# ACMEAtronOmatic/DSen2

Measured on AMD Instinct MI355X. Metric: 32x32x6 patches/sec (DSen2_20, d=6, batch 512), higher is better.
Workload: dtype f32; 1 GPU; DSen2_20 d=6 F=128 fp32, 512 synthetic 32x32 patches (4+6 bands) per GPU per step, he_uniform random-init weights; batch_per_gpu=512, parallelism=patch-sharded dp1, backend=rccl, output_gather=False

## Files before the change

dsen2_amd/DSen2Net.py:

```python
import ctypes
import sys
import threading

import numpy as np
import torch

from . import _lib, weights as _weights

RES_SCALE = 0.1
PRECISIONS = {'fp32': 0, 'bf16': 1, 'bf16x3': 2}


def _ptr(t):
    return ctypes.c_void_p(t.data_ptr()) if t is not None else ctypes.c_void_p(0)


def _stream_ptr(device):
    return ctypes.c_void_p(torch.cuda.current_stream(device).cuda_stream)


def ensemble_mask(ensemble):
    if ensemble is None or ensemble is False:
        return 0
    if ensemble is True:
        return 255
    mask = 0
    for op in ensemble:
        if int(op) != op or not 0 <= int(op) <= 7:
            raise ValueError('an ensemble member must be an op 0..7, got %r' % (op,))
        mask |= 1 << int(op)
    if mask == 0:
        raise ValueError('an ensemble needs at least one member')
    return mask


def dihedral(x, op=None, ops=None, inverse=False, out=None):
    if not torch.cuda.is_available():
        raise RuntimeError('dsen2_amd needs a ROCm GPU (gfx950); there is no CPU fallback')
    if (op is None) == (ops is None):
        raise ValueError('give either op (one for the tensor) or ops (one per sample)')
    if x.dim() != 4 or x.dtype != torch.float32 or not x.is_contiguous() or not x.is_cuda:
        raise ValueError('x must be a contiguous float32 CUDA tensor [n, c, h, w], got %r %s %s' % (tuple(x.shape), x.dtype, x.device))
    n, c, h, w = x.shape
    ops_dev = None
    if ops is not None:
        if h != w:
            raise ValueError('per-sample ops need square images (an odd rotation swaps H and W), got %dx%d' % (h, w))
        if isinstance(ops, torch.Tensor):
            ops_dev = ops
        else:
            host = np.ascontiguousarray(ops, dtype=np.int32)
            if host.size and (host.min() < 0 or host.max() > 7):
                raise ValueError('ops must be 0..7, got %r' % (host.tolist(),))
            ops_dev = torch.from_numpy(host).to(x.device)
        if tuple(ops_dev.shape) != (n,) or ops_dev.dtype != torch.int32 or not ops_dev.is_contiguous() or ops_dev.device != x.device:
            raise ValueError('ops must hold one int32 per sample (%d) on %s' % (n, x.device))
        op = 0
    elif int(op) != op or not 0 <= int(op) <= 7:
        raise ValueError('op must be 0..7, got %r' % (op,))
    shape = (n, c, w, h) if int(op) & 1 else (n, c, h, w)
    if out is None:
        out = torch.empty(shape, dtype=torch.float32, device=x.device)
    elif tuple(out.shape) != shape or out.dtype != torch.float32 or not out.is_contiguous() or out.device != x.device:
        raise ValueError('out must be a contiguous float32 %s tensor of shape %r, got %r %s' % (x.device, shape, tuple(out.shape), out.dtype))
    with torch.cuda.device(x.device):
        _lib.call('dsen2_dihedral_nchw', _ptr(x), _ptr(out), n, c, h, w, int(op), _ptr(ops_dev), int(bool(inverse)),
                  _stream_ptr(x.device))
    return out


class S2Model(object):

    def __init__(self, input_shape, num_layers, feature_size, device=None, precision='fp32'):
        if len(input_shape) not in (2, 3):
            raise ValueError('input_shape must describe 2 or 3 inputs, got %r' % (input_shape,))
        if not torch.cuda.is_available():
            raise RuntimeError('dsen2_amd needs a ROCm GPU (gfx950); there is no CPU fallback')
        self.device = torch.device('cuda', torch.cuda.current_device()) if device is None else torch.device(device)
        self.bands = tuple(int(s[0]) for s in input_shape)
        self.num_layers = int(num_layers)
        self.feature_size = int(feature_size)
        self.cin = sum(self.bands)
        self.cout = self.bands[-1]
        self._handle = ctypes.c_void_p(0)
        c60 = self.bands[2] if len(self.bands) == 3 else 0
        with torch.cuda.device(self.device):
            if precision not in PRECISIONS:
                raise ValueError("precision must be one of %s" % ', '.join(repr(k) for k in PRECISIONS))
            self.precision = precision
            _lib.call('dsen2_model_create', ctypes.byref(self._handle), self.bands[0], self.bands[1], c60,
                      self.num_layers, self.feature_size, PRECISIONS[precision])
        self._workspaces = {}
        self._ws_lock = threading.Lock()
        self.max_workspace_bytes = 6 << 30
        self.optimizer = None
        self._train = None
        self._error_work = None

    def count_params(self):
        return int(_lib.load().dsen2_model_num_params(self._handle))

    def set_weights_flat(self, flat):
        flat = np.ascontiguousarray(flat, np.float32).ravel()
        with torch.cuda.device(self.device):
            _lib.call('dsen2_model_load_weights', self._handle,
                      flat.ctypes.data_as(_lib.c_float_p), flat.size)
            if self._train is not None:
                self._train['flat'].copy_(torch.from_numpy(flat))

    def load_weights(self, path):
        self.set_weights_flat(_weights.load_flat(path, self.cin, self.cout, self.num_layers, self.feature_size))

    def workspace_bytes(self, n, h, w, ensemble=False):
        out = ctypes.c_size_t(0)
        mask = ensemble_mask(ensemble)
        if mask:
            _lib.call('dsen2_model_ensemble_workspace_bytes', self._handle, n, h, w, mask, ctypes.byref(out))
        else:
            _lib.call('dsen2_model_workspace_bytes', self._handle, n, h, w, ctypes.byref(out))
        return out.value

    def _get_workspace(self, nbytes):
        key = torch.cuda.current_stream(self.device).cuda_stream
        with self._ws_lock:
            ws = self._workspaces.get(key)
            if ws is None or ws.numel() < nbytes:
                self._workspaces.pop(key, None)
                ws = None
                ws = torch.empty(nbytes, dtype=torch.uint8, device=self.device)
                self._workspaces[key] = ws
            return ws

    def release_workspaces(self):
        with self._ws_lock:
            self._workspaces.clear()

    def forward_device(self, xs, out=None):
        if len(xs) != len(self.bands):
            raise ValueError('expected %d inputs, got %d' % (len(self.bands), len(xs)))
        n, _, h, w = xs[0].shape
        for x, c in zip(xs, self.bands):
            if tuple(x.shape) != (n, c, h, w) or x.dtype != torch.float32 or not x.is_contiguous() or \
                    x.device != self.device:
                raise ValueError('input must be a contiguous float32 %s tensor of shape %r, got %r %s %s'
                                 % (self.device, (n, c, h, w), tuple(x.shape), x.dtype, x.device))
        out = self._check_out(out, n, h, w)
        if n == 0:
            return out
        ws = self._get_workspace(self.workspace_bytes(n, h, w))
        with torch.cuda.device(self.device):
            _lib.call('dsen2_model_forward', self._handle, _ptr(xs[0]), _ptr(xs[1]),
                      _ptr(xs[2]) if len(xs) == 3 else ctypes.c_void_p(0), _ptr(out), n, h, w,
                      _ptr(ws), ws.numel(), _stream_ptr(self.device))
        return out

    def forward_device_ensemble(self, xs, out=None, ops=range(8)):
        ops = list(range(8)) if ops is True else list(ops)
        mask = ensemble_mask(ops)
        if len(xs) != len(self.bands):
            raise ValueError('expected %d inputs, got %d' % (len(self.bands), len(xs)))
        n, _, h, w = xs[0].shape
        for x, c in zip(xs, self.bands):
            if tuple(x.shape) != (n, c, h, w) or x.dtype != torch.float32 or not x.is_contiguous() or \
                    x.device != self.device:
                raise ValueError('input must be a contiguous float32 %s tensor of shape %r, got %r %s %s'
                                 % (self.device, (n, c, h, w), tuple(x.shape), x.dtype, x.device))
        out = self._check_out(out, n, h, w)
        if n == 0:
            return out
        ws = self._get_workspace(self.workspace_bytes(n, h, w, ensemble=ops))
        with torch.cuda.device(self.device):
            _lib.call('dsen2_model_forward_ensemble', self._handle, _ptr(xs[0]), _ptr(xs[1]),
                      _ptr(xs[2]) if len(xs) == 3 else ctypes.c_void_p(0), _ptr(out), n, h, w, mask,
                      _ptr(ws), ws.numel(), _stream_ptr(self.device))
        return out

    def _check_out(self, out, n, h, w):
        if out is None:
            return torch.empty((n, self.cout, h, w), dtype=torch.float32, device=self.device)
        if tuple(out.shape) != (n, self.cout, h, w) or out.dtype != torch.float32 or not out.is_contiguous() or \
                out.device != self.device:
            raise ValueError('out must be a contiguous float32 %s tensor of shape %r, got %r %s %s (contiguous: %s)'
                             % (self.device, (n, self.cout, h, w), tuple(out.shape), out.dtype, out.device,
                                out.is_contiguous()))
        return out

    def time_body_in_forward(self, xs, out=None, iters=10):
        n, _, h, w = xs[0].shape
        out = self._check_out(out, n, h, w)
        ws = self._get_workspace(self.workspace_bytes(n, h, w))
        ms = ctypes.c_float(0)
        with torch.cuda.device(self.device):
            _lib.call('dsen2_model_forward_timed', self._handle, _ptr(xs[0]), _ptr(xs[1]),
                      _ptr(xs[2]) if len(xs) == 3 else ctypes.c_void_p(0), _ptr(out), n, h, w,
                      _ptr(ws), ws.numel(), _stream_ptr(self.device), int(iters), ctypes.byref(ms))
        return ms.value

    def profile_forward(self, xs, out=None, iters=10, warm=3):
        n, _, h, w = xs[0].shape
        out = self._check_out(out, n, h, w)
        ws = self._get_workspace(self.workspace_bytes(n, h, w))
        ms = (ctypes.c_float * 5)()
        with torch.cuda.device(self.device):
            _lib.call('dsen2_model_forward_profile', self._handle, _ptr(xs[0]), _ptr(xs[1]),
                      _ptr(xs[2]) if len(xs) == 3 else ctypes.c_void_p(0), _ptr(out), n, h, w,
                      _ptr(ws), ws.numel(), _stream_ptr(self.device), int(warm), int(iters), ms)
        return dict(forward_ms=ms[0], first_ms=ms[1], body_ms=ms[2], out_ms=ms[3], wall_ms=ms[4])

    def body_launches(self, n, h, w):
        with torch.cuda.device(self.device):
            r = _lib.load().dsen2_model_body_launches(self._handle, int(n), int(h), int(w))
        if r < 0:
            raise _lib.DSen2Error(r, _lib.load().dsen2_last_error().decode())
        return r

    def batch_limit(self, h, w, ensemble=False):
        per = self.workspace_bytes(1, h, w, ensemble=ensemble)
        return max(1, int(self.max_workspace_bytes // per))

    def preferred_batch(self, h, w, ensemble=False):
        limit = self.batch_limit(h, w, ensemble=ensemble) if ensemble_mask(ensemble) else self.batch_limit(h, w)
        if self.precision == 'fp32' or self.num_layers <= 0:
            return limit
        turned = h != w and ensemble_mask(ensemble) & 0xAA
        cus = int(torch.cuda.get_device_properties(self.device).multi_processor_count)
        n = (limit // cus) * cus
        while n >= cus:
            if self.body_launches(n, h, w) == 1 and (not turned or self.body_launches(n, w, h) == 1):
                return n
            n -= cus
        return limit

    def predict(self, x, batch_size=None, verbose=0, ensemble=False):
        xs = [np.ascontiguousarray(a, dtype=np.float32) for a in x]
        if len(xs) != len(self.bands):
            raise ValueError('expected %d inputs, got %d' % (len(self.bands), len(xs)))
        n, _, h, w = xs[0].shape
        for a, c in zip(xs, self.bands):
            if a.shape != (n, c, h, w):
                raise ValueError('input of shape %r where %r is expected' % (a.shape, (n, c, h, w)))
        mask = ensemble_mask(ensemble if isinstance(ensemble, bool) or ensemble is None else list(ensemble))
        members = [op for op in range(8) if (mask >> op) & 1]
        if batch_size is not None:
            bs = int(batch_size)
        else:
            bs = self.preferred_batch(h, w, ensemble=members) if members else self.preferred_batch(h, w)
        out = np.empty((n, self.cout, h, w), np.float32)
        if n == 0:
            return self._progress_end(verbose, out)
        starts = list(range(0, n, bs))
        bs = min(bs, n)
        with torch.cuda.device(self.device):
            comp = torch.cuda.current_stream(self.device)
            h2d, d2h = torch.cuda.Stream(self.device), torch.cuda.Stream(self.device)
            slots = []
            for _ in range(min(2, len(starts))):
                slots.append(dict(
                    pin_in=[torch.empty((bs, c, h, w), dtype=torch.float32, pin_memory=True) for c in self.bands],
                    dev_in=[torch.empty((bs, c, h, w), dtype=torch.float32, device=self.device) for c in self.bands],
                    dev_out=torch.empty((bs, self.cout, h, w), dtype=torch.float32, device=self.device),
                    pin_out=torch.empty((bs, self.cout, h, w), dtype=torch.float32, pin_memory=True),
                    ev_in=torch.cuda.Event(), ev_comp=torch.cuda.Event(), ev_out=torch.cuda.Event(), span=None))

            def collect(slot):
                if slot['span'] is not None:
                    slot['ev_out'].synchronize()
                    j0, j1 = slot['span']
                    out[j0:j1] = slot['pin_out'][:j1 - j0].numpy()
                    slot['span'] = None
                    self._progress(verbose, j1, n)

            for i, i0 in enumerate(starts):
                i1 = min(n, i0 + bs)
                m = i1 - i0
                slot = slots[i % len(slots)]
                collect(slot)
                for k, a in enumerate(xs):
                    slot['pin_in'][k][:m].numpy()[...] = a[i0:i1]
                with torch.cuda.stream(h2d):
                    for k in range(len(xs)):
                        slot['dev_in'][k][:m].copy_(slot['pin_in'][k][:m], non_blocking=True)
                    slot['ev_in'].record(h2d)
                comp.wait_event(slot['ev_in'])
                if members:
                    self.forward_device_ensemble([t[:m] for t in slot['dev_in']], out=slot['dev_out'][:m], ops=members)
                else:
                    self.forward_device([t[:m] for t in slot['dev_in']], out=slot['dev_out'][:m])
                slot['ev_comp'].record(comp)
                with torch.cuda.stream(d2h):
                    d2h.wait_event(slot['ev_comp'])
                    slot['pin_out'][:m].copy_(slot['dev_out'][:m], non_blocking=True)
                    slot['ev_out'].record(d2h)
                slot['span'] = (i0, i1)
            last = len(starts) - 1
            if len(slots) > 1:
                collect(slots[(last - 1) % 2])
            collect(slots[last % len(slots)])
        return self._progress_end(verbose, out)

    @staticmethod
    def _progress(verbose, done, total):
        if verbose:
            sys.stdout.write('\r%d/%d' % (done, total))
            sys.stdout.flush()

    @staticmethod
    def _progress_end(verbose, out):
        if verbose:
            sys.stdout.write('\n')
        return out

    def time_body_conv(self, layer, x_in, aux, out, iters=10):
        n, h, w, _ = x_in.shape
        ms = ctypes.c_float(0)
        with torch.cuda.device(self.device):
            _lib.call('dsen2_model_time_body_conv', self._handle, layer, _ptr(x_in), _ptr(aux), _ptr(out), n, h, w,
                      iters, _stream_ptr(self.device), ctypes.byref(ms))
        return ms.value

    TRAINABLE = ('fp32', 'bf16x3')
    MIXED_PRECISIONS = {None: 0, 'bf16': 1}

    def compile(self, optimizer='nadam', loss='mean_absolute_error', metrics=None, mixed_precision=None, *, loss_param=None,
                mask_nodata=False, ssim_weight=0.0, ssim_win=11, ssim_sigma=1.5, ssim_data_range=5.0):
        from . import training, losses
        if self.precision not in self.TRAINABLE:
            raise ValueError('training needs an fp32 or a bf16x3 model (this one is %r)' % self.precision)
        if mixed_precision not in self.MIXED_PRECISIONS:
            raise ValueError("mixed_precision must be None or 'bf16', got %r" % (mixed_precision,))
        if mixed_precision is not None and self.precision != 'fp32':
            raise ValueError('mixed_precision=%r is an option of an fp32 model (this one is %r)' % (mixed_precision, self.precision))
        setting = losses.parse_ssim(losses.parse(loss, loss_param, mask_nodata), ssim_weight, ssim_win, ssim_sigma, ssim_data_range)
        if isinstance(optimizer, str):
            if optimizer.lower() != 'nadam':
                raise ValueError("optimizer must be 'nadam' or a dsen2_amd.training.Nadam, got %r" % optimizer)
            optimizer = training.Nadam()
        if not isinstance(optimizer, training.Nadam):
            raise ValueError('optimizer must be a dsen2_amd.training.Nadam')
        if self.precision == 'fp32':
            with torch.cuda.device(self.device):
                _lib.call('dsen2_model_set_train_precision', self._handle, self.MIXED_PRECISIONS[mixed_precision])
        with torch.cuda.device(self.device):
            _lib.call('dsen2_model_set_loss', self._handle, setting[0], setting[1], setting[2])
            ssim = losses.ssim_part(setting) or (0.0, 11, 1.5, 5.0)
            window, c1, c2 = losses.ssim_constants(ssim)
            _lib.call('dsen2_model_set_loss_ssim', self._handle, ssim[0], (ctypes.c_double * window.size)(*window.tolist()),
                      int(window.size), c1, c2)
        self.loss_setting = setting
        self.mixed_precision = mixed_precision
        self.optimizer = optimizer
        self.optimizer.reset()
        self._train = None
        self.stop_training = False

    def _train_state(self):
        if getattr(self, 'optimizer', None) is None:
            raise RuntimeError('compile() the model before training it')
        if self._train is None:
            count = self.count_params()
            kw = dict(dtype=torch.float32, device=self.device)
            flat = torch.empty(count, **kw)
            with torch.cuda.device(self.device):
                _lib.call('dsen2_model_get_weights', self._handle, _ptr(flat), _stream_ptr(self.device))
            self._train = dict(flat=flat, grad=torch.empty(count, **kw), m=torch.zeros(count, **kw),
                               v=torch.zeros(count, **kw), loss2=torch.empty(2, **kw), ws=None)
        return self._train

    def train_workspace_bytes(self, n, h, w):
        out = ctypes.c_size_t(0)
        _lib.call('dsen2_model_train_workspace_bytes', self._handle, n, h, w, ctypes.byref(out))
        return out.value

    def gradients_device(self, xs, y, grad, loss2, out=None, workspace=None):
        if self.precision not in self.TRAINABLE:
            raise ValueError('training needs an fp32 or a bf16x3 model (this one is %r)' % self.precision)
        n, _, h, w = xs[0].shape
        for x, c in zip(xs, self.bands):
            if tuple(x.shape) != (n, c, h, w) or x.dtype != torch.float32 or not x.is_contiguous() or x.device != self.device:
                raise ValueError('input must be a contiguous float32 %s tensor of shape %r' % (self.device, (n, c, h, w)))
        if len(xs) != len(self.bands):
            raise ValueError('expected %d inputs, got %d' % (len(self.bands), len(xs)))
        if tuple(y.shape) != (n, self.cout, h, w) or y.dtype != torch.float32 or not y.is_contiguous() or y.device != self.device:
            raise ValueError('target must be a contiguous float32 %s tensor of shape %r, got %r'
                             % (self.device, (n, self.cout, h, w), tuple(y.shape)))
        if grad.numel() != self.count_params() or not grad.is_contiguous() or loss2.numel() < 2:
            raise ValueError('grad must hold num_params floats, loss2 two')
        if out is not None:
            out = self._check_out(out, n, h, w)
        if workspace is None:
            need = self.train_workspace_bytes(n, h, w)
            st = self._train if self._train is not None else {}
            if st.get('ws') is None or st['ws'].numel() < need:
                st['ws'] = None
                st['ws'] = torch.empty(need, dtype=torch.uint8, device=self.device)
            workspace = st['ws']
        with torch.cuda.device(self.device):
            _lib.call('dsen2_model_gradients', self._handle, _ptr(xs[0]), _ptr(xs[1]),
                      _ptr(xs[2]) if len(xs) == 3 else ctypes.c_void_p(0), _ptr(y), _ptr(out), _ptr(grad), _ptr(loss2),
                      n, h, w, _ptr(workspace), workspace.numel(), _stream_ptr(self.device))
        return out

    def set_weights_device(self, flat):
        if flat.numel() != self.count_params() or flat.dtype != torch.float32 or not flat.is_contiguous() or \
                flat.device != self.device:
            raise ValueError('flat must be a contiguous float32 %s tensor of %d values' % (self.device, self.count_params()))
        with torch.cuda.device(self.device):
            _lib.call('dsen2_model_set_weights_device', self._handle, _ptr(flat), _stream_ptr(self.device))
            if self._train is not None and flat.data_ptr() != self._train['flat'].data_ptr():
                self._train['flat'].copy_(flat)

    def nadam_update(self, grad):
        st = self._train_state()
        s = self.optimizer.next_step()
        with torch.cuda.device(self.device):
            _lib.call('dsen2_nadam_step', _ptr(st['flat']), _ptr(grad), _ptr(st['m']), _ptr(st['v']), st['flat'].numel(),
                      s['lr'], s['b1'], s['b2'], s['eps'], s['mc_t'], s['mc_t1'], s['ms_new'], s['ms_next'], s['b2_pow_t'],
                      _stream_ptr(self.device))
        self.set_weights_device(st['flat'])

    def _to_device(self, arrays, shapes):
        out = []
        for a, shp in zip(arrays, shapes):
            a = np.ascontiguousarray(a, dtype=np.float32)
            if a.shape != shp:
                raise ValueError('array of shape %r where %r is expected' % (a.shape, shp))
            out.append(torch.from_numpy(a).to(self.device))
        return out

    def _shard_rows(self, k):
        st = self._train_state()
        count = st['flat'].numel()
        rows = st.get('rows')
        if rows is None or rows.shape[0] != k:
            stride = -(-(count + 2) // 4) * 4
            rows = st['rows'] = torch.empty((k, stride), dtype=torch.float32, device=self.device)
        return rows

    def nadam_update_shards(self, buf, counts, g_mean=None):
        st = self._train_state()
        count = st['flat'].numel()
        counts = [int(c) for c in counts]
        if buf.dim() != 2 or buf.shape[0] != len(counts) or buf.shape[1] < count or buf.dtype != torch.float32 or \
                buf.device != self.device or buf.stride(1) != 1 or (len(counts) > 1 and buf.stride(0) < count):
            raise ValueError('buf must hold %d float32 %s rows of at least %d values, got %r strides %r'
                             % (len(counts), self.device, count, tuple(buf.shape), buf.stride()))
        if g_mean is not None and (g_mean.numel() != count or g_mean.dtype != torch.float32 or not g_mean.is_contiguous() or
                                   g_mean.device != self.device):
            raise ValueError('g_mean must be a contiguous float32 %s tensor of %d values' % (self.device, count))
        before = (self.optimizer.iterations, self.optimizer.m_schedule)
        s = self.optimizer.next_step()
        try:
            with torch.cuda.device(self.device):
                _lib.call('dsen2_nadam_step_shards', _ptr(st['flat']), _ptr(buf), max(buf.stride(0), count), len(counts),
                          (ctypes.c_int * len(counts))(*counts), _ptr(g_mean), _ptr(st['m']), _ptr(st['v']), count,
                          s['lr'], s['b1'], s['b2'], s['eps'], s['mc_t'], s['mc_t1'], s['ms_new'], s['ms_next'], s['b2_pow_t'],
                          _stream_ptr(self.device))
        except Exception:
            self.optimizer.iterations, self.optimizer.m_schedule = before
            raise
        self.set_weights_device(st['flat'])

    @staticmethod
    def weighted_loss(loss2, counts):
        total = float(sum(counts))
        acc = [0.0, 0.0]
        for l2, c in zip(loss2, counts):
            if c > 0:
                acc[0] += float(c) * float(l2[0])
                acc[1] += float(c) * float(l2[1])
        return [acc[0] / total, acc[1] / total]

    @staticmethod
    def _check_augment_ops(augment_ops, n, h, w):
        if augment_ops is None:
            return None
        ops = np.ascontiguousarray(augment_ops, dtype=np.int32)
        if ops.shape != (n,) or (n and (ops.min() < 0 or ops.max() > 7)):
            raise ValueError('augment_ops must hold one op 0..7 for each of the %d samples, got %r' % (n, np.asarray(augment_ops).tolist()))
        if h != w:
            raise ValueError('augmentation turns every sample by its own op: it needs square patches, got %dx%d' % (h, w))
        return ops

    def _augment_device(self, tensors, ops):
        if ops is None:
            return tensors
        ops_dev = torch.from_numpy(ops).to(self.device)
        return [dihedral(t, ops=ops_dev) for t in tensors]

    def _step_on_shards(self, fetch, counts, mine=None, augment_ops=None):
        from . import dist
        count = self._train_state()['flat'].numel()
        rows = self._shard_rows(len(counts) if mine is None else 1)
        first = 0
        for r, n in enumerate(counts):
            if n > 0 and mine in (None, r):
                x, y = fetch(first, n)
                _, _, h, w = np.shape(x[0])
                if isinstance(y, torch.Tensor):
                    xs, yd = list(x), y
                else:
                    xs = self._to_device(x, [(n, c, h, w) for c in self.bands])
                    yd = self._to_device([y], [(n, self.cout, h, w)])[0]
                if augment_ops is not None:
                    *xs, yd = self._augment_device(xs + [yd], self._check_augment_ops(augment_ops[first:first + n], n, h, w))
                row = rows[r if mine is None else 0]
                self.gradients_device(xs, yd, row[:count], row[count:count + 2])
            first += n
        if mine is not None:
            rows = dist.all_gather_rows(rows[0])
        self.nadam_update_shards(rows, counts)
        return self.weighted_loss(rows[:, count:count + 2].cpu().numpy().astype(np.float64), counts)

    def _shard_counts(self, n, shards):
        from . import dist
        if isinstance(shards, (int, np.integer)):
            if shards < 1:
                raise ValueError('shards must be at least 1, got %d' % shards)
            return [dist.shard_range(n, r, int(shards))[1] for r in range(int(shards))]
        counts = [int(c) for c in shards]
        if not counts or min(counts) < 0 or sum(counts) != n:
            raise ValueError('the shard counts %r must be non-negative and add up to the batch of %d' % (counts, n))
        return counts

    def train_on_batch(self, x, y, shards=None, augment_ops=None):
        st = self._train_state()
        if len(x) != len(self.bands):
            raise ValueError('expected %d inputs, got %d' % (len(self.bands), len(x)))
        n, _, h, w = np.shape(x[0])
        ops = self._check_augment_ops(augment_ops, n, h, w)
        if shards is not None:
            counts = self._shard_counts(n, shards)
            x = [np.ascontiguousarray(a, dtype=np.float32) for a in x]
            y = np.ascontiguousarray(y, dtype=np.float32)
            if y.shape != (n, self.cout, h, w) or any(a.shape != (n, c, h, w) for a, c in zip(x, self.bands)):
                raise ValueError('inputs %r and target %r do not describe one batch' % ([a.shape for a in x], y.shape))
            return self._step_on_shards(lambda first, m: ([a[first:first + m] for a in x], y[first:first + m]), counts,
                                        augment_ops=ops)
        xs = self._to_device(x, [(n, c, h, w) for c in self.bands])
        yd = self._to_device([y], [(n, self.cout, h, w)])[0]
        *xs, yd = self._augment_device(xs + [yd], ops)
        self.gradients_device(xs, yd, st['grad'], st['loss2'])
        self.nadam_update(st['grad'])
        loss = st['loss2'].cpu().numpy().astype(np.float64)
        return [float(loss[0]), float(loss[1])]

    def train_on_device_batch(self, xs, y, loss_out=None):
        st = self._train_state()
        loss2 = st['loss2'] if loss_out is None else loss_out
        if loss2.dtype != torch.float32 or loss2.numel() != 2 or not loss2.is_contiguous() or loss2.device != self.device:
            raise ValueError('loss_out must be a contiguous float32 %s tensor of two values' % (self.device,))
        self.gradients_device(list(xs), y, st['grad'], loss2)
        self.nadam_update(st['grad'])
        return loss2

    def evaluate(self, x, y, batch_size=None, verbose=0):
        y = np.asarray(y, dtype=np.float32)
        pred = self.predict(x, batch_size=batch_size, verbose=verbose)
        if pred.shape != y.shape:
            raise ValueError('target of shape %r where %r is expected' % (y.shape, pred.shape))
        from . import losses
        return losses.host_loss(pred, y, self._loss_setting())

    def _loss_setting(self):
        from . import losses
        return getattr(self, 'loss_setting', losses.DEFAULT)

    def _means_of_triples(self, triples, mine):
        if mine is not None:
            from . import dist
            triples = dist.all_gather_rows(torch.from_numpy(triples[mine]).to(self.device)).cpu().numpy()
        sa = sq = cnt = 0.0
        for t in triples:
            sa, sq, cnt = sa + t[0], sq + t[1], cnt + t[2]
        return [float(sa / cnt), float(sq / cnt)]

    def _evaluate_shards(self, x, y, batch_size, world, mine=None):
        from . import dist, losses
        y = np.asarray(y, dtype=np.float32)
        n = y.shape[0]
        triples = np.zeros((world, 3), np.float64)
        for r in range(world):
            if mine in (None, r):
                first, cnt = dist.shard_range(n, r, world)
                pred = self.predict([a[first:first + cnt] for a in x], batch_size=batch_size)
                triples[r] = losses.host_sums(pred, y[first:first + cnt], self._loss_setting())
        return self._means_of_triples(triples, mine)

    def _data_parallel_plan(self, data_parallel, emulate_world):
        if not data_parallel and emulate_world is None:
            return None
        from . import dist
        rank, world = dist.rank_world()
        if emulate_world is not None:
            if not data_parallel or world > 1 or int(emulate_world) < 1:
                raise ValueError('emulate_world restates a data-parallel run in ONE process: it needs data_parallel=True, a world '
                                 'of at least 1 and no process group of more than one rank')
            return (int(emulate_world), None) if int(emulate_world) > 1 else None
        return (world, rank) if data_parallel and world > 1 else None

    def _data_parallel_start(self, seed):
        from . import dist
        rank, _ = dist.rank_world()
        payload = None
        if rank == 0:
            if seed is None:
                seed = int(np.random.SeedSequence().generate_state(1, np.uint64)[0] >> np.uint64(1))
            payload = np.concatenate([self.get_weights_flat(), np.array([seed], np.uint64).view(np.float32)])
        payload = dist.broadcast_weights(payload, self.count_params() + 2, device=self.device)
        self.set_weights_flat(payload[:-2])
        return int(payload[-2:].view(np.uint64)[0])

    def _sums_device(self, pred, target, out, setting=None):
        for t in (pred, target):
            if t.dtype != torch.float32 or not t.is_contiguous() or t.device != self.device or tuple(t.shape) != tuple(pred.shape) \
                    or (setting is not None and t.dim() != 4):
                raise ValueError('pred and target must be contiguous float32 %s %stensors of one shape'
                                 % (self.device, 'NCHW ' if setting is not None else ''))
        if out.dtype != torch.float64 or out.numel() != 2 or not out.is_contiguous() or out.device != self.device:
            raise ValueError('out must be a contiguous float64 %s tensor of two values' % (self.device,))
        need = ctypes.c_size_t(0)
        _lib.call('dsen2_abs_sq_error_sums_workspace_bytes' if setting is None else 'dsen2_loss_sums_workspace_bytes', ctypes.byref(need))
        size = need.value + (0 if setting is None else 24)
        work = self._error_work
        if work is None or work.numel() < size:
            work = self._error_work = torch.empty(size, dtype=torch.uint8, device=self.device)
        with torch.cuda.device(self.device):
            if setting is None:
                _lib.call('dsen2_abs_sq_error_sums', _ptr(pred), _ptr(target), pred.numel(), _ptr(work), work.numel(), _ptr(out),
                          _stream_ptr(self.device))
                return out
            out3 = work[need.value:need.value + 24].view(torch.float64)
            n, c, h, w = pred.shape
            kind, param, mask = setting
            _lib.call('dsen2_loss_sums', _ptr(pred), _ptr(target), n, c, h * w, kind, param, mask, _ptr(work), need.value, _ptr(out3),
                      _stream_ptr(self.device))
        out.copy_(out3[:2])
        return out

    def abs_sq_error_sums_device(self, pred, target, out):
        return self._sums_device(pred, target, out)

    def loss_sums_device(self, pred, target, out):
        from . import losses
        setting = self._loss_setting()
        kind, param, mask = losses.pointwise(setting)
        self._sums_device(pred, target, out, None if (kind, mask) == (0, 0) else (kind, param, mask))
        if losses.ssim_part(setting):
            s3 = self._ssim_sums_device(pred, target, setting)
            out[0:1].add_(s3[0:1] * losses.ssim_fold(setting, tuple(pred.shape)))
        return out

    def _ssim_sums_device(self, pred, target, setting):
        from . import losses
        window, c1, c2 = losses.ssim_constants(losses.ssim_part(setting))
        need = ctypes.c_size_t(0)
        _lib.call('dsen2_ssim_loss_sums_workspace_bytes', ctypes.byref(need))
        work = getattr(self, '_ssim_work', None)
        if work is None or work.numel() < need.value + 24 or work.device != self.device:
            work = self._ssim_work = torch.empty(need.value + 24, dtype=torch.uint8, device=self.device)
        out3 = work[need.value:need.value + 24].view(torch.float64)
        n, c, h, w = pred.shape
        with torch.cuda.device(self.device):
            _lib.call('dsen2_ssim_loss_sums', _ptr(pred), _ptr(target), n, c, h, w, (ctypes.c_double * window.size)(*window.tolist()),
                      int(window.size), c1, c2, setting[2], _ptr(work), need.value, _ptr(out3), _stream_ptr(self.device))
        return out3

    def _validation_rows(self, corpus, table, rows):
        from . import training
        chunk = self._validation_chunk(corpus)
        for j, i0 in enumerate(range(0, table.shape[0], chunk)):
            xs, y = corpus.batch(table[i0:i0 + chunk], divisor=training.SCALE)
            self.loss_sums_device(self.forward_device(xs), y, rows[j])

    def _validation_chunk(self, corpus):
        return max(1, int(self.preferred_batch(corpus.patch, corpus.patch)))

    @staticmethod
    def _check_validation_crops(corpus, validation_crops):
        table = corpus.check_table(validation_crops)
        if table.shape[0] == 0:
            raise ValueError('validation_crops holds no sample')
        if (table[:, 3] != 0).any():
            raise ValueError('validation is never augmented: every row of validation_crops must have op 0 (corpus.validation_table '
                             'draws such rows), got ops %r' % (sorted(set(table[:, 3].tolist())),))
        return table

    def _validate_crops(self, corpus, table, plan):
        from . import dist
        world, mine = plan
        elements = self.cout * corpus.patch * corpus.patch
        chunk = self._validation_chunk(corpus)
        triples = np.zeros((world, 3), np.float64)
        for r in range(world):
            if mine in (None, r):
                first, cnt = dist.shard_range(table.shape[0], r, world)
                if cnt > 0:
                    rows = torch.empty((-(-cnt // chunk), 2), dtype=torch.float64, device=self.device)
                    self._validation_rows(corpus, table[first:first + cnt], rows)
                    sa = sq = 0.0
                    for row in rows.cpu().numpy():
                        sa, sq = sa + row[0], sq + row[1]
                    triples[r] = (sa, sq, float(cnt * elements))
        return self._means_of_triples(triples, mine)

    def _end_epoch(self, epoch, epochs, sums, count, validation_data, batch_size, plan, callbacks, history, verbose, val=None):
        logs = {'loss': sums[0] / count, 'mean_squared_error': sums[1] / count}
        if val is not None:
            logs['val_loss'], logs['val_mean_squared_error'] = val
        elif validation_data is not None:
            if plan is None:
                vl = self.evaluate(validation_data[0], validation_data[1], batch_size=batch_size)
            else:
                vl = self._evaluate_shards(validation_data[0], validation_data[1], batch_size, plan[0], plan[1])
            logs['val_loss'], logs['val_mean_squared_error'] = vl
        logs['lr'] = self.optimizer.lr
        if verbose:
            sys.stdout.write('\rEpoch %d/%d ' % (epoch + 1, epochs) +
                             ' '.join('%s %.4e' % kv for kv in logs.items()) + '\n')
        for cb in callbacks:
            cb.on_epoch_end(epoch, logs)
        history.append(epoch, logs)
        if plan is not None and plan[1] is not None:
            from . import dist
            dist.assert_replicas_identical(self._train['flat'])

    def fit(self, x=None, y=None, batch_size=32, epochs=1, verbose=1, callbacks=None, validation_data=None, shuffle=True,
            initial_epoch=0, seed=None, data_parallel=False, emulate_world=None, augment=False):
        from . import training
        if getattr(y, 'class_masked', False) or (validation_data is not None and getattr(validation_data[1], 'class_masked', False)):
            training.check_masked_target(self._loss_setting(), True, 'fit')
        plan = self._data_parallel_plan(data_parallel, emulate_world)
        x = [np.ascontiguousarray(a, dtype=np.float32) for a in x]
        y = np.ascontiguousarray(y, dtype=np.float32)
        count = y.shape[0]
        if any(a.shape[0] != count for a in x):
            raise ValueError('inputs and target hold different numbers of samples')
        self._train_state()
        callbacks = list(callbacks or [])
        history = training.History()
        for cb in callbacks:
            cb.set_model(self)
            cb.on_train_begin()
        if plan is not None:
            seed = self._data_parallel_start(seed)
        rng = np.random.default_rng(seed)
        aug = training.AugmentOps(seed) if augment else None
        self.stop_training = False
        for epoch in range(initial_epoch, epochs):
            order = rng.permutation(count) if shuffle else np.arange(count)
            sums = np.zeros(2)
            for i0 in range(0, count, batch_size):
                idx = order[i0:i0 + batch_size]
                ops = aug.draw(len(idx)) if aug is not None else None
                if plan is None:
                    r = self.train_on_batch([a[idx] for a in x], y[idx], augment_ops=ops)
                else:
                    r = self._step_on_shards(lambda first, m: ([a[idx[first:first + m]] for a in x], y[idx[first:first + m]]),
                                             self._shard_counts(len(idx), plan[0]), plan[1], augment_ops=ops)
                sums += np.asarray(r) * len(idx)
                if verbose:
                    sys.stdout.write('\rEpoch %d/%d %d/%d loss %.4e' % (epoch + 1, epochs, min(i0 + batch_size, count), count,
                                                                     sums[0] / min(i0 + batch_size, count)))
                    sys.stdout.flush()
            self._end_epoch(epoch, epochs, sums, count, validation_data, batch_size, plan, callbacks, history, verbose)
            if self.stop_training:
                break
        return history

    def fit_corpus(self, corpus, batch_size, steps_per_epoch, epochs=1, validation_data=None, seed=None, augment=False,
                   callbacks=None, initial_epoch=0, verbose=1, shards=None, data_parallel=False, emulate_world=None,
                   validation_crops=None, masks=None):
        from . import training
        from .corpus import CorpusSampler
        if getattr(corpus, 'class_masked', False):
            training.check_masked_target(self._loss_setting(), True, 'fit_corpus')
        plan = self._data_parallel_plan(data_parallel, emulate_world)
        if plan is not None and shards is not None:
            raise ValueError('shards is the one-process cut of a batch: it cannot be combined with data_parallel')
        batch_size, steps = int(batch_size), int(steps_per_epoch)
        if batch_size < 1 or steps < 1:
            raise ValueError('batch_size and steps_per_epoch must be at least 1, got %d and %d' % (batch_size, steps))
        if corpus.device != self.device or tuple(c for c in self.bands) != tuple(s[1] for s in corpus.output_shapes(1)[0]) or \
                self.cout != corpus.cout:
            raise ValueError('the corpus (%s, run_60=%r) does not feed this model (%s, bands %r)'
                             % (corpus.device, corpus.run_60, self.device, tuple(self.bands)))
        if validation_crops is not None and validation_data is not None:
            raise ValueError('validation_data (host arrays) and validation_crops (a sample table, validated on the device) exclude '
                             'each other')
        val_table = None if validation_crops is None else self._check_validation_crops(corpus, validation_crops)
        self._train_state()
        callbacks = list(callbacks or [])
        history = training.History()
        for cb in callbacks:
            cb.set_model(self)
            cb.on_train_begin()
        if plan is not None:
            seed = self._data_parallel_start(seed)
        sampler = CorpusSampler(corpus, seed, augment, masks=masks)
        sharded = plan is not None or shards is not None
        chunks = 0
        if val_table is not None and plan is None:
            chunks = -(-val_table.shape[0] // self._validation_chunk(corpus))
            val_elements = float(val_table.shape[0] * self.cout * corpus.patch * corpus.patch)
        report = torch.empty((0 if sharded else steps) * 8 + chunks * 16, dtype=torch.uint8, device=self.device)
        if chunks:
            val_rows = report[report.numel() - chunks * 16:].view(torch.float64).view(chunks, 2)
        if not sharded:
            losses = report[:steps * 8].view(torch.float32).view(steps, 2)
            tables = torch.empty((steps, batch_size, 4), dtype=torch.int32).pin_memory()
            tables_dev = torch.empty((steps, batch_size, 4), dtype=torch.int32, device=self.device)
        count = steps * batch_size
        self.stop_training = False
        for epoch in range(initial_epoch, epochs):
            sums = np.zeros(2)
            for i in range(steps):
                table = sampler.draw(batch_size)
                if not sharded:
                    tables[i].numpy()[...] = table
                    tables_dev[i].copy_(tables[i], non_blocking=True)
                    xs, y = corpus.batch(table, table_dev=tables_dev[i])
                    self.train_on_device_batch(xs, y, loss_out=losses[i])
                else:
                    counts = self._shard_counts(batch_size, shards if plan is None else plan[0])
                    r = self._step_on_shards(lambda first, m: corpus.batch(table[first:first + m]), counts,
                                             None if plan is None else plan[1])
                    sums += np.asarray(r) * batch_size
                if verbose:
                    sys.stdout.write('\rEpoch %d/%d %d/%d' % (epoch + 1, epochs, (i + 1) * batch_size, count))
                    sys.stdout.flush()
            val = None
            if chunks:
                self._validation_rows(corpus, val_table, val_rows)
            if not sharded or chunks:
                host = report.cpu().numpy()
                if not sharded:
                    for r in host[:steps * 8].view(np.float32).reshape(steps, 2).astype(np.float64):
                        sums += r * batch_size
                if chunks:
                    sa = sq = 0.0
                    for row in host[host.size - chunks * 16:].view(np.float64).reshape(chunks, 2):
                        sa, sq = sa + row[0], sq + row[1]
                    val = [float(sa / val_elements), float(sq / val_elements)]
            elif val_table is not None:
                val = self._validate_crops(corpus, val_table, plan)
            self._end_epoch(epoch, epochs, sums, count, validation_data, batch_size, plan, callbacks, history, verbose, val=val)
            if self.stop_training:
                break
        return history

    def get_weights_flat(self):
        if self._train is not None:
            flat = self._train['flat']
        else:
            flat = torch.empty(self.count_params(), dtype=torch.float32, device=self.device)
            with torch.cuda.device(self.device):
                _lib.call('dsen2_model_get_weights', self._handle, _ptr(flat), _stream_ptr(self.device))
        return flat.cpu().numpy()

    def save_weights(self, path):
        np.save(path, self.get_weights_flat())

    def __del__(self):
        try:
            if self._handle:
                _lib.load().dsen2_model_destroy(self._handle)
                self._handle = ctypes.c_void_p(0)
        except Exception:
            pass


def s2model(input_shape, num_layers=32, feature_size=256, device=None, precision='fp32'):
    return S2Model(input_shape, num_layers, feature_size, device=device, precision=precision)


def to_blocked(x_nhwc):
    n, h, w, c = x_nhwc.shape
    return x_nhwc.reshape(n, h, w, c // 8, 8).permute(0, 3, 1, 2, 4).contiguous()


def from_blocked(x_blk):
    n, b, h, w, e = x_blk.shape
    return x_blk.permute(0, 2, 3, 1, 4).reshape(n, h, w, b * e).contiguous()


def split_f32(x):
    x = x.contiguous()
    n, h, w, c = x.shape
    hi = torch.empty((n, c // 8, h, w, 8), dtype=torch.int16, device=x.device)
    lo = torch.empty_like(hi)
    with torch.cuda.device(x.device):
        _lib.call('dsen2_split_f32', _ptr(x), _ptr(hi), _ptr(lo), n, h, w, c, _stream_ptr(x.device))
    return hi, lo


def join_f32(hi, lo):
    n, b, h, w, e = hi.shape
    out = torch.empty((n, h, w, b * e), dtype=torch.float32, device=hi.device)
    with torch.cuda.device(hi.device):
        _lib.call('dsen2_join_f32', _ptr(hi), _ptr(lo), _ptr(out), n, h, w, b * e, _stream_ptr(hi.device))
    return out


def split3_f32(x):
    x = x.contiguous()
    n, h, w, c = x.shape
    hx = torch.empty((n, 2, c // 8, h, w, 8), dtype=torch.int16, device=x.device)
    lo = torch.empty((n, c // 8, h, w, 8), dtype=torch.int16, device=x.device)
    with torch.cuda.device(x.device):
        _lib.call('dsen2_split3_f32', _ptr(x), _ptr(hx), _ptr(lo), n, h, w, c, _stream_ptr(x.device))
    return hx, lo


def join3_f32(hx, lo):
    n, _, b, h, w, e = hx.shape
    out = torch.empty((n, h, w, b * e), dtype=torch.float32, device=hx.device)
    with torch.cuda.device(hx.device):
        _lib.call('dsen2_join3_f32', _ptr(hx), _ptr(lo), _ptr(out), n, h, w, b * e, _stream_ptr(hx.device))
    return out


def conv3x3_wgrad_bf16x3(a_planes, g_planes, scale=1.0):
    n, _, b, h, w, e = a_planes.shape
    feat = b * e
    if tuple(g_planes.shape) != tuple(a_planes.shape) or not a_planes.is_contiguous() or not g_planes.is_contiguous():
        raise ValueError('a_planes and g_planes must be contiguous tensors of the same shape')
    dw = torch.empty((3, 3, feat, feat), dtype=torch.float32, device=a_planes.device)
    db = torch.empty(feat, dtype=torch.float32, device=a_planes.device)
    with torch.cuda.device(a_planes.device):
        _lib.call('dsen2_conv3x3_wgrad_bf16x3', _ptr(a_planes), _ptr(g_planes), _ptr(dw), _ptr(db), n, h, w, feat, float(scale),
                  _stream_ptr(a_planes.device))
    return dw, db


def bf16_plane_f32(x):
    return split_f32(x)[0]


def conv3x3_wgrad_bf16(a_plane, g_plane, scale=1.0):
    n, b, h, w, e = a_plane.shape
    feat = b * e
    if tuple(g_plane.shape) != tuple(a_plane.shape) or not a_plane.is_contiguous() or not g_plane.is_contiguous() or \
            a_plane.element_size() != 2 or g_plane.element_size() != 2:
        raise ValueError('a_plane and g_plane must be contiguous 16-bit tensors of the same shape')
    dw = torch.empty((3, 3, feat, feat), dtype=torch.float32, device=a_plane.device)
    db = torch.empty(feat, dtype=torch.float32, device=a_plane.device)
    with torch.cuda.device(a_plane.device):
        _lib.call('dsen2_conv3x3_wgrad_bf16', _ptr(a_plane), _ptr(g_plane), _ptr(dw), _ptr(db), n, h, w, feat, float(scale),
                  _stream_ptr(a_plane.device))
    return dw, db


WGRAD_KINDS = {'fp32': 0, 'bf16x3': 1, 'bf16': 2}


def conv3x3_wgrad_geometry(kind, n, h, w, ca, cg=None):
    cg = ca if cg is None else cg
    tiles, splits, floats = ctypes.c_longlong(0), ctypes.c_int(0), ctypes.c_size_t(0)
    _lib.call('dsen2_conv3x3_wgrad_geometry', WGRAD_KINDS[kind], n, h, w, ca, cg, ctypes.byref(tiles), ctypes.byref(splits),
              ctypes.byref(floats))
    return tiles.value, splits.value, floats.value


def conv3x3_first_planes(xs, kernel_hwio, bias, precision):
    kernel_hwio = np.ascontiguousarray(kernel_hwio, np.float32)
    bias = np.ascontiguousarray(bias, np.float32)
    feat = kernel_hwio.shape[3]
    n, _, h, w = xs[0].shape
    dev = xs[0].device
    xs = [x.contiguous() for x in xs]
    if precision == 2:
        out = torch.empty((n, 2, feat // 8, h, w, 8), dtype=torch.int16, device=dev)
    else:
        out = torch.empty((n, feat // 8, h, w, 8), dtype=torch.int16, device=dev)
    out2 = torch.empty((n, feat // 8, h, w, 8), dtype=torch.int16, device=dev)
    with torch.cuda.device(dev):
        _lib.call('dsen2_conv3x3_first_planes', _ptr(xs[0]), _ptr(xs[1]), _ptr(xs[2]) if len(xs) == 3 else ctypes.c_void_p(0),
                  xs[0].shape[1], xs[1].shape[1], xs[2].shape[1] if len(xs) == 3 else 0,
                  kernel_hwio.ctypes.data_as(_lib.c_float_p), bias.ctypes.data_as(_lib.c_float_p), int(feat), int(precision),
                  _ptr(out), _ptr(out2), n, h, w, _stream_ptr(dev))
    return out, out2


def conv3x3_body_bf16x3(x_planes, kernel_hwio, bias, epilogue=0, res_hx=None, res_lo=None, res_scale=RES_SCALE):
    n, _, blocks, h, w, _ = x_planes.shape
    feat = blocks * 8
    kernel_hwio = np.ascontiguousarray(kernel_hwio, np.float32)
    bias = np.ascontiguousarray(bias, np.float32)
    out = None
    if epilogue == 0:
        out = torch.empty((n, 2, feat // 8, h, w, 8), dtype=torch.int16, device=x_planes.device)
    elif epilogue == 3:
        out = torch.empty((n, h, w, feat), dtype=torch.float32, device=x_planes.device)
    with torch.cuda.device(x_planes.device):
        _lib.call('dsen2_conv3x3_body_bf16x3', _ptr(x_planes.contiguous()), kernel_hwio.ctypes.data_as(_lib.c_float_p),
                  bias.ctypes.data_as(_lib.c_float_p), _ptr(res_hx), _ptr(res_lo), _ptr(out), n, h, w, feat, int(epilogue),
                  float(res_scale), _stream_ptr(x_planes.device))
    return (res_hx, res_lo) if epilogue == 1 else out


def conv3x3_body_bf16(x_bf16, kernel_hwio, bias, epilogue=0, res_hi=None, res_lo=None, res_scale=RES_SCALE):
    n, h, w, feat = x_bf16.shape
    kernel_hwio = np.ascontiguousarray(kernel_hwio, np.float32)
    bias = np.ascontiguousarray(bias, np.float32)
    xb = to_blocked(x_bf16)
    out = None
    if epilogue == 0:
        out = torch.empty((n, feat // 8, h, w, 8), dtype=torch.bfloat16, device=x_bf16.device)
    elif epilogue == 3:
        out = torch.empty((n, h, w, feat), dtype=torch.float32, device=x_bf16.device)
    with torch.cuda.device(x_bf16.device):
        _lib.call('dsen2_conv3x3_body_bf16', _ptr(xb), kernel_hwio.ctypes.data_as(_lib.c_float_p),
                  bias.ctypes.data_as(_lib.c_float_p), _ptr(res_hi), _ptr(res_lo), _ptr(out), n, h, w, feat, int(epilogue),
                  float(res_scale), _stream_ptr(x_bf16.device))
    if epilogue == 1:
        return res_hi, res_lo
    return from_blocked(out) if epilogue == 0 else out


def conv3x3_nhwc(x, kernel_hwio, bias, epilogue=0, aux=None, res_scale=RES_SCALE, ref=False):
    n, h, w, cin = x.shape
    kernel_hwio = np.ascontiguousarray(kernel_hwio, np.float32)
    bias = np.ascontiguousarray(bias, np.float32)
    cout = kernel_hwio.shape[3]
    if epilogue == 2:
        out = torch.empty((n, cout, h, w), dtype=torch.float32, device=x.device)
    else:
        out = torch.empty((n, h, w, cout), dtype=torch.float32, device=x.device)
    with torch.cuda.device(x.device):
        _lib.call('dsen2_conv3x3_nhwc_ref' if ref else 'dsen2_conv3x3_nhwc', _ptr(x), kernel_hwio.ctypes.data_as(_lib.c_float_p),
                  bias.ctypes.data_as(_lib.c_float_p), _ptr(aux), _ptr(out), n, h, w, cin, cout, int(epilogue),
                  float(res_scale), _stream_ptr(x.device))
    return out
```

dsen2_amd/_lib.py:

```python
import ctypes
import os
import sys

_HERE = os.path.dirname(os.path.abspath(__file__))
LIB_PATH = os.environ.get('DSEN2_HIP_LIB') or os.path.join(_HERE, 'libdsen2_hip.so')

OK = 0
ERR_INVALID, ERR_HIP, ERR_NO_WEIGHTS, ERR_WORKSPACE, ERR_NO_DEVICE, ERR_NOMEM, ERR_INTERNAL = -1, -2, -3, -4, -5, -6, -7
DTYPE_U16, DTYPE_F32 = 0, 1
DTYPE_F64 = 2
MASK_BLANK_MAP = 3

c_float_p = ctypes.POINTER(ctypes.c_float)
c_int_p = ctypes.POINTER(ctypes.c_int)
c_void_p = ctypes.c_void_p
c_int = ctypes.c_int
c_size_t = ctypes.c_size_t
c_double = ctypes.c_double


class CorpusTile(ctypes.Structure):
    _fields_ = [('dev_lr10', c_void_p), ('dev_lr20', c_void_p), ('dev_lr60', c_void_p), ('dev_gt', c_void_p),
                ('grid_h', c_int), ('grid_w', c_int), ('gt_dtype', c_int)]


SIGNATURES = {
    'dsen2_version': (ctypes.c_char_p, []),
    'dsen2_last_error': (ctypes.c_char_p, []),
    'dsen2_device_count': (c_int, []),
    'dsen2_model_create': (c_int, [ctypes.POINTER(c_void_p), c_int, c_int, c_int, c_int, c_int, c_int]),
    'dsen2_model_destroy': (None, [c_void_p]),
    'dsen2_model_num_params': (c_size_t, [c_void_p]),
    'dsen2_model_load_weights': (c_int, [c_void_p, c_float_p, c_size_t]),
    'dsen2_model_workspace_bytes': (c_int, [c_void_p, c_int, c_int, c_int, ctypes.POINTER(c_size_t)]),
    'dsen2_model_forward': (c_int, [c_void_p, c_void_p, c_void_p, c_void_p, c_void_p, c_int, c_int, c_int,
                                    c_void_p, c_size_t, c_void_p]),
    'dsen2_model_body_launches': (c_int, [c_void_p, c_int, c_int, c_int]),
    'dsen2_dihedral_nchw': (c_int, [c_void_p, c_void_p, c_int, c_int, c_int, c_int, c_int, c_void_p, c_int, c_void_p]),
    'dsen2_dihedral_accumulate': (c_int, [c_void_p, c_void_p, c_int, c_int, c_int, c_int, c_int, c_int, c_void_p]),
    'dsen2_model_ensemble_workspace_bytes': (c_int, [c_void_p, c_int, c_int, c_int, c_int, ctypes.POINTER(c_size_t)]),
    'dsen2_model_forward_ensemble': (c_int, [c_void_p, c_void_p, c_void_p, c_void_p, c_void_p, c_int, c_int, c_int, c_int,
                                             c_void_p, c_size_t, c_void_p]),
    'dsen2_model_forward_timed': (c_int, [c_void_p, c_void_p, c_void_p, c_void_p, c_void_p, c_int, c_int, c_int,
                                          c_void_p, c_size_t, c_void_p, c_int, c_float_p]),
    'dsen2_model_forward_profile': (c_int, [c_void_p, c_void_p, c_void_p, c_void_p, c_void_p, c_int, c_int, c_int,
                                            c_void_p, c_size_t, c_void_p, c_int, c_int, c_float_p]),
    'dsen2_conv3x3_nhwc': (c_int, [c_void_p, c_float_p, c_float_p, c_void_p, c_void_p, c_int, c_int, c_int, c_int,
                                   c_int, c_int, ctypes.c_float, c_void_p]),
    'dsen2_conv3x3_nhwc_ref': (c_int, [c_void_p, c_float_p, c_float_p, c_void_p, c_void_p, c_int, c_int, c_int, c_int,
                                       c_int, c_int, ctypes.c_float, c_void_p]),
    'dsen2_split_f32': (c_int, [c_void_p, c_void_p, c_void_p, c_int, c_int, c_int, c_int, c_void_p]),
    'dsen2_join_f32': (c_int, [c_void_p, c_void_p, c_void_p, c_int, c_int, c_int, c_int, c_void_p]),
    'dsen2_conv3x3_body_bf16': (c_int, [c_void_p, c_float_p, c_float_p, c_void_p, c_void_p, c_void_p, c_int, c_int, c_int,
                                        c_int, c_int, ctypes.c_float, c_void_p]),
    'dsen2_conv3x3_first_planes': (c_int, [c_void_p, c_void_p, c_void_p, c_int, c_int, c_int, c_float_p, c_float_p, c_int, c_int,
                                           c_void_p, c_void_p, c_int, c_int, c_int, c_void_p]),
    'dsen2_split3_f32': (c_int, [c_void_p, c_void_p, c_void_p, c_int, c_int, c_int, c_int, c_void_p]),
    'dsen2_conv3x3_body_bf16x3': (c_int, [c_void_p, c_float_p, c_float_p, c_void_p, c_void_p, c_void_p, c_int, c_int, c_int,
                                          c_int, c_int, ctypes.c_float, c_void_p]),
    'dsen2_model_time_body_conv': (c_int, [c_void_p, c_int, c_void_p, c_void_p, c_void_p, c_int, c_int, c_int, c_int,
                                           c_void_p, c_float_p]),
    'dsen2_model_train_workspace_bytes': (c_int, [c_void_p, c_int, c_int, c_int, ctypes.POINTER(c_size_t)]),
    'dsen2_model_gradients': (c_int, [c_void_p, c_void_p, c_void_p, c_void_p, c_void_p, c_void_p, c_void_p, c_void_p, c_int,
                                      c_int, c_int, c_void_p, c_size_t, c_void_p]),
    'dsen2_model_set_train_precision': (c_int, [c_void_p, c_int]),
    'dsen2_model_get_weights': (c_int, [c_void_p, c_void_p, c_void_p]),
    'dsen2_model_set_weights_device': (c_int, [c_void_p, c_void_p, c_void_p]),
    'dsen2_nadam_step': (c_int, [c_void_p, c_void_p, c_void_p, c_void_p, c_size_t] + [ctypes.c_float] * 9 + [c_void_p]),
    'dsen2_nadam_step_shards': (c_int, [c_void_p, c_void_p, c_size_t, c_int, c_int_p, c_void_p, c_void_p, c_void_p, c_size_t] +
                                [ctypes.c_float] * 9 + [c_void_p]),
    'dsen2_conv3x3_wgrad': (c_int, [c_void_p, c_void_p, c_void_p, c_void_p, c_int, c_int, c_int, c_int, c_int, c_int, c_int,
                                    ctypes.c_float, c_void_p]),
    'dsen2_conv3x3_wgrad_bf16x3': (c_int, [c_void_p, c_void_p, c_void_p, c_void_p, c_int, c_int, c_int, c_int, ctypes.c_float,
                                           c_void_p]),
    'dsen2_conv3x3_wgrad_bf16': (c_int, [c_void_p, c_void_p, c_void_p, c_void_p, c_int, c_int, c_int, c_int, ctypes.c_float,
                                         c_void_p]),
    'dsen2_conv3x3_wgrad_geometry': (c_int, [c_int, c_int, c_int, c_int, c_int, c_int, ctypes.POINTER(ctypes.c_longlong), c_int_p,
                                             ctypes.POINTER(c_size_t)]),
    'dsen2_join3_f32': (c_int, [c_void_p, c_void_p, c_void_p, c_int, c_int, c_int, c_int, c_void_p]),
    'dsen2_upsample_mirror_bilinear': (c_int, [c_void_p, c_void_p, c_int, c_int, c_int, c_int, c_int, ctypes.c_float,
                                               c_void_p]),
    'dsen2_upsample_mirror_bilinear_ref': (c_int, [c_void_p, c_void_p, c_int, c_int, c_int, c_int, c_int, ctypes.c_float,
                                                   c_void_p]),
    'dsen2_tile_gather': (c_int, [c_void_p, c_int, c_int, c_int, c_int, c_void_p, c_int, c_int, ctypes.c_float,
                                  c_void_p, c_void_p]),
    'dsen2_recompose': (c_int, [c_void_p, c_int, c_int, c_int, c_int, c_void_p, c_int, c_int, ctypes.c_float,
                                c_void_p]),
    'dsen2_recompose_rows': (c_int, [c_void_p, c_int, c_int, c_int, c_int, c_void_p, c_int, c_int, ctypes.c_float,
                                     c_int, c_int, c_void_p]),
    'dsen2_tile_nodata_geometry': (c_int, [c_int, c_int, c_int, c_int, c_int_p, c_int_p, ctypes.POINTER(c_size_t)]),
    'dsen2_tile_nodata': (c_int, [c_void_p, c_int, c_int, c_int, c_int, c_int, c_void_p, c_void_p, c_void_p]),
    'dsen2_recompose_rows_nodata': (c_int, [c_void_p, c_int, c_int, c_int, c_int, c_void_p, c_void_p, c_void_p, c_int, c_int,
                                            ctypes.c_float, c_int, c_int, c_void_p]),
    'dsen2_recompose_rows_blend': (c_int, [c_void_p, c_int, c_int, c_int, c_int, c_int, c_void_p, c_void_p, c_void_p, c_int, c_int,
                                           ctypes.c_float, c_int, c_int, c_void_p]),
    'dsen2_corpus_create': (c_int, [c_void_p, c_int, c_int, ctypes.POINTER(c_void_p)]),
    'dsen2_corpus_destroy': (None, [c_void_p]),
    'dsen2_corpus_batch': (c_int, [c_void_p, c_void_p, c_void_p, c_int, ctypes.c_float, c_void_p, c_void_p, c_void_p, c_void_p,
                                   c_void_p]),
    'dsen2_corpus_origin_mask': (c_int, [c_void_p, c_int, c_int, c_int, c_int, c_int, c_int, c_void_p, c_void_p, c_int, c_int, c_void_p,
                                         c_void_p, c_void_p, c_void_p]),
    'dsen2_class_valid_bits': (c_int, [c_void_p, c_int, c_int, c_void_p, c_int, c_int, c_int, c_int, c_int, c_void_p, c_void_p, c_void_p]),
    'dsen2_tile_flags_from_bits': (c_int, [c_void_p, c_int, c_int, c_int, c_int, c_void_p, c_void_p]),
    'dsen2_raster_apply_valid': (c_int, [c_void_p, c_int, c_int, c_int, c_int, c_void_p, c_void_p]),
    'dsen2_cells_from_valid_bits': (c_int, [c_void_p, c_int, c_int, c_int, c_int, c_void_p, c_void_p]),
    'dsen2_abs_sq_error_sums_workspace_bytes': (c_int, [ctypes.POINTER(c_size_t)]),
    'dsen2_abs_sq_error_sums': (c_int, [c_void_p, c_void_p, ctypes.c_longlong, c_void_p, c_size_t, c_void_p, c_void_p]),
    'dsen2_model_set_loss': (c_int, [c_void_p, c_int, ctypes.c_float, c_int]),
    'dsen2_loss_grad': (c_int, [c_void_p, c_void_p, c_int, c_int, c_int, c_int, c_int, ctypes.c_float, c_int, c_void_p, c_void_p,
                                c_void_p]),
    'dsen2_loss_sums_workspace_bytes': (c_int, [ctypes.POINTER(c_size_t)]),
    'dsen2_loss_sums': (c_int, [c_void_p, c_void_p, c_int, c_int, ctypes.c_longlong, c_int, ctypes.c_float, c_int, c_void_p, c_size_t,
                                c_void_p, c_void_p]),
    'dsen2_model_set_loss_ssim': (c_int, [c_void_p, ctypes.c_float, ctypes.POINTER(c_double), c_int, c_double, c_double]),
    'dsen2_ssim_loss_grad': (c_int, [c_void_p, c_void_p, c_int, c_int, c_int, c_int, ctypes.c_float, ctypes.POINTER(c_double), c_int,
                                     c_double, c_double, c_int, c_void_p, c_void_p, c_void_p]),
    'dsen2_ssim_loss_sums_workspace_bytes': (c_int, [ctypes.POINTER(c_size_t)]),
    'dsen2_ssim_loss_sums': (c_int, [c_void_p, c_void_p, c_int, c_int, c_int, c_int, ctypes.POINTER(c_double), c_int, c_double, c_double,
                                     c_int, c_void_p, c_size_t, c_void_p, c_void_p]),
    'dsen2_down_pixel_aggr': (c_int, [c_void_p, c_int, c_int, c_int, c_int, c_int, ctypes.POINTER(ctypes.c_double), c_int,
                                      c_void_p, c_int, c_void_p]),
    'dsen2_imresize_axis': (c_int, [c_void_p, c_int, c_int, c_int, c_int, c_int, c_int, c_void_p, c_void_p, c_int, c_void_p, c_void_p]),
    'dsen2_band_errors_workspace_bytes': (c_int, [c_int, ctypes.POINTER(c_size_t)]),
    'dsen2_band_errors': (c_int, [c_void_p, c_int, c_void_p, c_int, c_int, c_int, c_int, c_void_p, c_size_t, c_void_p, c_void_p]),
    'dsen2_imresize_band_errors': (c_int, [c_void_p, c_int, c_int, c_int, c_int, c_int, c_int, c_void_p, c_void_p, c_int, c_void_p, c_int,
                                           c_void_p, c_size_t, c_void_p, c_void_p]),
    'dsen2_quality_workspace_bytes': (c_int, [c_int, ctypes.POINTER(c_size_t)]),
    'dsen2_uiq_map': (c_int, [c_void_p, c_int, c_void_p, c_int, c_int, c_int, c_int, c_int, c_void_p, c_void_p]),
    'dsen2_uiq_sums': (c_int, [c_void_p, c_int, c_void_p, c_int, c_int, c_int, c_int, c_int, c_void_p, c_size_t, c_void_p, c_void_p]),
    'dsen2_sam_sums': (c_int, [c_void_p, c_int, c_void_p, c_int, c_int, c_int, c_int, c_void_p, c_size_t, c_void_p, c_void_p]),
    'dsen2_imresize_uiq_sums': (c_int, [c_void_p, c_int, c_int, c_int, c_int, c_int, c_int, c_void_p, c_void_p, c_int, c_void_p, c_int,
                                        c_int, c_void_p, c_size_t, c_void_p, c_void_p]),
    'dsen2_imresize_sam_sums': (c_int, [c_void_p, c_int, c_int, c_int, c_int, c_int, c_int, c_void_p, c_void_p, c_int, c_void_p, c_int,
                                        c_void_p, c_size_t, c_void_p, c_void_p]),
    'dsen2_ssim_map': (c_int, [c_void_p, c_int, c_void_p, c_int, c_int, c_int, c_int, ctypes.POINTER(c_double), c_int, c_double, c_double,
                               c_void_p, c_void_p]),
    'dsen2_ssim_sums': (c_int, [c_void_p, c_int, c_void_p, c_int, c_int, c_int, c_int, ctypes.POINTER(c_double), c_int, c_double, c_double,
                                c_void_p, c_size_t, c_void_p, c_void_p]),
    'dsen2_imresize_ssim_sums': (c_int, [c_void_p, c_int, c_int, c_int, c_int, c_int, c_int, c_void_p, c_void_p, c_int, c_void_p, c_int,
                                         ctypes.POINTER(c_double), c_int, c_double, c_double, c_void_p, c_size_t, c_void_p, c_void_p]),
}

_lib = None


class DSen2Error(RuntimeError):
    def __init__(self, code, message):
        super().__init__('libdsen2_hip error %d: %s' % (code, message))
        self.code = code


def load():
    global _lib
    if _lib is None:
        import torch
        if not os.path.exists(LIB_PATH):
            raise ImportError('%s not found: build it with `python -m dsen2_amd.build` (hipcc, gfx950). '
                              'dsen2_amd has no CPU fallback.' % LIB_PATH)
        if os.environ.get('DSEN2_HIP_LIB'):
            sys.stderr.write('dsen2_amd: DSEN2_HIP_LIB overrides the product library: loading %s\n' % LIB_PATH)
        lib = ctypes.CDLL(LIB_PATH)
        for name, (restype, argtypes) in SIGNATURES.items():
            fn = getattr(lib, name)
            fn.restype = restype
            fn.argtypes = argtypes
        _lib = lib
        want = list(filter(None, os.environ.get('DSEN2_DIAG_SET', '').split(',')))
        if want and not hasattr(lib, 'dsen2_diag_set'):
            raise ImportError('DSEN2_DIAG_SET is set but %s is not a diagnostic build' % LIB_PATH)
        for kv in want:
            key, value = kv.split('=')
            diag_set(int(key), int(value))
    return _lib


def diag_set(key, value):
    lib = load()
    if not hasattr(lib, 'dsen2_diag_set'):
        raise DSen2Error(ERR_INVALID, '%s is not a diagnostic build (python -m dsen2_amd.build --diag)' % LIB_PATH)
    fn = lib.dsen2_diag_set
    fn.restype, fn.argtypes = c_int, [c_int, c_int]
    check(fn(int(key), int(value)))


def check(code):
    if code == ERR_NOMEM:
        raise MemoryError('libdsen2_hip: ' + load().dsen2_last_error().decode('utf-8', 'replace'))
    if code != OK:
        raise DSen2Error(code, load().dsen2_last_error().decode('utf-8', 'replace'))


def call(name, *args):
    check(getattr(load(), name)(*args))
```

dsen2_amd/asm_contract.py:

```python
import os
import re
import subprocess
import tempfile

HERE = os.path.dirname(os.path.abspath(__file__))
CSRC = os.path.join(HERE, 'csrc')
DMA_SOURCES = ['conv3x3_body32.hip', 'conv3x3_body16w.hip']


class AsmContractError(RuntimeError):
    pass


def _code_lines(text):
    return [ln.strip() for ln in text.splitlines() if ln.strip() and not ln.strip().startswith((';', '.', '//'))]


def _kernels(text):
    out, name, body = {}, None, []
    for ln in text.splitlines():
        m = re.match(r'^(_Z\w+):', ln)
        if m:
            name, body = m.group(1), []
            continue
        if name is not None:
            t = ln.strip()
            if t and not t.startswith((';', '.', '//')):
                body.append(t.split(';')[0].strip())
            if t.startswith('s_endpgm'):
                out[name] = body
                name = None
    return out


def normalised(body):
    return [re.sub(r'\.L\w+', 'L', re.sub(r'\s+', ' ', ln)) for ln in body]


def compile_isa(hipcc, flags, path, out, verbose=False):
    cmd = [hipcc] + [f for f in flags if f != '-fPIC'] + ['-S', '--cuda-device-only', path, '-o', out]
    if verbose:
        print(' '.join(cmd), flush=True)
    subprocess.check_call(cmd, stderr=subprocess.DEVNULL)
    with open(out) as f:
        return f.read()


def _needer(src):
    def need(cond, msg, ctx=()):
        if not cond:
            raise AsmContractError('%s: %s %s' % (src, msg, list(ctx)))
    return need


def check_listing(text, src):
    code = _code_lines(text)
    code = [ln.split(';')[0].strip() for ln in code]
    need = _needer(src)

    m0 = [i for i, ln in enumerate(code) if re.search(r'\bm0\b', ln)]
    need(m0, 'no M0 use found (the DMA statements are gone?)')
    dma = [i for i, ln in enumerate(code) if ln.startswith('buffer_load_dword') and ln.endswith('lds')]
    need(dma, 'no LDS-DMA instruction found')
    allowed = set()
    for i in dma:
        need(code[i - 1] == 's_nop 0' and re.match(r's_mov_b32 m0, (s\d+|vcc_lo|vcc_hi)$', code[i - 2]), 'DMA without its M0 write + wait state',
             code[i - 2:i + 1])
        allowed.update((i - 2,))
        for j in range(i - 3, max(i - 7, -1), -1):
            if re.match(r's_mov_b32 (s\d+|vcc_lo|vcc_hi), m0$', code[j]):
                allowed.add(j)
                break
        k = i + 1
        if re.match(r's_mov_b32 m0, (s\d+|vcc_lo|vcc_hi)$', code[k]):
            allowed.add(k)
    for i in m0:
        need(i in allowed, 'M0 touched outside a DMA statement', code[max(0, i - 2):i + 3])
    saves = sum(1 for ln in code if re.match(r's_mov_b32 (s\d+|vcc_lo|vcc_hi), m0$', ln))
    need(saves > 0, 'the DMA statements no longer save M0')
    STEP_MFMAS = 9 * 32
    need(not any(ln.startswith(('s_swappc', 's_call')) for ln in code), 'a DMA kernel calls a function (an epilogue was not inlined)')
    kernels = _kernels(text)
    need(kernels, 'no kernel found')
    n_dma_kernels = 0
    for name, body in kernels.items():
        if not any(ln.startswith('buffer_load_dword') and ln.endswith('lds') for ln in body):
            continue
        n_dma_kernels += 1
        chain = '_chain_kernel' in name
        if not chain:
            need(not any('scratch_' in ln for ln in body), 'kernel %s spills registers' % name)
        else:
            mf = [i for i, ln in enumerate(body) if ln.startswith('v_mfma')]
            need(mf and len(mf) % STEP_MFMAS == 0, 'chain kernel %s: %d MFMAs is not a whole number of item bodies' % (name, len(mf)))
            for g in range(0, len(mf), STEP_MFMAS):
                inner = body[mf[g]:mf[g + STEP_MFMAS - 1]]
                need(not any('scratch_' in ln for ln in inner), 'chain kernel %s spills inside an item body' % name)
            for i, ln in enumerate(body):
                if 'scratch_' not in ln:
                    continue
                nxt = None
                for ln2 in body[i + 1:]:
                    if ln2.startswith('v_mfma'):
                        break
                    mm = re.search(r'vmcnt\((\d+)\)', ln2) if ln2.startswith('s_waitcnt') else None
                    if mm:
                        nxt = int(mm.group(1))
                        break
                need(nxt == 0, 'chain kernel %s: scratch access outside a drained region (next vmcnt wait: %r)' % (name, nxt), [ln])
        back = [ln for ln in body[-40:] if ln.startswith('s_waitcnt') and 'vmcnt' in ln]
        need(back and back[-1].replace(' ', '') in ('s_waitcntvmcnt(0)', 's_waitcntvmcnt(0)lgkmcnt(0)'),
             'kernel %s does not drain its DMAs before s_endpgm' % name, back[-3:])
    need(n_dma_kernels > 0, 'no LDS-DMA kernel found')
    if src == 'conv3x3_body32.hip':
        ITEM_MFMAS = 2 * 9 * 64
        asym = {k: v for k, v in kernels.items() if re.search(r'conv3x3_body32_kernelILi\d+ELi\d+ELi\d+ELi\d+ELi\d+ELi[2-9]E', k)}
        need(asym, 'no DeferAsym instantiation of the fp32 body kernel found')
        for name, body in asym.items():
            mf = [i for i, ln in enumerate(body) if ln.startswith('v_mfma')]
            need(len(mf) == 2 * ITEM_MFMAS, 'kernel %s: %d MFMAs, expected two copies of the item loop' % (name, len(mf)))
            copies = [body[mf[0]:mf[ITEM_MFMAS - 1]], body[mf[ITEM_MFMAS]:mf[-1]]]
            n_dma = [sum(1 for ln in c if ln.startswith('buffer_load_dword') and ln.endswith('lds')) for c in copies]
            need(min(n_dma) == 0 and max(n_dma) > 0, 'kernel %s: DMAs in both copies of the item loop' % name, n_dma)
            quiet, loud = (copies[0], copies[1]) if n_dma[0] == 0 else (copies[1], copies[0])
            need(not any(re.search(r'\bm0\b', ln) for ln in quiet), 'kernel %s: M0 use in the compute-only copy' % name)
            run = None
            for ln in loud:
                if re.match(r's_mov_b32 (s\d+|vcc_lo|vcc_hi), m0$', ln):
                    need(run is None, 'kernel %s: M0 saved twice in one DMA statement' % name)
                    run = 0
                elif ln.startswith('buffer_load_dword') and ln.endswith('lds'):
                    need(run is not None, 'kernel %s: DMA outside a statement that saves M0' % name)
                    run += 1
                elif run and not re.match(r'(s_mov_b32 m0, |s_nop 0$)', ln):
                    need(run in (2, 4), 'kernel %s: a DMA statement of %d instructions' % (name, run))
                    run = None
    if src == 'conv3x3_body16w.hip':
        expect = {0: (0, 32), 1: (64, 64), 3: (64, 64)}
        expect3 = {0: (0, 64), 1: (64, 96), 3: (64, 64)}

        def count(pattern, want, msg, product=lambda m: True):
            found = []
            for name, body in kernels.items():
                m = re.search(pattern, name)
                if not m or not product(m):
                    continue
                found.append(body)
                loads = sum(1 for ln in body if ln.startswith('buffer_load_dwordx4') and not ln.endswith('lds'))
                stores = sum(1 for ln in body if ln.startswith('buffer_store_dwordx4'))
                need((loads, stores) == want(m), msg(m) % (loads, stores, want(m)))
            return found

        def total(e):
            return lambda m: (sum(v[0] for v in e.values()), sum(v[1] for v in e.values()))

        found = count(r'conv3x3_body16[wx]_kernelILi(\d+)ELi(\d+)ELi(\d+)ELi(\d+)E', lambda m: expect[int(m.group(3))],
                      lambda m: 'epilogue ' + m.group(3) + ' has %d loads / %d stores, the waits count %r', lambda m: int(m.group(4)) == 0)
        need(len(found) >= 6, 'expected the 6 product instantiations of the bf16 body kernel, found %d' % len(found))
        for body in found:
            other = [ln for ln in body if re.match(r'(buffer|global|flat)_(load|store|atomic)', ln)
                     and not ln.startswith(('buffer_load_dwordx4', 'buffer_store_dwordx4'))]
            need(len(other) <= 1, 'unexpected vector-memory instructions in the bf16 body kernel', other[:4])
        found3 = count(r'conv3x3_body16w_x3_kernelILi(\d+)ELi(\d+)ELi(\d+)E', lambda m: expect3[int(m.group(3))],
                       lambda m: 'bf16x3 epilogue ' + m.group(3) + ' has %d loads / %d stores, the waits count %r')
        need(len(found3) == 6, 'expected the 6 instantiations of the bf16x3 body kernel, found %d' % len(found3))
        chains = count(r'conv3x3_body16w_chain_kernelILi(\d+)ELi(\d+)ELi(\d+)E', total(expect),
                       lambda m: 'chain kernel has %d loads / %d stores in its epilogues, the waits count %r', lambda m: int(m.group(3)) == 0)
        need(len(chains) == 2, 'expected the 2 product instantiations of the chain kernel, found %d' % len(chains))
        chains3 = count(r'conv3x3_body16w_x3_chain_kernelILi(\d+)ELi(\d+)E', total(expect3),
                        lambda m: 'bf16x3 chain kernel has %d loads / %d stores in its epilogues, the waits count %r')
        need(len(chains3) == 2, 'expected the 2 instantiations of the bf16x3 chain kernel, found %d' % len(chains3))


def check_out_mfma_listing(text, src='conv3x3_out_mfma.hip'):
    need = _needer(src)
    kernels = {k: v for k, v in _kernels(text).items() if 'conv3x3_out_mfma_kernel' in k}
    need(len(kernels) == 4, 'expected 4 instantiations of the output kernel, found %d' % len(kernels))
    for name, body in kernels.items():
        need(not any('scratch_' in ln for ln in body), 'kernel %s spills registers' % name)
        need(not any(ln.startswith(('s_swappc', 's_call')) for ln in body), 'kernel %s calls a function' % name)
        mf = [i for i, ln in enumerate(body) if ln.startswith('v_mfma')]
        need(mf, 'kernel %s has no MFMA' % name)
        waits = [ln for ln in body[mf[0]:mf[-1]] if ln.startswith('s_waitcnt') and 'vmcnt' in ln]
        need(len(waits) >= 8, 'kernel %s: no operand waits between its MFMAs' % name)
        bad = [ln for ln in waits if int(re.search(r'vmcnt\((\d+)\)', ln).group(1)) < 8]
        need(not bad, 'kernel %s waits for the loads of the NEXT unit' % name, bad[:4])
    return True


def check_first16_listing(text, src='conv3x3_first16.hip'):
    need = _needer(src)
    kernels = {k: v for k, v in _kernels(text).items() if 'conv3x3_first16_kernel' in k}
    need(len(kernels) == 8, 'expected 8 instantiations of the kernel, found %d' % len(kernels))
    for name, body in kernels.items():
        need(not any('scratch_' in ln for ln in body), 'kernel %s spills registers' % name)
        need(not any(ln.startswith(('s_swappc', 's_call')) for ln in body), 'kernel %s calls a function' % name)
        stores = [ln for ln in body if ln.startswith('buffer_store_dwordx4')]
        need(stores, 'kernel %s has no 128-bit buffer store' % name)
        bad = [ln for ln in stores if not re.search(r'\], 0 offen', ln)]
        need(not bad, 'kernel %s: 128-bit buffer store with a register soffset (late data read, unpadded hazard)' % name, bad[:2])
        need(not any(ln.startswith('global_store') for ln in body), 'kernel %s stores outside its buffer descriptors' % name)
        mf = [i for i, ln in enumerate(body) if ln.startswith('v_mfma')]
        need(mf, 'kernel %s has no MFMA' % name)
        x3 = 'ELb1EEE' in name
        floor = 24 if x3 else 16
        loop = body[mf[0]:]
        scat = [i for i, ln in enumerate(loop) if ln.startswith('ds_write_b16')]
        need(scat, 'kernel %s: no halo scatter after the first MFMA' % name)
        waits = [ln for ln in loop[:scat[-1]] if ln.startswith('s_waitcnt') and 'vmcnt' in ln]
        low = [ln for ln in waits if int(re.search(r'vmcnt\((\d+)\)', ln).group(1)) < floor]
        need(not low, 'kernel %s: a wait inside the tile loop drains the deferred stores (divergent branch in the loop body?)' % name, low[:4])
    return True


TRAFFIC_KERNELS = {
    'dsen2_20_fp32': ('conv3x3_body32.hip', r'conv3x3_body32_kernelILi128ELi128ELi0ELi0ELi0ELi4ELb1E'),
    'vdsen2_20_bf16': ('conv3x3_body16w.hip', r'conv3x3_body16w_chain_kernelILi128ELi256ELi0E'),
    'dsen2_20_bf16x3': ('conv3x3_body16w.hip', r'conv3x3_body16w_x3_chain_kernelILi64ELi128E'),
    'vdsen2_20_fp32': ('conv3x3_body32.hip', r'conv3x3_body32_kernelILi256ELi256ELi0ELi0ELi0ELi4ELb1E'),
    'dsen2_20_bf16': ('conv3x3_body16w.hip', r'conv3x3_body16w_chain_kernelILi64ELi128ELi0E'),
    'vdsen2_20_bf16x3': ('conv3x3_body16w.hip', r'conv3x3_body16w_x3_chain_kernelILi128ELi256E'),
}
ISA_JSON = os.path.join(HERE, 'kernel_isa.json')


def isa_hashes(text):
    import hashlib
    out = {}
    for name, body in _kernels(text).items():
        out[name] = hashlib.sha256('\n'.join(normalised(body)).encode()).hexdigest()
    return out


def traffic_kernel_hashes(listings):
    out = {}
    for cfg, (src, pat) in TRAFFIC_KERNELS.items():
        hits = {k: v for k, v in isa_hashes(listings[src]).items() if re.search(pat, k)}
        if len(hits) != 1:
            raise AsmContractError('%s: expected one kernel matching %s, found %d' % (src, pat, len(hits)))
        (k, v), = hits.items()
        out[cfg] = {'kernel': k, 'isa_sha256': v}
    return out


def check_sources(hipcc, flags, verbose=False, isa_json=None):
    listings = {}
    with tempfile.TemporaryDirectory(prefix='dsen2_asm_') as tmp:
        for src in DMA_SOURCES + ['conv3x3_out_mfma.hip', 'conv3x3_first16.hip']:
            listings[src] = compile_isa(hipcc, flags, os.path.join(CSRC, src), os.path.join(tmp, src + '.s'), verbose)
            if src in DMA_SOURCES:
                check_listing(listings[src], src)
            elif src == 'conv3x3_first16.hip':
                check_first16_listing(listings[src], src)
            else:
                check_out_mfma_listing(listings[src], src)
    hashes = traffic_kernel_hashes(listings)
    if isa_json:
        import json
        with open(isa_json, 'w') as f:
            json.dump(hashes, f, indent=1, sort_keys=True)
            f.write('\n')
    return hashes
```

dsen2_amd/csrc/capi.hip:

```cpp

#include <chrono>
#include <cstdarg>
#include <cstdio>
#include <cstring>
#include <exception>
#include <new>
#include <vector>

#include "capi_internal.h"

using namespace dsen2;

namespace {

thread_local char g_err[512] = "";

#ifdef DSEN2_DIAG
Tuning g_diag_tuning;
unsigned long long* g_diag_stamps = nullptr;
#endif
Tuning default_tuning() {
#ifdef DSEN2_DIAG
  return g_diag_tuning;
#else
  return Tuning{};
#endif
}

constexpr int kWarmLaunches = 24;

}

namespace dsen2 {
int fail(int code, const char* fmt, ...) {
  va_list ap;
  va_start(ap, fmt);
  vsnprintf(g_err, sizeof(g_err), fmt, ap);
  va_end(ap);
  return code;
}
}

static bool may_chain(const dsen2_model* m) {
  return m->chain_stride != 0 && m->tune.chain && m->tune.grid_cap == 0 && (m->precision == 1 || m->tune.ablate == 0);
}

static int first_layer(const dsen2_model* m, const float* x10, const float* x20, const float* x60, int n, int h, int w,
                       const ForwardWs& B, bool x0_packed, hipStream_t stream) {
  const Layer& L = m->layers[0];
  const ConvPlan& pl = L.plan;
  const float* P = m->dev_params;
  const bool x3 = m->precision == 2 && m->num_layers > 0;
  ConvParams pf = make_params(B.x0, L.weights(P), L.bias(P), nullptr, B.a, n, h, w, 0, 0.f);
  if (pl.epilogue == kEpiReluSplit) {
    pf.out = reinterpret_cast<float*>(B.s0);
    pf.out2 = B.s1;
  }
  const FirstInputs fi{x60, m->c10, m->c20, m->c60};
  ConvParams pd = pf;
  pd.in = x10;
  pd.aux = x20;
  bool done = false;
  if (pl.first16_planes) {
    pd.wpk = L.first16(P);
    pd.out = reinterpret_cast<float*>(B.s0);
    pd.out2 = B.s1;
    HIP_TRY(try_launch(launch_conv3x3_first16(pd, fi, m->feat, x3, stream), &done));
  } else if (pl.first_direct) {
    HIP_TRY(try_launch(launch_conv3x3_first(pd, fi, m->feat, pl.epilogue, stream, m->tune.first_ablate), &done));
  }
  if (!done) {
    if (!x0_packed) HIP_TRY(launch_pack_inputs(x10, x20, x60, m->c10, m->c20, m->c60, B.x0, n, h, w, stream));
    HIP_TRY(launch(pl, pf, pl.epilogue, m->tune, stream));
    if (x3) HIP_TRY(launch_split3_f32(B.a, B.s0, B.s1, n, h, w, m->feat, stream));
  }
  return DSEN2_OK;
}

static size_t operand16_bytes(const dsen2_model* m, int n, int h, int w) {
  return (size_t)n * h * w * m->feat * (m->precision == 2 ? 4 : 2);
}

static int body16(const dsen2_model* m, void* s0, void* s1, void* t16, float* out_f32, int n, int h, int w, hipStream_t stream,
                  size_t keep_step = 0, void* xkeep = nullptr) {
  const float* P = m->dev_params;
  if (keep_step == 0 && may_chain(m)) {
    const Layer& L1 = m->layers[1];
    const bool x3 = L1.plan.kernel == ConvKernel::Body16x3;
    ConvParams pc = make_params(nullptr, L1.weights(P), L1.bias(P), nullptr, nullptr, n, h, w, 0, 0.1f);
#ifdef DSEN2_DIAG
    if (!x3) pc.diag = g_diag_stamps;
#endif
    ChainArgs ca;
    ca.hi = s0; ca.lo = s1; ca.t = t16; ca.out_f32 = out_f32;
    ca.layer_stride = (unsigned)m->chain_stride; ca.n_layers = 2 * m->num_layers; ca.patches_per_wg = 0; ca.seamless = 0;
    bool done = false;
    HIP_TRY(try_launch(launch_conv3x3_body16w_chain(pc, ca, m->feat, stream, m->tune.ablate, x3), &done));
    if (done) return DSEN2_OK;
  }
  for (int l = 1; l <= m->num_layers; ++l) {
    const Layer& LA = m->layers[2 * l - 1];
    const Layer& LB = m->layers[2 * l];
    float* const t = reinterpret_cast<float*>(t16) + (size_t)(l - 1) * keep_step;
    HIP_TRY(launch(LA.plan, make_params(reinterpret_cast<const float*>(s0), LA.weights(P), LA.bias(P), nullptr, t, n, h, w, 0, 0.f),
                   kEpiRelu, m->tune, stream));
    const bool last = l == m->num_layers;
    ConvParams pb = make_params(t, LB.weights(P), LB.bias(P),
                                reinterpret_cast<const float*>(s0), last ? out_f32 : reinterpret_cast<float*>(s0), n, h, w, 0, 0.1f);
    pb.out2 = s1;
    HIP_TRY(launch(LB.plan, pb, last ? kEpiResidualF32 : kEpiResidual, m->tune, stream));
    if (keep_step > 0 && !last)
      HIP_TRY(hipMemcpyAsync(reinterpret_cast<float*>(xkeep) + (size_t)l * keep_step, s0, operand16_bytes(m, n, h, w),
                             hipMemcpyDeviceToDevice, stream));
  }
  return DSEN2_OK;
}

namespace dsen2 {

ForwardWs forward_ws(const dsen2_model* m, int n, int h, int w, char* base) {
  const size_t pix = (size_t)n * h * w;
  const size_t full = align_up(pix * m->feat), half = align_up(pix * m->feat / 2);
  ForwardWs r;
  size_t off = 0;
  auto take = [&](size_t floats) -> float* {
    float* p = base ? reinterpret_cast<float*>(base) + off : nullptr;
    off += floats;
    return p;
  };
  r.x0 = take(align_up(pix * 16));
  r.a = take(full);
  if (m->precision == 0) {
    r.t = take(full);
  } else {
    const size_t operand = m->precision == 2 ? full : half;
    r.s0 = take(operand); r.s1 = take(half); r.t16 = take(operand);
  }
  r.bytes = off * sizeof(float);
  return r;
}

int forward_launches(const dsen2_model* m, const float* x10, const float* x20, const float* x60, float* out, int n, int h, int w,
                     const ForwardWs& B, size_t keep_step, bool x0_packed, hipStream_t stream, const hipEvent_t* ev) {
  const float* P = m->dev_params;
  const int d = m->num_layers;
  if (ev) HIP_TRY(hipEventRecord(ev[0], stream));
  if (int rc = first_layer(m, x10, x20, x60, n, h, w, B, x0_packed, stream)) return rc;
  if (ev) HIP_TRY(hipEventRecord(ev[1], stream));
  if (m->precision != 0 && d > 0) {
    if (keep_step > 0) {
      HIP_TRY((m->precision == 2 ? launch_join3_f32 : launch_join_f32)(B.s0, B.s1, B.x0f, n, h, w, m->feat, stream));
      HIP_TRY(hipMemcpyAsync(B.xkeep, B.s0, operand16_bytes(m, n, h, w), hipMemcpyDeviceToDevice, stream));
    }
    if (int rc = body16(m, B.s0, B.s1, B.t16, B.a, n, h, w, stream, keep_step, B.xkeep)) return rc;
  } else {
    for (int l = 1; l <= d; ++l) {
      const Layer& LA = m->layers[2 * l - 1];
      const Layer& LB = m->layers[2 * l];
      const float* x_in = B.a + (size_t)(l - 1) * keep_step;
      float* t = B.t + (size_t)(l - 1) * keep_step;
      HIP_TRY(launch(LA.plan, make_params(x_in, LA.weights(P), LA.bias(P), nullptr, t, n, h, w, 0, 0.f), LA.plan.epilogue, m->tune, stream));
      HIP_TRY(launch(LB.plan, make_params(t, LB.weights(P), LB.bias(P), x_in, B.a + (size_t)l * keep_step, n, h, w, 0, 0.1f),
                     LB.plan.epilogue, m->tune, stream));
    }
  }
  if (ev) HIP_TRY(hipEventRecord(ev[2], stream));
  {
    const Layer& L = m->layers.back();
    const float* skip = m->c60 > 0 ? x60 : x20;
    const float* x_d = B.a + (m->precision == 0 ? (size_t)d * keep_step : 0);
    ConvParams po = make_params(x_d, L.weights(P), L.bias(P), skip, out, n, h, w, m->cout, 0.f);
#ifdef DSEN2_DIAG
    po.diag = g_diag_stamps;
#endif
    HIP_TRY(launch(L.plan, po, L.plan.epilogue, m->tune, stream));
  }
  if (ev) HIP_TRY(hipEventRecord(ev[3], stream));
  return DSEN2_OK;
}

}

static int forward(dsen2_model* m, const float* x10, const float* x20, const float* x60, float* out, int n, int h, int w,
                   void* workspace, size_t workspace_bytes, void* stream, const hipEvent_t* ev) {
  if (!m || !x10 || !x20 || !out || !workspace) return fail(DSEN2_ERR_INVALID, "NULL argument");
  if ((m->c60 > 0) != (x60 != nullptr)) return fail(DSEN2_ERR_INVALID, "x60 must be given iff the model has a 60 m input");
  if (!m->loaded) return fail(DSEN2_ERR_NO_WEIGHTS, "dsen2_model_load_weights has not been called");
  if (int rc = check_shape(m, n, h, w)) return rc;
  if (int rc = check_device(m)) return rc;
  const ForwardWs B = forward_ws(m, n, h, w, reinterpret_cast<char*>(workspace));
  if (workspace_bytes < B.bytes) return fail(DSEN2_ERR_WORKSPACE, "workspace %zu < %zu bytes", workspace_bytes, B.bytes);
  return forward_launches(m, x10, x20, x60, out, n, h, w, B, 0, false, (hipStream_t)stream, ev);
}

static int forward_profile(dsen2_model* m, const float* x10, const float* x20, const float* x60, float* out, int n, int h, int w,
                           void* workspace, size_t workspace_bytes, void* stream, int warm, int iters, float* ms) {
  if (iters <= 0 || iters > 4096 || warm < 0 || warm > 4096 || !ms) return fail(DSEN2_ERR_INVALID, "bad warm / iters / NULL result");
  if (!m) return fail(DSEN2_ERR_INVALID, "NULL model");
  Events evs;
  if (int rc = evs.create(4 * (size_t)iters)) return rc;
  for (int i = 0; i < warm; ++i) {
    int rc = forward(m, x10, x20, x60, out, n, h, w, workspace, workspace_bytes, stream, nullptr);
    if (rc != DSEN2_OK) return rc;
  }
  const auto t0 = std::chrono::steady_clock::now();
  for (int i = 0; i < iters; ++i) {
    int rc = forward(m, x10, x20, x60, out, n, h, w, workspace, workspace_bytes, stream, &evs.ev[4 * (size_t)i]);
    if (rc != DSEN2_OK) {
      (void)hipStreamSynchronize((hipStream_t)stream);
      return rc;
    }
  }
  HIP_TRY(hipEventSynchronize(evs.ev.back()));
  const auto t1 = std::chrono::steady_clock::now();
  double sum[4] = {0.0, 0.0, 0.0, 0.0};
  for (int i = 0; i < iters; ++i) {
    const hipEvent_t* e = &evs.ev[4 * (size_t)i];
    float v = 0.f;
    HIP_TRY(hipEventElapsedTime(&v, e[0], e[3])); sum[0] += v;
    HIP_TRY(hipEventElapsedTime(&v, e[0], e[1])); sum[1] += v;
    HIP_TRY(hipEventElapsedTime(&v, e[1], e[2])); sum[2] += v;
    HIP_TRY(hipEventElapsedTime(&v, e[2], e[3])); sum[3] += v;
  }
  for (int k = 0; k < 4; ++k) ms[k] = (float)(sum[k] / iters);
  double wall = std::chrono::duration<double, std::milli>(t1 - t0).count();
  if (warm > 0) {
    float span = 0.f;
    HIP_TRY(hipEventElapsedTime(&span, evs.ev.front(), evs.ev.back()));
    wall = span;
  }
  ms[4] = (float)(wall / iters);
  return DSEN2_OK;
}

static int conv3x3_nhwc(const float* dev_in, const float* host_kernel, const float* host_bias, const float* dev_aux, float* dev_out,
                        int n, int h, int w, int cin, int cout, int epilogue, float res_scale, void* stream_, const Tuning& tune) {
  if (!dev_in || !host_kernel || !host_bias || !dev_out) return fail(DSEN2_ERR_INVALID, "NULL argument");
  if (epilogue != kEpiRelu && epilogue != kEpiResidual && epilogue != kEpiSkipNCHW) return fail(DSEN2_ERR_INVALID, "epilogue %d", epilogue);
  if (epilogue != kEpiRelu && !dev_aux) return fail(DSEN2_ERR_INVALID, "epilogue %d needs dev_aux", epilogue);
  if (int rc = check_shape(nullptr, n, h, w)) return rc;
  const ConvRole role = epilogue == kEpiSkipNCHW ? ConvRole::Output
                        : cin <= 16 ? (epilogue == kEpiRelu ? ConvRole::First : ConvRole::DgradOutput)
                        : epilogue == kEpiRelu ? ConvRole::BodyA : ConvRole::BodyB;
  ConvPlan pl;
  if (!plan_conv(role, cin, cout, 0, tune, nullptr, &pl) || pl.cin_pad != cin)
    return fail(DSEN2_ERR_INVALID, "unsupported conv %d->%d epilogue %d", cin, cout, epilogue);
  hipStream_t stream = (hipStream_t)stream_;
  std::vector<float> staged(pl.floats);
  pack(pl, host_kernel, host_bias, staged.data());
  return launch_once_with_temp("conv3x3", staged.data(), staged.size() * sizeof(float), stream, [&](char* dev) {
    const float* wpk = reinterpret_cast<const float*>(dev);
    return launch(pl, make_params(dev_in, wpk, wpk + pl.bias_off, dev_aux, dev_out, n, h, w, cout, res_scale), epilogue, tune, stream);
  });
}

static int conv3x3_body16(int precision, const void* dev_in, const float* host_kernel, const float* host_bias, void* s0, void* s1,
                          void* dev_out, int n, int h, int w, int feat, int epilogue, float res_scale, void* stream_) {
  const bool x3 = precision == 2;
  if (!dev_in || !host_kernel || !host_bias) return fail(DSEN2_ERR_INVALID, "NULL argument");
  if (feat != 128 && feat != 256) return fail(DSEN2_ERR_INVALID, "feat %d unsupported", feat);
  if (epilogue != kEpiRelu && epilogue != kEpiResidual && epilogue != kEpiResidualF32) return fail(DSEN2_ERR_INVALID, "epilogue %d", epilogue);
  if (epilogue != kEpiRelu && (!s0 || !s1))
    return fail(DSEN2_ERR_INVALID, x3 ? "residual epilogue needs the stream's tensors" : "residual epilogue needs the hi and lo planes");
  if (epilogue != kEpiResidual && !dev_out) return fail(DSEN2_ERR_INVALID, "dev_out is NULL");
  if (int rc = check_shape(nullptr, n, h, w)) return rc;
  hipStream_t stream = (hipStream_t)stream_;
  const Tuning tune = default_tuning();
  ConvPlan pl;
  if (!plan_conv(epilogue == kEpiRelu ? ConvRole::BodyA : ConvRole::BodyB, feat, feat, precision, tune, nullptr, &pl))
    return fail(DSEN2_ERR_INVALID, "feat %d unsupported", feat);
  std::vector<float> staged(pl.floats);
  pack(pl, host_kernel, host_bias, staged.data());
  return launch_once_with_temp(x3 ? "bf16x3 conv" : "bf16 conv", staged.data(), staged.size() * sizeof(float), stream, [&](char* dev) {
    const float* wpk = reinterpret_cast<const float*>(dev);
    ConvParams p = make_params(reinterpret_cast<const float*>(dev_in), wpk, wpk + pl.bias_off, reinterpret_cast<const float*>(s0),
                               reinterpret_cast<float*>(epilogue == kEpiResidual ? s0 : dev_out), n, h, w, 0, res_scale);
    p.out2 = s1;
    return launch(pl, p, epilogue, tune, stream);
  });
}

static int check_split_args(const void* a, const void* b, const void* c_, int n, int h, int w, int c) {
  if (!a || !b || !c_ || n < 0 || h <= 0 || w <= 0 || c <= 0 || c % 8 != 0 || c > 512)
    return fail(DSEN2_ERR_INVALID, "bad argument (c must be a multiple of 8, at most 512)");
  return DSEN2_OK;
}

static int upsample(const float* dev_in, float* dev_out, int planes, int h, int w, int oh, int ow, float post_divisor, void* stream,
                    bool general) {
  if (!dev_in || !dev_out || planes < 0 || h <= 0 || w <= 0 || oh <= 0 || ow <= 0 || post_divisor == 0.f)
    return fail(DSEN2_ERR_INVALID, "bad argument");
  if ((size_t)h * w >= ((size_t)1 << 31) || (size_t)oh * ow >= ((size_t)1 << 31))
    return fail(DSEN2_ERR_INVALID, "plane too large");
  if (planes == 0) return DSEN2_OK;
  HIP_TRY(launch_upsample(dev_in, dev_out, planes, h, w, oh, ow, post_divisor, (hipStream_t)stream, general));
  return DSEN2_OK;
}

static int recompose_rows(const float* dev_patches, int count, int C, int P, int border, float* dev_img, int H, int W, float scale,
                          int row0, int row1, void* stream) {
  if (!dev_patches || !dev_img || count <= 0 || C <= 0 || P <= 0 || border < 0 || H <= 0 || W <= 0)
    return fail(DSEN2_ERR_INVALID, "bad argument");
  hipError_t e = launch_recompose(dev_patches, count, C, P, border, dev_img, H, W, scale, row0, row1, (hipStream_t)stream);
  if (e == hipErrorInvalidValue)
    return fail(DSEN2_ERR_INVALID, "recompose geometry: count=%d P=%d border=%d H=%d W=%d rows [%d, %d)", count, P, border, H, W, row0, row1);
  if (e != hipSuccess) return fail(DSEN2_ERR_HIP, "recompose launch: %s", hipGetErrorString(e));
  return DSEN2_OK;
}

static bool overlaps(const void* a, size_t a_bytes, const void* b, size_t b_bytes) {
  const uintptr_t x = reinterpret_cast<uintptr_t>(a), y = reinterpret_cast<uintptr_t>(b);
  return x < y + b_bytes && y < x + a_bytes;
}

static int check_dihedral_args(const void* in, const void* out, int n, int c, int h, int w, int op, size_t* elems) {
  if (!in || !out) return fail(DSEN2_ERR_INVALID, "NULL argument");
  if (n < 0 || c <= 0 || h <= 0 || w <= 0) return fail(DSEN2_ERR_INVALID, "bad shape n=%d c=%d h=%d w=%d", n, c, h, w);
  if (op < 0 || op > 7) return fail(DSEN2_ERR_INVALID, "op %d outside 0..7", op);
  *elems = (size_t)n * c * h * w;
  if (*elems >= ((size_t)1 << 31)) return fail(DSEN2_ERR_INVALID, "tensor of %zu elements (2^31 or more)", *elems);
  if (*elems > 0 && overlaps(in, *elems * sizeof(float), out, *elems * sizeof(float))) return fail(DSEN2_ERR_INVALID, "the output aliases the input");
  return DSEN2_OK;
}

namespace {
struct EnsembleWs {
  char* fwd = nullptr;
  size_t fwd_bytes = 0;
  float *x10 = nullptr, *x20 = nullptr, *x60 = nullptr, *y = nullptr;
  size_t bytes = 0;
};
}

static EnsembleWs ensemble_ws(const dsen2_model* m, int n, int h, int w, int mask, char* base) {
  const size_t pix = (size_t)n * h * w;
  EnsembleWs r;
  r.fwd = base;
  r.fwd_bytes = forward_ws(m, n, h, w, nullptr).bytes;
  size_t off = r.fwd_bytes / sizeof(float);
  auto take = [&](size_t floats) -> float* {
    float* p = base ? reinterpret_cast<float*>(base) + off : nullptr;
    off += align_up(floats);
    return p;
  };
  if (mask & ~1) {
    r.x10 = take(pix * m->c10);
    r.x20 = take(pix * m->c20);
    if (m->c60 > 0) r.x60 = take(pix * m->c60);
    r.y = take(pix * m->cout);
  }
  r.bytes = off * sizeof(float);
  return r;
}

static int check_ensemble_shape(const dsen2_model* m, int n, int h, int w, int mask) {
  if (mask <= 0 || mask > 255) return fail(DSEN2_ERR_INVALID, "ensemble mask %d outside 1..255", mask);
  if (int rc = check_shape(m, n, h, w)) return rc;
  if (int rc = check_shape(m, n, w, h)) return rc;
  int cmax = m->cout;
  for (int c : {m->c10, m->c20, m->c60}) cmax = c > cmax ? c : cmax;
  if ((size_t)n * h * w * cmax >= ((size_t)1 << 31))
    return fail(DSEN2_ERR_INVALID, "batch of %d images of %dx%d: a tensor of 2^31 elements or more", n, h, w);
  return DSEN2_OK;
}

static int forward_ensemble(dsen2_model* m, const float* x10, const float* x20, const float* x60, float* out, int n, int h, int w,
                            int mask, void* workspace, size_t workspace_bytes, void* stream_) {
  if (!m || !x10 || !x20 || !out || !workspace) return fail(DSEN2_ERR_INVALID, "NULL argument");
  if ((m->c60 > 0) != (x60 != nullptr)) return fail(DSEN2_ERR_INVALID, "x60 must be given iff the model has a 60 m input");
  if (mask <= 0 || mask > 255) return fail(DSEN2_ERR_INVALID, "ensemble mask %d outside 1..255", mask);
  if (n == 0) return DSEN2_OK;
  if (!m->loaded) return fail(DSEN2_ERR_NO_WEIGHTS, "dsen2_model_load_weights has not been called");
  if (int rc = check_ensemble_shape(m, n, h, w, mask)) return rc;
  if (int rc = check_device(m)) return rc;
  const size_t pix = (size_t)n * h * w;
  const float* const ins[3] = {x10, x20, x60};
  const int cs[3] = {m->c10, m->c20, m->c60};
  for (int k = 0; k < 3; ++k)
    if (ins[k] && overlaps(ins[k], pix * cs[k] * sizeof(float), out, pix * m->cout * sizeof(float)))
      return fail(DSEN2_ERR_INVALID, "the output aliases an input");
  const EnsembleWs E = ensemble_ws(m, n, h, w, mask, reinterpret_cast<char*>(workspace));
  if (workspace_bytes < E.bytes) return fail(DSEN2_ERR_WORKSPACE, "workspace %zu < %zu bytes", workspace_bytes, E.bytes);
  hipStream_t stream = (hipStream_t)stream_;
  int count = 0;
  for (int op = 0; op < 8; ++op) count += (mask >> op) & 1;
  int done = 0;
  for (int op = 0; op < 8; ++op) {
    if (!((mask >> op) & 1)) continue;
    const bool first = done == 0, last = done + 1 == count;
    if (op == 0) {
      const ForwardWs B = forward_ws(m, n, h, w, E.fwd);
      if (int rc = forward_launches(m, x10, x20, x60, out, n, h, w, B, 0, false, stream, nullptr)) return rc;
    } else {
      const bool tr = op & 1;
      const int th = tr ? w : h, tw = tr ? h : w;
      float* const turned[3] = {E.x10, E.x20, E.x60};
      for (int k = 0; k < 3; ++k)
        if (ins[k]) HIP_TRY(launch_dihedral(ins[k], turned[k], n, cs[k], h, w, op, nullptr, false, stream));
      const ForwardWs B = forward_ws(m, n, th, tw, E.fwd);
      if (int rc = forward_launches(m, E.x10, E.x20, E.x60, E.y, n, th, tw, B, 0, false, stream, nullptr)) return rc;
      if (first) HIP_TRY(launch_dihedral(E.y, out, n, m->cout, th, tw, op, nullptr, true, stream));
      else HIP_TRY(launch_dihedral_accumulate(E.y, out, n, m->cout, h, w, op, last ? count : 0, stream));
    }
    ++done;
  }
  return DSEN2_OK;
}

extern "C" {

const char* dsen2_version(void) {
#ifdef DSEN2_DIAG
  return "dsen2_hip 0.3-diag (gfx950; fp32 MFMA 32x32x2 / bf16 MFMA 16x16x32 / bf16x3; DIAGNOSTIC build)";
#else
  return "dsen2_hip 0.3 (gfx950; fp32 MFMA 32x32x2 / bf16 MFMA 16x16x32 / bf16x3)";
#endif
}
const char* dsen2_last_error(void) { return g_err; }

#ifdef DSEN2_DIAG
int dsen2_diag_set(int key, int value) {
  Tuning& t = g_diag_tuning;
  switch (key) {
    case 0:
      if (value != 0 && (value < 11 || value > 19)) return fail(DSEN2_ERR_INVALID, "body variant %d unknown", value);
      t.first = value == 0 ? FirstKernel::Tile16 : FirstKernel::Direct;
      t.body = value == 0 ? BodyKernel::Tile : BodyKernel::Body32;
      t.body32 = value == 0 ? Body32Form::DeferAsym : static_cast<Body32Form>(value - 11);
      return DSEN2_OK;
    case 2:
      if (value != 0 && value != 2 && value != 3) return fail(DSEN2_ERR_INVALID, "output variant %d unknown", value);
      t.out = value == 2 ? OutKernel::MfmaThenValu : value == 3 ? OutKernel::Valu : OutKernel::Tile;
      return DSEN2_OK;
    case 1: t.ablate = value; return DSEN2_OK;
    case 3: t.grid_cap = value; return DSEN2_OK;
    case 4: t.chain = value; return DSEN2_OK;
    case 5: t.first_ablate = value; return DSEN2_OK;
    case 6: t.out_ablate = value; return DSEN2_OK;
  }
  return fail(DSEN2_ERR_INVALID, "unknown diagnostic key %d", key);
}
int dsen2_diag_set_stamps(void* dev_buffer) {
  g_diag_stamps = reinterpret_cast<unsigned long long*>(dev_buffer);
  return DSEN2_OK;
}
#endif

int dsen2_device_count(void) {
  int n = 0;
  hipError_t e = hipGetDeviceCount(&n);
  if (e != hipSuccess) {
    (void)hipGetLastError();
    return fail(DSEN2_ERR_NO_DEVICE, "hipGetDeviceCount: %s", hipGetErrorString(e));
  }
  int good = 0;
  for (int i = 0; i < n; ++i) {
    hipDeviceProp_t prop;
    if (hipGetDeviceProperties(&prop, i) == hipSuccess && strncmp(prop.gcnArchName, "gfx950", 6) == 0) ++good;
  }
  return good;
}

int dsen2_model_create(dsen2_model** out, int c10, int c20, int c60, int num_layers, int feature_size, int precision) {
  return guarded([&]() -> int {
    if (!out) return fail(DSEN2_ERR_INVALID, "out is NULL");
    *out = nullptr;
    if (c10 <= 0 || c20 <= 0 || c60 < 0 || num_layers < 0) return fail(DSEN2_ERR_INVALID, "bad channel/layer counts");
    if (feature_size != 128 && feature_size != 256)
      return fail(DSEN2_ERR_INVALID, "feature_size %d unsupported (128 or 256)", feature_size);
    if (precision < 0 || precision > 2)
      return fail(DSEN2_ERR_INVALID, "precision %d unknown (0 = fp32, 1 = bf16 operands, 2 = bf16x3)", precision);
    const int cin = c10 + c20 + c60;
    const int cout = c60 > 0 ? c60 : c20;
    if (cin > 16) return fail(DSEN2_ERR_INVALID, "%d input channels > 16", cin);
    dsen2_model* m = new (std::nothrow) dsen2_model();
    if (!m) return fail(DSEN2_ERR_INVALID, "out of host memory");
    m->c10 = c10; m->c20 = c20; m->c60 = c60; m->cin = cin; m->cout = cout;
    m->num_layers = num_layers; m->feat = feature_size; m->precision = precision;
    m->dev_params = nullptr; m->loaded = false; m->train = nullptr;
    m->tune = default_tuning();
    if (hipGetDevice(&m->device) != hipSuccess) {
      delete m;
      return fail(DSEN2_ERR_NO_DEVICE, "no HIP device");
    }
    if (!plan_network(c10, c20, c60, num_layers, feature_size, precision, m->tune, m)) {
      delete m;
      return fail(DSEN2_ERR_INVALID, "no kernel for a layer of this network");
    }
    *out = m;
    return DSEN2_OK;
  });
}

void dsen2_model_destroy(dsen2_model* m) {
  if (!m) return;
  train_state_destroy(m->train);
  if (m->dev_params) (void)hipFree(m->dev_params);
  delete m;
}

size_t dsen2_model_num_params(const dsen2_model* m) { return m ? m->n_params : 0; }

int dsen2_model_load_weights(dsen2_model* m, const float* host_flat, size_t count) {
  return guarded([&]() -> int {
    if (!m || !host_flat) return fail(DSEN2_ERR_INVALID, "NULL argument");
    if (count != m->n_params)
      return fail(DSEN2_ERR_INVALID, "expected %zu parameters, got %zu", m->n_params, count);
    if (int rc = check_device(m)) return rc;
    std::vector<float> staged(m->dev_param_floats);
    for (const Layer& L : m->layers) {
      const float* k = host_flat + L.flat_off;
      pack(L.plan, k, k + (size_t)9 * L.plan.cin * L.plan.cout, staged.data() + L.off);
    }
    if (!m->dev_params) HIP_TRY(hipMalloc((void**)&m->dev_params, m->dev_param_floats * sizeof(float)));
    HIP_TRY(hipMemcpy(m->dev_params, staged.data(), m->dev_param_floats * sizeof(float), hipMemcpyHostToDevice));
    m->loaded = true;
    if (m->train_planes() == 2) m->host_flat.assign(host_flat, host_flat + count);
    if (m->train) return train_state_after_load(m);
    return DSEN2_OK;
  });
}

int dsen2_model_workspace_bytes(const dsen2_model* m, int n, int h, int w, size_t* bytes) {
  if (!m || !bytes || n <= 0 || h <= 0 || w <= 0) return fail(DSEN2_ERR_INVALID, "bad argument");
  *bytes = forward_ws(m, n, h, w, nullptr).bytes;
  return DSEN2_OK;
}

int dsen2_model_forward(dsen2_model* m, const float* x10, const float* x20, const float* x60, float* out, int n, int h, int w,
                        void* workspace, size_t workspace_bytes, void* stream) {
  return guarded([&] { return forward(m, x10, x20, x60, out, n, h, w, workspace, workspace_bytes, stream, nullptr); });
}

int dsen2_model_body_launches(const dsen2_model* m, int n, int h, int w) {
  return guarded([&]() -> int {
    if (!m) return fail(DSEN2_ERR_INVALID, "NULL model");
    if (int rc = check_shape(m, n, h, w)) return rc;
    if (int rc = check_device(m)) return rc;
    int dev = 0, cus = 0;
    if (hipGetDevice(&dev) != hipSuccess || hipDeviceGetAttribute(&cus, hipDeviceAttributeMultiprocessorCount, dev) != hipSuccess)
      return fail(DSEN2_ERR_NO_DEVICE, "no HIP device");
    return may_chain(m) && body16w_chain_patches_per_wg(n, h, w, m->feat, cus) > 0 ? 1 : 2 * m->num_layers;
  });
}

int dsen2_model_forward_timed(dsen2_model* m, const float* x10, const float* x20, const float* x60, float* out, int n, int h, int w,
                              void* workspace, size_t workspace_bytes, void* stream, int iters, float* body_ms_per_launch) {
  return guarded([&]() -> int {
    if (!body_ms_per_launch) return fail(DSEN2_ERR_INVALID, "NULL result");
    if (!m || m->num_layers <= 0) return fail(DSEN2_ERR_INVALID, "model has no residual blocks");
    float ms[5];
    int rc = forward_profile(m, x10, x20, x60, out, n, h, w, workspace, workspace_bytes, stream, 0, iters, ms);
    if (rc == DSEN2_OK) *body_ms_per_launch = ms[2] / (2.0f * m->num_layers);
    return rc;
  });
}

int dsen2_model_forward_profile(dsen2_model* m, const float* x10, const float* x20, const float* x60, float* out, int n, int h,
                                int w, void* workspace, size_t workspace_bytes, void* stream, int warm, int iters, float* ms5) {
  return guarded([&] { return forward_profile(m, x10, x20, x60, out, n, h, w, workspace, workspace_bytes, stream, warm, iters, ms5); });
}

int dsen2_conv3x3_nhwc(const float* dev_in, const float* host_kernel, const float* host_bias, const float* dev_aux, float* dev_out,
                       int n, int h, int w, int cin, int cout, int epilogue, float res_scale, void* stream) {
  return guarded([&] {
    return conv3x3_nhwc(dev_in, host_kernel, host_bias, dev_aux, dev_out, n, h, w, cin, cout, epilogue, res_scale, stream, default_tuning());
  });
}

int dsen2_conv3x3_nhwc_ref(const float* dev_in, const float* host_kernel, const float* host_bias, const float* dev_aux,
                           float* dev_out, int n, int h, int w, int cin, int cout, int epilogue, float res_scale, void* stream) {
  return guarded([&] {
    return conv3x3_nhwc(dev_in, host_kernel, host_bias, dev_aux, dev_out, n, h, w, cin, cout, epilogue, res_scale, stream,
                        Tuning::reference());
  });
}

int dsen2_split_f32(const float* dev_in, void* dev_hi, void* dev_lo, int n, int h, int w, int c, void* stream) {
  return guarded([&]() -> int {
    if (int rc = check_split_args(dev_in, dev_hi, dev_lo, n, h, w, c)) return rc;
    if (n == 0) return DSEN2_OK;
    HIP_TRY(launch_split_f32(dev_in, dev_hi, dev_lo, n, h, w, c, (hipStream_t)stream));
    return DSEN2_OK;
  });
}

int dsen2_join_f32(const void* dev_hi, const void* dev_lo, float* dev_out, int n, int h, int w, int c, void* stream) {
  return guarded([&]() -> int {
    if (int rc = check_split_args(dev_hi, dev_lo, dev_out, n, h, w, c)) return rc;
    if (n == 0) return DSEN2_OK;
    HIP_TRY(launch_join_f32(dev_hi, dev_lo, dev_out, n, h, w, c, (hipStream_t)stream));
    return DSEN2_OK;
  });
}

int dsen2_split3_f32(const float* dev_in, void* dev_hx, void* dev_lo, int n, int h, int w, int c, void* stream) {
  return guarded([&]() -> int {
    if (int rc = check_split_args(dev_in, dev_hx, dev_lo, n, h, w, c)) return rc;
    if (n == 0) return DSEN2_OK;
    HIP_TRY(launch_split3_f32(dev_in, dev_hx, dev_lo, n, h, w, c, (hipStream_t)stream));
    return DSEN2_OK;
  });
}

int dsen2_join3_f32(const void* dev_hx, const void* dev_lo16, float* dev_out, int n, int h, int w, int c, void* stream) {
  return guarded([&]() -> int {
    if (int rc = check_split_args(dev_hx, dev_lo16, dev_out, n, h, w, c)) return rc;
    if (n == 0) return DSEN2_OK;
    HIP_TRY(launch_join3_f32(dev_hx, dev_lo16, dev_out, n, h, w, c, (hipStream_t)stream));
    return DSEN2_OK;
  });
}

int dsen2_conv3x3_body_bf16(const void* dev_in_bf16, const float* host_kernel, const float* host_bias, void* dev_res_hi,
                            void* dev_res_lo, void* dev_out, int n, int h, int w, int feat, int epilogue, float res_scale,
                            void* stream) {
  return guarded([&] {
    return conv3x3_body16(1, dev_in_bf16, host_kernel, host_bias, dev_res_hi, dev_res_lo, dev_out, n, h, w, feat, epilogue, res_scale, stream);
  });
}

int dsen2_conv3x3_body_bf16x3(const void* dev_in_planes, const float* host_kernel, const float* host_bias, void* dev_res_hx,
                              void* dev_res_lo, void* dev_out, int n, int h, int w, int feat, int epilogue, float res_scale,
                              void* stream) {
  return guarded([&] {
    return conv3x3_body16(2, dev_in_planes, host_kernel, host_bias, dev_res_hx, dev_res_lo, dev_out, n, h, w, feat, epilogue, res_scale, stream);
  });
}

int dsen2_conv3x3_first_planes(const float* dev_x10, const float* dev_x20, const float* dev_x60, int c10, int c20, int c60,
                               const float* host_kernel, const float* host_bias, int feat, int precision, void* dev_out,
                               void* dev_out2, int n, int h, int w, void* stream_) {
  return guarded([&]() -> int {
    if (!dev_x10 || !dev_x20 || !host_kernel || !host_bias || !dev_out || !dev_out2) return fail(DSEN2_ERR_INVALID, "NULL argument");
    if ((c60 > 0) != (dev_x60 != nullptr)) return fail(DSEN2_ERR_INVALID, "dev_x60 must be given iff c60 > 0");
    if (feat != 128 && feat != 256) return fail(DSEN2_ERR_INVALID, "feat %d unsupported", feat);
    if (precision != 1 && precision != 2) return fail(DSEN2_ERR_INVALID, "precision %d (1 = bf16 operands, 2 = bf16x3)", precision);
    if (c10 != 4 || c20 != 6 || (c60 != 0 && c60 != 2)) return fail(DSEN2_ERR_INVALID, "band groups %d + %d + %d (4 + 6 (+ 2) only)", c10, c20, c60);
    if (int rc = check_shape(nullptr, n, h, w)) return rc;
    hipStream_t stream = (hipStream_t)stream_;
    const BandGroups bands{c10, c20, c60};
    ConvPlan pl;
    if (!plan_conv(ConvRole::First, c10 + c20 + c60, feat, precision, default_tuning(), &bands, &pl) || !pl.first16_planes)
      return fail(DSEN2_ERR_INVALID, "no bf16 first convolution for this shape");
    std::vector<float> staged(pl.floats);
    pack(pl, host_kernel, host_bias, staged.data());
    return launch_once_with_temp("first convolution (bf16 matrix cores)", staged.data(), staged.size() * sizeof(float), stream, [&](char* dev) {
      const float* buf = reinterpret_cast<const float*>(dev);
      ConvParams p = make_params(dev_x10, buf + pl.first16_off, buf + pl.bias_off, dev_x20, reinterpret_cast<float*>(dev_out), n, h, w, 0, 0.f);
      p.out2 = dev_out2;
      return launch_conv3x3_first16(p, FirstInputs{dev_x60, c10, c20, c60}, feat, precision == 2, stream);
    });
  });
}

int dsen2_model_time_body_conv(dsen2_model* m, int layer, const float* dev_in, const float* dev_aux, float* dev_out, int n, int h,
                               int w, int iters, void* stream_, float* ms_per_launch) {
  return guarded([&]() -> int {
    if (!m || !dev_in || !dev_out || !ms_per_launch || iters <= 0) return fail(DSEN2_ERR_INVALID, "bad argument");
    if (!m->loaded) return fail(DSEN2_ERR_NO_WEIGHTS, "weights not loaded");
    if (layer < 1 || layer > 2 * m->num_layers) return fail(DSEN2_ERR_INVALID, "layer %d out of range", layer);
    if (int rc = check_shape(m, n, h, w)) return rc;
    if (int rc = check_device(m)) return rc;
    const Layer& L = m->layers[layer];
    if (L.plan.kernel == ConvKernel::Body16x3) return fail(DSEN2_ERR_INVALID, "dsen2_model_time_body_conv: not available for precision 2 (use dsen2_model_forward_profile)");
    if (L.plan.epilogue == kEpiResidual && !dev_aux) return fail(DSEN2_ERR_INVALID, "residual layer needs dev_aux");
    hipStream_t stream = (hipStream_t)stream_;
    const float* P = m->dev_params;
    ConvParams p = make_params(dev_in, L.weights(P), L.bias(P), dev_aux, dev_out, n, h, w, 0, 0.1f);
    int epi = L.plan.epilogue;
    if (L.plan.kernel == ConvKernel::Body16 && epi == kEpiResidual) {
      const bool last = layer == 2 * m->num_layers;
      p.out2 = reinterpret_cast<char*>(const_cast<float*>(dev_aux)) + (size_t)n * h * w * m->feat * 2;
      p.out = last ? dev_out : const_cast<float*>(dev_aux);
      epi = last ? kEpiResidualF32 : kEpiResidual;
    }
#ifdef DSEN2_DIAG
    p.diag = g_diag_stamps;
#endif
    auto launch = [&]() -> hipError_t { return dsen2::launch(L.plan, p, epi, m->tune, stream); };
    Events ev;
    if (int rc = ev.create(2)) return rc;
    for (int i = 0; i < kWarmLaunches; ++i) HIP_TRY(launch());
    HIP_TRY(hipEventRecord(ev.ev[0], stream));
    for (int i = 0; i < iters; ++i) HIP_TRY(launch());
    HIP_TRY(hipEventRecord(ev.ev[1], stream));
    HIP_TRY(hipEventSynchronize(ev.ev[1]));
    float ms = 0.f;
    HIP_TRY(hipEventElapsedTime(&ms, ev.ev[0], ev.ev[1]));
    *ms_per_launch = ms / iters;
    return DSEN2_OK;
  });
}

int dsen2_upsample_mirror_bilinear(const float* dev_in, float* dev_out, int planes, int h, int w, int oh, int ow, float post_divisor,
                                   void* stream) {
  return guarded([&] { return upsample(dev_in, dev_out, planes, h, w, oh, ow, post_divisor, stream, false); });
}

int dsen2_upsample_mirror_bilinear_ref(const float* dev_in, float* dev_out, int planes, int h, int w, int oh, int ow,
                                       float post_divisor, void* stream) {
  return guarded([&] { return upsample(dev_in, dev_out, planes, h, w, oh, ow, post_divisor, stream, true); });
}

int dsen2_tile_gather(const float* dev_img, int H, int W, int C, int border, const int* dev_origins, int count, int P, float divisor,
                      float* dev_patches, void* stream) {
  return guarded([&]() -> int {
    if (!dev_img || !dev_patches || (!dev_origins && count > 0) || H <= 0 || W <= 0 || C <= 0 || border < 0 ||
        count < 0 || P <= 0 || divisor == 0.f)
      return fail(DSEN2_ERR_INVALID, "bad argument");
    if (border > H || border > W) return fail(DSEN2_ERR_INVALID, "border %d larger than the image", border);
    if ((size_t)C * P * P >= ((size_t)1 << 31)) return fail(DSEN2_ERR_INVALID, "patch too large");
    HIP_TRY(launch_tile_gather(dev_img, H, W, C, border, dev_origins, count, P, divisor, dev_patches, (hipStream_t)stream));
    return DSEN2_OK;
  });
}

int dsen2_recompose(const float* dev_patches, int count, int C, int P, int border, float* dev_img, int H, int W, float scale,
                    void* stream) {
  return guarded([&] { return recompose_rows(dev_patches, count, C, P, border, dev_img, H, W, scale, 0, H, stream); });
}

int dsen2_recompose_rows(const float* dev_patches, int count, int C, int P, int border, float* dev_img, int H, int W, float scale,
                         int row0, int row1, void* stream) {
  return guarded([&] { return recompose_rows(dev_patches, count, C, P, border, dev_img, H, W, scale, row0, row1, stream); });
}

int dsen2_dihedral_nchw(const float* dev_in, float* dev_out, int n, int c, int h, int w, int op, const int* dev_ops, int inverse,
                        void* stream) {
  return guarded([&]() -> int {
    size_t elems = 0;
    if (int rc = check_dihedral_args(dev_in, dev_out, n, c, h, w, op, &elems)) return rc;
    if (dev_ops && h != w) return fail(DSEN2_ERR_INVALID, "per-sample ops need square images (an odd rotation swaps H and W), got %dx%d", h, w);
    if (elems == 0) return DSEN2_OK;
    HIP_TRY(launch_dihedral(dev_in, dev_out, n, c, h, w, op, dev_ops, inverse != 0, (hipStream_t)stream));
    return DSEN2_OK;
  });
}

int dsen2_dihedral_accumulate(const float* dev_in, float* dev_acc, int n, int c, int h, int w, int op, int count, void* stream) {
  return guarded([&]() -> int {
    size_t elems = 0;
    if (int rc = check_dihedral_args(dev_in, dev_acc, n, c, h, w, op, &elems)) return rc;
    if (count < 0) return fail(DSEN2_ERR_INVALID, "count %d is negative", count);
    if (elems == 0) return DSEN2_OK;
    HIP_TRY(launch_dihedral_accumulate(dev_in, dev_acc, n, c, h, w, op, count, (hipStream_t)stream));
    return DSEN2_OK;
  });
}

int dsen2_model_ensemble_workspace_bytes(const dsen2_model* m, int n, int h, int w, int mask, size_t* bytes) {
  if (!m || !bytes) return fail(DSEN2_ERR_INVALID, "NULL argument");
  if (int rc = check_ensemble_shape(m, n, h, w, mask)) return rc;
  *bytes = ensemble_ws(m, n, h, w, mask, nullptr).bytes;
  return DSEN2_OK;
}

int dsen2_model_forward_ensemble(dsen2_model* m, const float* dev_x10, const float* dev_x20, const float* dev_x60, float* dev_out,
                                 int n, int h, int w, int mask, void* dev_workspace, size_t workspace_bytes, void* stream) {
  return guarded([&] {
    return forward_ensemble(m, dev_x10, dev_x20, dev_x60, dev_out, n, h, w, mask, dev_workspace, workspace_bytes, stream);
  });
}

}
```

dsen2_amd/csrc/conv3x3_body32.hip:

```cpp
#include <type_traits>

#include "conv3x3_dma.h"

namespace dsen2 {

namespace {

using dma::KC; using dma::NT; using dma::THREADS; using dma::QS; using dma::IN_BYTES; using dma::IN_BLOCKS;
using dma::WCH; using dma::NWBUF; using dma::LDS_BYTES; using dma::wait_vmcnt;
constexpr int KSTEPS = 4;
constexpr int PB = 2, MB = 2;
static_assert((8 * kHalo) % 16 == 0, "rows R and R+8 of a pixel block sit on the same banks");

}

template <int CIN, int COUT, int EPI, int ABL, int PRE, int STG, bool DEFER>
__global__ __launch_bounds__(THREADS, 2) void conv3x3_body32_kernel(const ConvParams p, const int n_items) {
  constexpr int NCC = CIN / KC;
  constexpr int NS = COUT / NT;
  static_assert(NCC % 2 == 0, "input double buffer parity");
  constexpr bool ASYM = STG >= 2;
  using Stage = dma::Stage<CIN, NS, false, ASYM ? dma::Role::Issuer : dma::Role::All>;
  constexpr int N_W = (ABL & 4) ? 0 : Stage::N_W;

  extern __shared__ __attribute__((aligned(16))) float smem[];
  float* const in_s = smem;
  float* const w_s = smem + 2 * IN_BYTES / 4;
  float* const bias_s = w_s + NWBUF * WCH;

  const int tid = threadIdx.x;
  const int lane = tid & 63;
  const int wave = __builtin_amdgcn_readfirstlane(tid >> 6);
  const int wn = wave & 1;
  const int wp = wave >> 1;
  const int l31 = lane & 31;
  const int hsel = lane >> 5;
  const int rh = l31 >> 4, c16 = l31 & 15;

  const int G = gridDim.x;
  const int lid = xcd_contiguous_id(blockIdx.x, G);
  if (lid >= n_items) return;
  const int my_items = (n_items - lid + G - 1) / G;
  const int tiles_per_img = p.tiles_x * p.tiles_y;
  const size_t img_pix = (size_t)p.h * p.w;

  Stage st;
  st.init(p, in_s, w_s, lane, wave, lid, G, n_items);

  const int x_lane = (hsel * QS + (2 * wp + 8 * rh) * kHalo + c16) * 4;
  const int w_lane = (hsel * NT + wn * 64 + l31) * 4;

  if (!ASYM || wave < 4) {
    st.set_stage_item(lid);
    if constexpr (!(ABL & 8)) {
#pragma unroll
      for (int b = 0; b < IN_BLOCKS; ++b) st.issue_in(0, b, 0);
    }
    if constexpr (!(ABL & 4)) {
      st.issue_w();
      st.issue_w();
      st.issue_w();
    }
  }
  if (tid < COUT) bias_s[tid] = p.bias[tid];
  wait_vmcnt<0>();
  __syncthreads();

  f32x4 w_cur[MB], x_cur[PB], w_nxt[MB], x_nxt[PB];
  int mf_slot = 0;
  auto read_frags = [&](f32x4 (&wf)[MB], f32x4 (&xf)[PB], const float* ib, const float* wb, int tap, int s) {
    const int dy = tap / 3, dx = tap - dy * 3;
    const float* wp_ = wb + w_lane + (2 * s * NT) * 4;
    const float* xp_ = ib + x_lane + (2 * s * QS + dy * kHalo + dx) * 4;
#pragma unroll
    for (int mb = 0; mb < MB; ++mb) wf[mb] = *reinterpret_cast<const f32x4*>(wp_ + mb * 32 * 4);
#pragma unroll
    for (int pb = 0; pb < PB; ++pb) xf[pb] = *reinterpret_cast<const f32x4*>(xp_ + pb * kHalo * 4);
  };
  read_frags(w_cur, x_cur, in_s, w_s, 0, 0);

  struct OutGeom { int img; unsigned lane_eoff; int ey; bool col_ok; int chb; };
  auto out_geom = [&](int item, bool valid) -> OutGeom {
    const Tile t = tile_at<NS>(item, tiles_per_img, p.tiles_x);
    const int chb = t.slab * NT + wn * 64 + 4 * hsel;
    const int ex = t.tx0 + c16, ey = t.ty0 + 2 * wp + 8 * rh;
    return OutGeom{t.img, (unsigned)((ey * p.w + ex) * COUT + chb), ey, valid && ex < p.w, chb};
  };
  auto aux_desc = [&](int img) {
    return __builtin_amdgcn_make_buffer_rsrc(
        const_cast<float*>(p.aux) + (EPI == kEpiResidual ? (size_t)img * img_pix * COUT : 0), 0,
        EPI == kEpiResidual ? (unsigned)(img_pix * COUT * 4) : 0, 0x00020000);
  };
  auto byte_off = [&](const OutGeom& g_, int mb, int pb, int g) -> unsigned {
    return g_.col_ok && g_.ey + pb < p.h ? (g_.lane_eoff + (unsigned)(pb * p.w * COUT + mb * 32 + 8 * g)) * 4u : 0x80000000u;
  };

  auto run = [&](auto mid_c, auto issue_c) {
  constexpr int MIDS = decltype(mid_c)::value;
  constexpr bool ISSUE = decltype(issue_c)::value;
  f32x16 acc[MB][PB];
#pragma unroll
  for (int mb = 0; mb < MB; ++mb)
#pragma unroll
    for (int pb = 0; pb < PB; ++pb)
#pragma unroll
      for (int e = 0; e < 16; ++e) acc[mb][pb][e] = 0.f;
  constexpr int kPre = EPI == kEpiResidual && !(ABL & 2) && !DEFER ? PRE : 0;
  f32x4 resv[kPre ? kPre : 1][PB][4];
#pragma unroll
  for (int mb = 0; mb < (kPre ? kPre : 1); ++mb)
#pragma unroll
    for (int pb = 0; pb < PB; ++pb)
#pragma unroll
      for (int g = 0; g < 4; ++g) resv[mb][pb][g] = f32x4{0.f, 0.f, 0.f, 0.f};

  f32x16 held[DEFER ? MB : 1][DEFER ? PB : 1];
  f32x4 rq[DEFER && EPI == kEpiResidual ? 4 : 1];
  for (int it = 0; it <= my_items; ++it) {
    const OutGeom g_ = out_geom(it > 0 ? lid + (it - 1) * G : lid, it > 0);
    const auto aux_rsrc = aux_desc(g_.img);
    const auto out_rsrc = __builtin_amdgcn_make_buffer_rsrc(
        p.out + (size_t)g_.img * img_pix * COUT, 0, (unsigned)(img_pix * COUT * 4), 0x00020000);
    auto load_res = [&](int j) -> f32x4 {
      const int mb = j >> 3, pb = (j >> 2) & 1, g = j & 3;
      return __builtin_bit_cast(f32x4, __builtin_amdgcn_raw_buffer_load_b128(aux_rsrc, byte_off(g_, mb, pb, g), 0, 0));
    };
    auto finish = [&](int j, const f32x16& a, f32x4 rr) {
      const int mb = j >> 3, pb = (j >> 2) & 1, g = j & 3;
      const f32x4 bias = *reinterpret_cast<const f32x4*>(bias_s + g_.chb + mb * 32 + 8 * g);
      f32x4 v = {a[4 * g], a[4 * g + 1], a[4 * g + 2], a[4 * g + 3]};
      v = v + bias;
      if constexpr (EPI == kEpiRelu) {
#pragma unroll
        for (int e = 0; e < 4; ++e) v[e] = fmaxf(v[e], 0.f);
      } else {
        v = rr + v * p.res_scale;
      }
      if constexpr (!(ABL & 1))
        __builtin_amdgcn_raw_buffer_store_b128(__builtin_bit_cast(u32x4, v), out_rsrc, byte_off(g_, mb, pb, g), 0, 0);
      else
        asm volatile("" ::"v"(v));
    };
    constexpr bool kRes = EPI == kEpiResidual && !(ABL & 2);
    if constexpr (!DEFER) {
#pragma unroll
      for (int j = 0; j < 16; ++j) {
        const int mb = j >> 3, pb = (j >> 2) & 1, g = j & 3;
        f32x4 rr = {1.f, 1.f, 1.f, 1.f};
        if constexpr (kRes) rr = mb < kPre ? resv[mb][pb][g] : load_res(j);
        finish(j, acc[mb][pb], rr);
      }
    } else {
#pragma unroll
      for (int mb = 0; mb < MB; ++mb)
#pragma unroll
        for (int pb = 0; pb < PB; ++pb) held[mb][pb] = acc[mb][pb];
      if (it == my_items) {
#pragma unroll
        for (int j = 0; j < 16; ++j) {
          f32x4 rr = {1.f, 1.f, 1.f, 1.f};
          if constexpr (kRes) rr = load_res(j);
          finish(j, held[j >> 3][(j >> 2) & 1], rr);
        }
      } else if constexpr (kRes) {
        rq[0] = load_res(0);
        rq[1] = load_res(1);
      }
    }
    if (it == my_items) break;
    const int item = lid + it * G;
    const bool have_next_item = it + 1 < my_items;
#pragma unroll
    for (int mb = 0; mb < MB; ++mb)
#pragma unroll
      for (int pb = 0; pb < PB; ++pb)
#pragma unroll
        for (int e = 0; e < 16; ++e) acc[mb][pb][e] = 0.f;

    auto do_cc = [&](const int cc, auto first_c) {
      constexpr bool kFirst = decltype(first_c)::value;
      (void)kFirst;
      const float* const ib = in_s + (cc & 1) * (IN_BYTES / 4);
      const float* const ib_next = in_s + ((cc + 1) & 1) * (IN_BYTES / 4);
      const bool last_cc = cc == NCC - 1;
      const int in_cc = last_cc ? 0 : cc + 1;
      if constexpr (ISSUE) {
        if (last_cc && have_next_item) st.set_stage_item(item + G);
      }
#pragma unroll
      for (int tap = 0; tap < 9; ++tap) {
        const float* const wb = w_s + mf_slot * WCH;
        const int nx_slot = mf_slot == NWBUF - 1 ? 0 : mf_slot + 1;
        const float* const wb_nx = w_s + nx_slot * WCH;
        constexpr int kNoIn = (ABL & 8) ? 1 : 0;
        const int n_in = (tap < IN_BLOCKS && !kNoIn) ? Stage::N_IN : 0;

#pragma unroll
        for (int s = 0; s < KSTEPS; ++s) {
          if (s < KSTEPS - 1) {
            read_frags(w_nxt, x_nxt, ib, wb, tap, s + 1);
          } else if (tap < 8) {
            read_frags(w_nxt, x_nxt, ib, wb_nx, tap + 1, 0);
          } else {
            read_frags(w_nxt, x_nxt, ib_next, wb_nx, 0, 0);
          }
          if constexpr (DEFER) {
            if (kFirst && tap < 8) {
              if (s == MIDS && kRes && tap < 7) {
                rq[2 * ((tap + 1) & 1)] = load_res(2 * tap + 2);
                rq[2 * ((tap + 1) & 1) + 1] = load_res(2 * tap + 3);
              }
            }
          }
          if constexpr (ISSUE) {
            if (s == MIDS) {
              if (n_in) st.issue_in((cc + 1) & 1, tap < IN_BLOCKS ? tap : 0, in_cc);
              if constexpr (!(ABL & 4)) st.issue_w();
            }
          }
          if constexpr (DEFER) {
            if (kFirst && tap < 8 && (s == 1 || s == 3)) {
              const int j = 2 * tap + (s >> 1);
              f32x4 rr = {1.f, 1.f, 1.f, 1.f};
              if constexpr (kRes) rr = rq[2 * (tap & 1) + (s >> 1)];
              finish(j, held[j >> 3][(j >> 2) & 1], rr);
            }
          }
          if constexpr (kPre > 0 && !DEFER) {
            if (tap == 8 && last_cc && s == (MIDS < KSTEPS - 1 ? MIDS + 1 : MIDS)) {
              const OutGeom g_ = out_geom(item, true);
              const auto aux_rsrc = aux_desc(g_.img);
#pragma unroll
              for (int mb = 0; mb < kPre; ++mb)
#pragma unroll
                for (int pb = 0; pb < PB; ++pb)
#pragma unroll
                  for (int g = 0; g < 4; ++g)
                    resv[mb][pb][g] = __builtin_bit_cast(f32x4, __builtin_amdgcn_raw_buffer_load_b128(
                                                                    aux_rsrc, byte_off(g_, mb, pb, g), 0, 0));
            }
          }
          __builtin_amdgcn_sched_barrier(0);
#pragma unroll
          for (int j = 0; j < 4; ++j)
#pragma unroll
            for (int mb = 0; mb < MB; ++mb)
#pragma unroll
              for (int pb = 0; pb < PB; ++pb)
                acc[mb][pb] = __builtin_amdgcn_mfma_f32_32x32x2f32(w_cur[mb][j], x_cur[pb][j], acc[mb][pb], 0, 0, 0);
#pragma unroll
          for (int q = 0; q < MB; ++q) w_cur[q] = w_nxt[q];
#pragma unroll
          for (int q = 0; q < PB; ++q) x_cur[q] = x_nxt[q];
        }
        mf_slot = nx_slot;
        __builtin_amdgcn_sched_barrier(0);
        if constexpr (ISSUE) {
          if (n_in) wait_vmcnt<N_W + Stage::N_IN>(); else wait_vmcnt<N_W>();
        }
        if constexpr (!(ABL & 16)) __syncthreads();
      }
    };
    do_cc(0, std::true_type{});
#pragma unroll 1
    for (int cc = 1; cc < NCC; ++cc) do_cc(cc, std::false_type{});
  }
  };
  if constexpr (ASYM) {
    if (wave < 4) {
      run(std::integral_constant<int, (STG - 2) % KSTEPS>{}, std::true_type{});
    } else {
      if constexpr ((STG - 2) / KSTEPS == 1) __builtin_amdgcn_s_setprio(1);
      run(std::integral_constant<int, 0>{}, std::false_type{});
    }
  } else if constexpr (STG == 1) {
    if (wave < 4)
      run(std::integral_constant<int, 0>{}, std::true_type{});
    else
      run(std::integral_constant<int, KSTEPS / 2>{}, std::true_type{});
  } else {
    run(std::integral_constant<int, 0>{}, std::true_type{});
  }
  wait_vmcnt<0>();
}

template <int CIN, int COUT, int EPI, int ABL = 0, int PRE = 0, int STG = 0, bool DEFER = false>
static hipError_t launch_body32_one(const ConvParams& p, hipStream_t stream) {
  const long long items = (long long)p.n * p.tiles_x * p.tiles_y * (COUT / NT);
  return launch_persistent<conv3x3_body32_kernel<CIN, COUT, EPI, ABL, PRE, STG, DEFER>>(LDS_BYTES, THREADS, items, 1, 0, stream, p);
}

constexpr int kAsym = 2 + KSTEPS / 2;

template <int F>
static hipError_t launch_body32_feat(const ConvParams& p, int epilogue, Body32Form form, hipStream_t stream) {
  const bool relu = epilogue == kEpiRelu;
#ifdef DSEN2_DIAG
  if (form == Body32Form::Plain || form == Body32Form::StaggerA) {
    if (!relu) return launch_body32_one<F, F, kEpiResidual, 0, 2, 0>(p, stream);
    return form == Body32Form::Plain ? launch_body32_one<F, F, kEpiRelu, 0, 0, 0>(p, stream) : launch_body32_one<F, F, kEpiRelu, 0, 0, 1>(p, stream);
  }
  if (form == Body32Form::DeferStaggerA && !relu) return launch_body32_one<F, F, kEpiResidual, 0, 0, 0, true>(p, stream);
  if (form == Body32Form::DeferStagger || form == Body32Form::DeferStaggerA)
    return relu ? launch_body32_one<F, F, kEpiRelu, 0, 0, 1, true>(p, stream) : launch_body32_one<F, F, kEpiResidual, 0, 0, 1, true>(p, stream);
#define DSEN2_ASYM(FORM, STG)                                                                                      \
  if (form == Body32Form::FORM)                                                                                    \
    return relu ? launch_body32_one<F, F, kEpiRelu, 0, 0, STG, true>(p, stream) : launch_body32_one<F, F, kEpiResidual, 0, 0, STG, true>(p, stream);
  DSEN2_ASYM(DeferAsymS0, 2) DSEN2_ASYM(DeferAsymS1, 3) DSEN2_ASYM(DeferAsymS3, 5) DSEN2_ASYM(DeferAsymPrio, 8)
#undef DSEN2_ASYM
#else
  if (form != Body32Form::DeferAsym) return hipErrorInvalidValue;
#endif
  return relu ? launch_body32_one<F, F, kEpiRelu, 0, 0, kAsym, true>(p, stream) : launch_body32_one<F, F, kEpiResidual, 0, 0, kAsym, true>(p, stream);
}

hipError_t launch_conv3x3_body32(const ConvParams& p, int feat, int epilogue, Body32Form form, int ablate, hipStream_t stream) {
  if ((size_t)p.h * p.w * feat * 4 >= 0x80000000ull) return hipErrorNotSupported;
#ifdef DSEN2_DIAG
  if (feat == 128 && ablate != 0) {
#define DSEN2_ABL_ASYM(M)                                                                                \
  if (ablate == M && form == Body32Form::DeferAsym)                                                      \
    return epilogue == kEpiRelu ? launch_body32_one<128, 128, kEpiRelu, M, 0, kAsym, true>(p, stream)    \
                                : launch_body32_one<128, 128, kEpiResidual, M, 0, kAsym, true>(p, stream);
    DSEN2_ABL_ASYM(3) DSEN2_ABL_ASYM(15) DSEN2_ABL_ASYM(16)
#undef DSEN2_ABL_ASYM
#define DSEN2_ABL(M)                                                                             \
  if (ablate == M)                                                                               \
    return epilogue == kEpiRelu ? launch_body32_one<128, 128, kEpiRelu, M>(p, stream)            \
                                : launch_body32_one<128, 128, kEpiResidual, M, 2>(p, stream);
    DSEN2_ABL(1) DSEN2_ABL(2) DSEN2_ABL(3) DSEN2_ABL(4) DSEN2_ABL(8) DSEN2_ABL(12) DSEN2_ABL(15) DSEN2_ABL(16) DSEN2_ABL(31)
#undef DSEN2_ABL
    return hipErrorInvalidValue;
  }
#endif
  if (ablate != 0) return hipErrorInvalidValue;
  if (feat == 128) return launch_body32_feat<128>(p, epilogue, form, stream);
  if (feat == 256) return launch_body32_feat<256>(p, epilogue, form, stream);
  return hipErrorInvalidValue;
}

}
```

dsen2_amd/csrc/conv3x3_dma.h:

```cpp
#pragma once
#include "conv3x3_items.h"

namespace dsen2 {
namespace dma {

constexpr int KC = 32;
constexpr int NT = 128;
constexpr int THREADS = 512;
constexpr int QS = 336;
constexpr int IN_BYTES = 8 * QS * 16;
constexpr int IN_BLOCKS = 6;
constexpr int WCH = KC * NT;
constexpr int NWBUF = 4;
constexpr size_t LDS_BYTES = (size_t)2 * IN_BYTES + (size_t)NWBUF * WCH * 4 + 256 * 4;
static_assert(QS >= kHaloPix && QS % 16 == 0 && 64 * (IN_BLOCKS - 1) + 16 == QS, "input chunk geometry");
static_assert(LDS_BYTES <= 160 * 1024, "LDS budget");

template <int N>
__device__ __forceinline__ void wait_vmcnt() {
  static_assert(N >= 0 && N <= 63, "vmcnt is a 6-bit field");
  asm volatile("s_waitcnt vmcnt(%0)" ::"n"(N) : "memory");
}

__device__ __forceinline__ unsigned lds_address(const float* p) {
  return (unsigned)(size_t)(__attribute__((address_space(3))) const float*)p;
}

enum class Role { All, Issuer };

template <int CINW, int NS, bool LAZY_VOFF = false, Role ROLE = Role::All>
struct Stage {
  static constexpr int N_W = ROLE == Role::Issuer ? 4 : 2;
  static constexpr int N_IN = ROLE == Role::Issuer ? 2 : 1;
  static constexpr int NCC = CINW / KC;
  static constexpr int NCHUNK = NCC * 9;

  const float* in;
  int h, w, tiles_x, tiles_per_img;
  size_t img_pix;
  int lane, wave, lid, G, n_items;
  unsigned lds_in, lds_w;
  unsigned in_voff[LAZY_VOFF ? 1 : IN_BLOCKS];
  int st_y0, st_x0;
  __amdgpu_buffer_rsrc_t in_rsrc, w_rsrc;
  unsigned w_voff;
  int wl_item, wl_chunk, st_slot;

  __device__ __forceinline__ void init(const ConvParams& p, const float* in_s, const float* w_s, int lane_, int wave_,
                                       int lid_, int G_, int n_items_) {
    in = p.in; h = p.h; w = p.w; tiles_x = p.tiles_x; tiles_per_img = p.tiles_x * p.tiles_y;
    img_pix = (size_t)p.h * p.w;
    lane = lane_; wave = wave_; lid = lid_; G = G_; n_items = n_items_;
    lds_in = lds_address(in_s);
    lds_w = lds_address(w_s);
    in_rsrc = __builtin_amdgcn_make_buffer_rsrc(const_cast<float*>(p.in), 0, 0, 0x00020000);
    w_rsrc = __builtin_amdgcn_make_buffer_rsrc(const_cast<float*>(p.wpk), 0, (unsigned)(NS * NCHUNK * WCH * 4), 0x00020000);
    w_voff = lane * 16;
    wl_item = lid; wl_chunk = 0; st_slot = 0;
    st_y0 = st_x0 = 0;
  }

  __device__ __forceinline__ unsigned voff_of(int b, int ty0, int tx0) const {
    const int hp = 64 * b + lane;
    const int hy = hp / kHalo, hx = hp - hy * kHalo;
    const int gy = ty0 - 1 + hy, gx = tx0 - 1 + hx;
    const bool inb = hp < kHaloPix && (unsigned)gy < (unsigned)h && (unsigned)gx < (unsigned)w;
    return inb ? (unsigned)(((gy * w + gx) * CINW + wave * 4) * 4) : 0x80000000u;
  }

  __device__ __forceinline__ void set_stage_item(int item) {
    const Tile t = tile_at<NS>(item, tiles_per_img, tiles_x);
    in_rsrc = __builtin_amdgcn_make_buffer_rsrc(const_cast<float*>(in) + (size_t)t.img * img_pix * CINW, 0,
                                                (unsigned)(img_pix * CINW * 4), 0x00020000);
    if constexpr (LAZY_VOFF) {
      st_y0 = t.ty0;
      st_x0 = t.tx0;
    } else {
#pragma unroll
      for (int b = 0; b < IN_BLOCKS; ++b) in_voff[b] = voff_of(b, t.ty0, t.tx0);
    }
  }

  __device__ __forceinline__ void issue_in(int buf, int b, int cc) {
    const unsigned m0v = lds_in + buf * IN_BYTES + (wave * QS + 64 * b) * 16;
    const unsigned so = cc * (KC * 4);
    const unsigned voff = LAZY_VOFF ? voff_of(b, st_y0, st_x0) : in_voff[LAZY_VOFF ? 0 : b];
    if constexpr (ROLE == Role::Issuer) {
      const unsigned m1v = m0v + 4 * QS * 16, so1 = so + 64;
      unsigned saved_m0;
      if (b < IN_BLOCKS - 1) {
        asm volatile("s_mov_b32 %0, m0\n\t"
                     "s_mov_b32 m0, %1\n\ts_nop 0\n\tbuffer_load_dwordx4 %3, %4, %5 offen lds\n\t"
                     "s_mov_b32 m0, %2\n\ts_nop 0\n\tbuffer_load_dwordx4 %3, %4, %6 offen lds\n\t"
                     "s_mov_b32 m0, %0"
                     : "=&s"(saved_m0) : "s"(m0v), "s"(m1v), "v"(voff), "s"(in_rsrc), "s"(so), "s"(so1) : "memory");
      } else if (lane < 16) {
        asm volatile("s_mov_b32 %0, m0\n\t"
                     "s_mov_b32 m0, %1\n\ts_nop 0\n\tbuffer_load_dwordx4 %3, %4, %5 offen lds\n\t"
                     "s_mov_b32 m0, %2\n\ts_nop 0\n\tbuffer_load_dwordx4 %3, %4, %6 offen lds\n\t"
                     "s_mov_b32 m0, %0"
                     : "=&s"(saved_m0) : "s"(m0v), "s"(m1v), "v"(voff), "s"(in_rsrc), "s"(so), "s"(so1) : "memory");
      }
      return;
    }
    unsigned saved_m0;
    if (b < IN_BLOCKS - 1) {
      asm volatile("s_mov_b32 %0, m0\n\ts_mov_b32 m0, %1\n\ts_nop 0\n\tbuffer_load_dwordx4 %2, %3, %4 offen lds\n\ts_mov_b32 m0, %0"
                   : "=&s"(saved_m0) : "s"(m0v), "v"(voff), "s"(in_rsrc), "s"(so) : "memory");
    } else if (lane < 16) {
      asm volatile("s_mov_b32 %0, m0\n\ts_mov_b32 m0, %1\n\ts_nop 0\n\tbuffer_load_dwordx4 %2, %3, %4 offen lds\n\ts_mov_b32 m0, %0"
                   : "=&s"(saved_m0) : "s"(m0v), "v"(voff), "s"(in_rsrc), "s"(so) : "memory");
    }
  }

  __device__ __forceinline__ void issue_w() {
    const unsigned so = (unsigned)(((wl_item % NS) * NCHUNK + wl_chunk) * (WCH * 4) + wave * 1024);
    const unsigned l0 = lds_w + st_slot * (WCH * 4) + wave * 1024;
    unsigned saved_m0;
    if constexpr (ROLE == Role::Issuer)
      asm volatile(
          "s_mov_b32 %0, m0\n\t"
          "s_mov_b32 m0, %1\n\ts_nop 0\n\tbuffer_load_dwordx4 %5, %6, %7 offen lds\n\t"
          "s_mov_b32 m0, %2\n\ts_nop 0\n\tbuffer_load_dwordx4 %5, %6, %8 offen lds\n\t"
          "s_mov_b32 m0, %3\n\ts_nop 0\n\tbuffer_load_dwordx4 %5, %6, %9 offen lds\n\t"
          "s_mov_b32 m0, %4\n\ts_nop 0\n\tbuffer_load_dwordx4 %5, %6, %10 offen lds\n\t"
          "s_mov_b32 m0, %0"
          : "=&s"(saved_m0)
          : "s"(l0), "s"(l0 + 4096u), "s"(l0 + 8192u), "s"(l0 + 12288u), "v"(w_voff), "s"(w_rsrc), "s"(so), "s"(so + 4096u),
            "s"(so + 8192u), "s"(so + 12288u)
          : "memory");
    else
    asm volatile(
        "s_mov_b32 %0, m0\n\t"
        "s_mov_b32 m0, %1\n\ts_nop 0\n\tbuffer_load_dwordx4 %3, %4, %5 offen lds\n\t"
        "s_mov_b32 m0, %2\n\ts_nop 0\n\tbuffer_load_dwordx4 %3, %4, %6 offen lds\n\t"
        "s_mov_b32 m0, %0"
        : "=&s"(saved_m0) : "s"(l0), "s"(l0 + 8192u), "v"(w_voff), "s"(w_rsrc), "s"(so), "s"(so + 8192u)
        : "memory");
    if (++wl_chunk == NCHUNK) {
      wl_chunk = 0;
      wl_item = wl_item + G < n_items ? wl_item + G : lid;
    }
    st_slot = st_slot == NWBUF - 1 ? 0 : st_slot + 1;
  }
};

}
}
```

dsen2_amd/csrc/conv_plan.hip:

```cpp
#include <cstring>
#include <vector>

#include "conv_plan.h"

namespace dsen2 {

namespace {

constexpr int kBody16Chunk = 32;

bool sentinel2(const BandGroups* b) { return b && b->c10 == 4 && b->c20 == 6 && (b->c60 == 0 || b->c60 == 2); }

void pack_tile_weights(const float* k, const ConvPlan& pl, float* dst) {
  const int ncc = pl.cin_pad / pl.kc, nslab = pl.cout_pad / pl.nt, ng = pl.kc / 4;
  size_t i = 0;
  for (int slab = 0; slab < nslab; ++slab)
    for (int cc = 0; cc < ncc; ++cc)
      for (int tap = 0; tap < 9; ++tap)
        for (int gg = 0; gg < ng; ++gg)
          for (int o = 0; o < pl.nt; ++o)
            for (int j = 0; j < 4; ++j, ++i) {
              const int c = cc * pl.kc + 4 * gg + j, oc = slab * pl.nt + o;
              dst[i] = (c < pl.cin && oc < pl.cout) ? k[((size_t)tap * pl.cin + c) * pl.cout + oc] : 0.f;
            }
}

void pack_conv_weights_bf16_host(const float* k, int cin, int cout, uint16_t* dst) {
  const int ncc = cin / kBody16Chunk, nslab = cout / 128, ng = kBody16Chunk / 8;
  size_t i = 0;
  for (int slab = 0; slab < nslab; ++slab)
    for (int cc = 0; cc < ncc; ++cc)
      for (int step = 0; step < 9; ++step) {
        const int tap = (step % 3) * 3 + step / 3;
        for (int g = 0; g < ng; ++g)
          for (int o = 0; o < 128; ++o)
            for (int j = 0; j < 8; ++j, ++i) {
              const int ch = 32 * (o >> 5) + 8 * ((o & 15) >> 2) + 4 * ((o >> 4) & 1) + (o & 3);
              const int c = cc * kBody16Chunk + 8 * g + j, oc = slab * 128 + ch;
              dst[i] = f32_to_bf16_rne(k[((size_t)tap * cin + c) * cout + oc]);
            }
      }
}

void pack_conv_weights_bf16x3_host(const float* k, int cin, int cout, uint16_t* dst) {
  const int vcin = 3 * cin;
  std::vector<float> v((size_t)9 * vcin * cout);
  for (int tap = 0; tap < 9; ++tap)
    for (int c = 0; c < cin; ++c)
      for (int o = 0; o < cout; ++o) {
        const float w = k[((size_t)tap * cin + c) * cout + o];
        const uint32_t hu = (uint32_t)f32_to_bf16_rne(w) << 16;
        float wh;
        memcpy(&wh, &hu, 4);
        const float wl = w - wh;
        const int cc = c / kBody16Chunk, j = c % kBody16Chunk;
        float* base = v.data() + ((size_t)tap * vcin + (size_t)cc * 3 * kBody16Chunk + j) * cout + o;
        base[0] = wh;
        base[(size_t)kBody16Chunk * cout] = wl;
        base[(size_t)2 * kBody16Chunk * cout] = wh;
      }
  pack_conv_weights_bf16_host(v.data(), vcin, cout, dst);
}

size_t tap_floats(const ConvPlan& pl) { return (size_t)9 * pl.cin_pad * pl.cout_pad; }

}

bool plan_conv(ConvRole role, int cin, int cout, int precision, const Tuning& tune, const BandGroups* bands, ConvPlan* plan) {
  if (cin <= 0 || cout <= 0 || precision < 0 || precision > 2) return false;
  ConvPlan& pl = *plan;
  pl = ConvPlan{};
  pl.role = role; pl.cin = cin; pl.cout = cout; pl.body32 = tune.body32;
  const bool feat_out = cout == 128 || cout == 256;
  switch (role) {
    case ConvRole::Output:
      if (cout > 32 || (cin != 128 && cin != 256)) return false;
      pl.epilogue = kEpiSkipNCHW; pl.cin_pad = cin;
      pl.kernel = ConvKernel::Tile; pl.kc = 32; pl.nt = 32; pl.cout_pad = 32;
      if (cout <= 8 && tune.out != OutKernel::Tile) {
        pl.kernel = ConvKernel::Out; pl.kc = pl.nt = 0; pl.cout_pad = 8; pl.out_mfma = tune.out == OutKernel::MfmaThenValu;
      }
      break;
    case ConvRole::First:
    case ConvRole::DgradOutput:
      if (!feat_out || cin > 16) return false;
      pl.kernel = ConvKernel::Tile; pl.kc = 16; pl.nt = 128; pl.cin_pad = 16; pl.cout_pad = cout;
      pl.epilogue = kEpiResidual;
      if (role == ConvRole::DgradOutput) break;
      pl.epilogue = precision == 1 ? kEpiReluSplit : kEpiRelu;
      if (tune.first == FirstKernel::Direct && (cin == 10 || cin == 12)) pl.real_channels = cin;
      pl.first_direct = precision == 0 && tune.first == FirstKernel::Direct && sentinel2(bands);
      if (precision != 0 && sentinel2(bands)) pl.first16_planes = precision;
      break;
    case ConvRole::BodyA:
    case ConvRole::BodyB:
    case ConvRole::DgradBody:
      if (!feat_out || cin != cout) return false;
      pl.epilogue = role == ConvRole::BodyA ? kEpiRelu : kEpiResidual;
      pl.cin_pad = cin; pl.cout_pad = cout; pl.kc = 32; pl.nt = 128;
      pl.kernel = precision == 1   ? ConvKernel::Body16
                  : precision == 2 ? ConvKernel::Body16x3
                  : tune.body == BodyKernel::Body32 ? ConvKernel::Body32 : ConvKernel::Tile;
      break;
  }
  const size_t taps = tap_floats(pl);
  pl.weight_floats = pl.kernel == ConvKernel::Body16     ? taps / 2
                     : pl.kernel == ConvKernel::Body16x3 ? 3 * taps / 2
                                                         : taps + (pl.out_mfma ? out_mfma_weight_floats(cin) : 0);
  pl.bias_off = align_up(pl.weight_floats);
  pl.floats = pl.first16_off = pl.bias_off + align_up((size_t)pl.cout_pad);
  if (pl.first16_planes) pl.floats += align_up((first16_weight_u16(cout, pl.first16_planes == 2) + 1) / 2);
  return true;
}

void pack(const ConvPlan& pl, const float* k, const float* bias, float* dst) {
  memset(dst, 0, sizeof(float) * (bias ? pl.floats : pl.weight_floats));
  switch (pl.kernel) {
    case ConvKernel::Tile:
    case ConvKernel::Body32: pack_tile_weights(k, pl, dst); break;
    case ConvKernel::Body16: pack_conv_weights_bf16_host(k, pl.cin, pl.cout, reinterpret_cast<uint16_t*>(dst)); break;
    case ConvKernel::Body16x3: pack_conv_weights_bf16x3_host(k, pl.cin, pl.cout, reinterpret_cast<uint16_t*>(dst)); break;
    case ConvKernel::Out:
      pack_out_valu_weights_host(k, pl.cin, pl.cout, dst);
      if (pl.out_mfma) pack_out_mfma_weights_host(k, pl.cin, pl.cout, dst + tap_floats(pl));
      break;
  }
  if (!bias) return;
  memcpy(dst + pl.bias_off, bias, sizeof(float) * pl.cout);
  if (pl.first16_planes)
    pack_first16_weights_host(k, pl.cin, pl.cout, pl.first16_planes == 2, reinterpret_cast<uint16_t*>(dst + pl.first16_off));
}

hipError_t launch(const ConvPlan& pl, const ConvParams& p, int epilogue, const Tuning& t, hipStream_t stream) {
  switch (pl.kernel) {
    case ConvKernel::Out: {
      ConvParams pm = p;
      pm.wpk += tap_floats(pl);
      bool done = false;
      const hipError_t e = pl.out_mfma ? try_launch(launch_conv3x3_out_mfma(pm, pl.cin_pad, stream, t.out_ablate), &done) : hipSuccess;
      return e != hipSuccess || done ? e : launch_conv3x3_out_valu(p, pl.cin_pad, stream);
    }
    case ConvKernel::Body32: return launch_conv3x3_body32(p, pl.cin_pad, epilogue, pl.body32, t.ablate, stream);
    case ConvKernel::Body16: return launch_conv3x3_body16w(p, pl.cin_pad, epilogue, false, t.ablate & 1023, stream, t.grid_cap);
    case ConvKernel::Body16x3: return launch_conv3x3_body16w(p, pl.cin_pad, epilogue, true, 0, stream);
    case ConvKernel::Tile: {
      const int mask = pl.role == ConvRole::Output ? t.out_ablate : pl.cin_pad == pl.cout_pad ? t.ablate : 0;
      if (mask != 0) return hipErrorInvalidValue;
      return launch_conv3x3_tile(p, pl.cin_pad, pl.cout_pad, epilogue, pl.real_channels, stream);
    }
  }
  return hipErrorInvalidValue;
}

bool plan_network(int c10, int c20, int c60, int num_layers, int feat, int precision, const Tuning& tune, NetworkPlan* net) {
  const BandGroups bands{c10, c20, c60};
  *net = NetworkPlan{};
  auto add = [&](ConvRole role, int ci, int co, int prec) {
    Layer L;
    if (!plan_conv(role, ci, co, prec, tune, &bands, &L.plan)) return false;
    L.flat_off = net->n_params;
    net->n_params += (size_t)9 * ci * co + co;
    L.off = net->dev_param_floats;
    net->dev_param_floats += L.plan.floats;
    net->layers.push_back(L);
    return true;
  };
  if (!add(ConvRole::First, c10 + c20 + c60, feat, num_layers > 0 ? precision : 0)) return false;
  for (int i = 0; i < num_layers; ++i)
    if (!add(ConvRole::BodyA, feat, feat, precision) || !add(ConvRole::BodyB, feat, feat, precision)) return false;
  if (!add(ConvRole::Output, feat, c60 > 0 ? c60 : c20, 0)) return false;
  if (num_layers > 0 && precision != 0) net->chain_stride = net->layers[1].plan.floats * sizeof(float);
  return true;
}

}
```

dsen2_amd/csrc/dsen2_internal.h:

```cpp
#pragma once
#include <hip/hip_runtime.h>
#include <stddef.h>
#include <stdint.h>

#include <mutex>

namespace dsen2 {


constexpr int kTile = 16;
constexpr int kHalo = kTile + 2;
constexpr int kHaloPix = kHalo * kHalo;

enum Epilogue : int {
  kEpiRelu = 0, kEpiResidual = 1, kEpiSkipNCHW = 2,
  kEpiResidualF32 = 3,
  kEpiReluSplit = 4
};

struct ConvParams {
  const float* in;
  const float* wpk;
  const float* bias;
  const float* aux;
  float* out;
  void* out2;
  int n, h, w;
  int tiles_x, tiles_y;
  int cout_real;
  float res_scale;
  unsigned long long* diag;
};

enum class FirstKernel { Direct, Tile16 };
enum class BodyKernel { Body32, Tile };
enum class Body32Form { StaggerA, Plain, DeferStaggerA, DeferStagger, DeferAsym, DeferAsymS0, DeferAsymS1, DeferAsymS3, DeferAsymPrio };
enum class OutKernel { MfmaThenValu, Valu, Tile };
struct Tuning {
  FirstKernel first = FirstKernel::Direct;
  BodyKernel body = BodyKernel::Body32;
  Body32Form body32 = Body32Form::DeferAsym;
  OutKernel out = OutKernel::MfmaThenValu;
  int ablate = 0;
  int grid_cap = 0;
  int first_ablate = 0;
  int out_ablate = 0;
  int chain = 1;
  static Tuning reference() { Tuning t; t.first = FirstKernel::Tile16; t.body = BodyKernel::Tile; t.out = OutKernel::Tile; return t; }
};

struct KernelOnce {
  std::mutex mu;
  bool done[64] = {};
  int cus[64] = {};
  hipError_t prepare(const void* kern, size_t lds_bytes, int* dev_cus) {
    int dev = 0;
    hipError_t e = hipGetDevice(&dev);
    if (e != hipSuccess) return e;
    if (dev < 0 || dev >= 64) return hipErrorInvalidDevice;
    std::lock_guard<std::mutex> lock(mu);
    if (!done[dev]) {
      if (lds_bytes > 0) {
        e = hipFuncSetAttribute(kern, hipFuncAttributeMaxDynamicSharedMemorySize, (int)lds_bytes);
        if (e != hipSuccess) return e;
      }
      e = hipDeviceGetAttribute(&cus[dev], hipDeviceAttributeMultiprocessorCount, dev);
      if (e != hipSuccess) return e;
      done[dev] = true;
    }
    if (dev_cus) *dev_cus = cus[dev];
    return hipSuccess;
  }
};

hipError_t launch_conv3x3_tile(const ConvParams& p, int cin_pad, int cout_pad, int epilogue, int real_channels, hipStream_t stream);
hipError_t launch_conv3x3_out_valu(const ConvParams& p, int feat, hipStream_t stream);
void pack_out_valu_weights_host(const float* kernel_hwio, int cin, int cout, float* dst);
hipError_t launch_conv3x3_out_mfma(const ConvParams& p, int feat, hipStream_t stream, int ablate = 0);
size_t out_mfma_weight_floats(int cin);
void pack_out_mfma_weights_host(const float* kernel_hwio, int cin, int cout, float* dst);
struct FirstInputs { const float* x60; int c10, c20, c60; };
hipError_t launch_conv3x3_first(const ConvParams& p, const FirstInputs& f, int cout, int epilogue, hipStream_t stream, int ablate = 0);
hipError_t launch_conv3x3_first16(const ConvParams& p, const FirstInputs& f, int cout, bool x3, hipStream_t stream);
size_t first16_weight_u16(int cout, bool x3);
void pack_first16_weights_host(const float* kernel_hwio, int cin, int cout, bool x3, uint16_t* dst);
hipError_t launch_conv3x3_body32(const ConvParams& p, int feat, int epilogue, Body32Form form, int ablate, hipStream_t stream);
hipError_t launch_conv3x3_body16w(const ConvParams& p, int feat, int epilogue, bool x3, int ablate, hipStream_t stream, int grid_cap = 0);
hipError_t launch_split3_f32(const float* in_nhwc, void* hx, void* lo, int n, int h, int w, int c, hipStream_t stream);
struct ChainArgs {
  void* hi;
  void* lo;
  void* t;
  float* out_f32;
  unsigned layer_stride;
  int n_layers;
  int patches_per_wg;
  int seamless;
};
hipError_t launch_conv3x3_body16w_chain(const ConvParams& p, const ChainArgs& c, int feat, hipStream_t stream, int ablate = 0,
                                        bool x3 = false);
int body16w_chain_patches_per_wg(int n, int h, int w, int feat, int cus);
hipError_t launch_split_f32(const float* in_nhwc, void* hi, void* lo, int n, int h, int w, int c, hipStream_t stream);
hipError_t launch_join_f32(const void* hi, const void* lo, float* out_nhwc, int n, int h, int w, int c, hipStream_t stream);
inline uint16_t f32_to_bf16_rne(float f) {
  uint32_t u = __builtin_bit_cast(uint32_t, f);
  if ((u & 0x7fffffffu) > 0x7f800000u) return (uint16_t)((u >> 16) | 0x40);
  u += 0x7fffu + ((u >> 16) & 1u);
  return (uint16_t)(u >> 16);
}

hipError_t launch_pack_inputs(const float* x10, const float* x20, const float* x60, int c10, int c20, int c60,
                              float* out_nhwc16, int n, int h, int w, hipStream_t stream);
hipError_t launch_upsample(const float* in, float* out, int planes, int h, int w, int oh, int ow, float post_div,
                           hipStream_t stream, bool general = false);
hipError_t launch_tile_gather(const float* img, int H, int W, int C, int border, const int* origins, int count,
                              int P, float divisor, float* patches, hipStream_t stream);
hipError_t launch_recompose(const float* patches, int count, int C, int P, int border, float* img, int H, int W,
                            float scale, int row0, int row1, hipStream_t stream);

hipError_t launch_dihedral(const float* in, float* out, int n, int c, int ih, int iw, int op, const int* dev_ops, bool inverse,
                           hipStream_t stream);
hipError_t launch_dihedral_accumulate(const float* in, float* acc, int n, int c, int h, int w, int op, int count, hipStream_t stream);
__host__ __device__ __forceinline__ int dihedral_bits(int op) {
  return (int)(0x72416350u >> (4 * (op & 7))) & 7;
}

struct CorpusTileDev {
  const float *lr10, *lr20, *lr60;
  const void* gt;
  int eh, ew, gt_u16, pad_;
};
hipError_t launch_corpus_batch(const CorpusTileDev* dev_tiles, int n_tiles, bool run_60, const int* dev_samples, int n, float divisor,
                               float* x10, float* x20, float* x60, float* y, hipStream_t stream);

size_t wgrad_workspace_floats(int n, int h, int w, int ca, int cg);
bool wgrad_geometry(int n, int h, int w, int ca, int cg, long long* tiles, int* splits);
hipError_t launch_conv3x3_wgrad(const float* a, int ca, const float* g, int cg, int n, int h, int w, int ci_real, int co_real,
                                float scale, float* dw, float* db, float* ws, size_t ws_floats, hipStream_t stream);
size_t wgrad16_workspace_floats(int n, int h, int w, int feat);
bool wgrad16_geometry(int n, int h, int w, int feat, long long* tiles, int* splits);
hipError_t launch_conv3x3_wgrad16(const void* a_planes, const void* g_planes, int n, int h, int w, int feat, float scale, float* dw,
                                  float* db, float* ws, size_t ws_floats, hipStream_t stream);
hipError_t launch_conv3x3_wgrad16_bf16(const void* a, const void* g, int n, int h, int w, int feat, float scale, float* dw, float* db,
                                       float* ws, size_t ws_floats, hipStream_t stream);
enum { kLossMae = 0, kLossMse = 1, kLossHuber = 2, kLossCharbonnier = 3, kLossKinds = 4 };
enum { kMaskNone = 0, kMaskNoData = 1, kMaskModes = 2 };
size_t loss_partial_doubles(size_t pixels);
constexpr int kSsimLossMinWin = 3, kSsimLossMaxWin = 11;
struct SsimLossTerm {
  float weight = 0.f;
  int win = 0;
  double w[kSsimLossMaxWin] = {};
  double c1 = 0.0, c2 = 0.0;
};
size_t ssim_loss_work_doubles();
hipError_t launch_ssim_loss(const float* out, const float* y, int n, int c, int h, int w, const SsimLossTerm& term, int mask, float* gpad,
                            double* work, bool three, hipStream_t stream);
hipError_t launch_loss_grad(const float* out, const float* y, float* gpad, double* partial, float* loss2, int n, int c, int h, int w,
                            int kind, float param, int mask, hipStream_t stream, const SsimLossTerm* ssim = nullptr,
                            double* ssim_work = nullptr);
hipError_t launch_relu_mask(float* v, const float* m, size_t count, hipStream_t stream);
hipError_t launch_join3_f32(const void* hx, const void* lo, float* out_nhwc, int n, int h, int w, int c, hipStream_t stream);
hipError_t launch_mask_split3(const float* v_nhwc, const void* t_planes, void* du_planes, int n, int h, int w, int c, hipStream_t stream);
hipError_t launch_mask_round16(const float* v_nhwc, const void* t_plane, void* du_plane, int n, int h, int w, int c, hipStream_t stream);
hipError_t launch_nadam(float* p, const float* g, float* m, float* v, size_t count, float lr, float b1, float b2, float eps,
                        float mc_t, float mc_t1, float ms_new, float ms_next, float b2_pow_t, hipStream_t stream);
constexpr int kMaxShards = 64;
struct ShardCounts {
  int n[kMaxShards];
};
hipError_t launch_nadam_shards(float* p, const float* g_shards, size_t shard_stride, int shards, const ShardCounts& counts, float* g_mean,
                               float* m, float* v, size_t count, float lr, float b1, float b2, float eps, float mc_t, float mc_t1,
                               float ms_new, float ms_next, float b2_pow_t, hipStream_t stream);
hipError_t launch_gather(float* dst, const float* src, const int* map, size_t n, hipStream_t stream);
hipError_t launch_scatter(float* flat, const float* packed, const int* map, size_t n, hipStream_t stream);
enum : int { kGatherHi = 0, kGatherLo = 1, kGatherF32Low = 2, kGatherF32High = 3 };
hipError_t launch_gather16(void* dst, const float* src, const int* map, size_t words, int layers, size_t dst_stride, size_t src_stride,
                           hipStream_t stream);

}
```

include/dsen2_hip.h:

```cpp
#ifndef DSEN2_HIP_H
#define DSEN2_HIP_H

#include <stddef.h>

#ifdef __cplusplus
extern "C" {
#endif

#define DSEN2_OK 0
#define DSEN2_ERR_INVALID (-1)
#define DSEN2_ERR_HIP (-2)
#define DSEN2_ERR_NO_WEIGHTS (-3)
#define DSEN2_ERR_WORKSPACE (-4)
#define DSEN2_ERR_NO_DEVICE (-5)
#define DSEN2_ERR_NOMEM (-6)
#define DSEN2_ERR_INTERNAL (-7)

typedef struct dsen2_model dsen2_model;

const char *dsen2_version(void);
const char *dsen2_last_error(void);
int dsen2_device_count(void);

int dsen2_model_create(dsen2_model **out, int c10, int c20, int c60, int num_layers, int feature_size,
                       int precision);
void dsen2_model_destroy(dsen2_model *m);

size_t dsen2_model_num_params(const dsen2_model *m);

int dsen2_model_load_weights(dsen2_model *m, const float *host_flat, size_t count);

int dsen2_model_workspace_bytes(const dsen2_model *m, int n, int h, int w, size_t *bytes);

int dsen2_model_forward(dsen2_model *m, const float *dev_x10, const float *dev_x20, const float *dev_x60,
                        float *dev_out, int n, int h, int w, void *dev_workspace, size_t workspace_bytes,
                        void *stream);

int dsen2_model_body_launches(const dsen2_model *m, int n, int h, int w);

int dsen2_model_forward_timed(dsen2_model *m, const float *x10, const float *x20, const float *x60, float *out,
                              int n, int h, int w, void *workspace, size_t workspace_bytes, void *stream, int iters,
                              float *body_ms_per_launch);

int dsen2_model_forward_profile(dsen2_model *m, const float *x10, const float *x20, const float *x60, float *out,
                                int n, int h, int w, void *workspace, size_t workspace_bytes, void *stream, int warm,
                                int iters, float *ms5);

int dsen2_dihedral_nchw(const float *dev_in, float *dev_out, int n, int c, int h, int w, int op, const int *dev_ops_or_null,
                        int inverse, void *stream);
int dsen2_dihedral_accumulate(const float *dev_in, float *dev_acc, int n, int c, int h, int w, int op, int count_or_0,
                              void *stream);
int dsen2_model_ensemble_workspace_bytes(const dsen2_model *m, int n, int h, int w, int mask, size_t *bytes);
int dsen2_model_forward_ensemble(dsen2_model *m, const float *dev_x10, const float *dev_x20, const float *dev_x60,
                                 float *dev_out, int n, int h, int w, int mask, void *dev_workspace, size_t workspace_bytes,
                                 void *stream);

int dsen2_conv3x3_nhwc(const float *dev_in, const float *host_kernel, const float *host_bias,
                       const float *dev_aux, float *dev_out, int n, int h, int w, int cin, int cout,
                       int epilogue, float res_scale, void *stream);

int dsen2_conv3x3_nhwc_ref(const float *dev_in, const float *host_kernel, const float *host_bias,
                           const float *dev_aux, float *dev_out, int n, int h, int w, int cin, int cout,
                           int epilogue, float res_scale, void *stream);

int dsen2_split_f32(const float *dev_in_nhwc, void *dev_hi, void *dev_lo, int n, int h, int w, int c, void *stream);
int dsen2_join_f32(const void *dev_hi, const void *dev_lo, float *dev_out_nhwc, int n, int h, int w, int c, void *stream);

int dsen2_conv3x3_body_bf16(const void *dev_in_bf16, const float *host_kernel, const float *host_bias,
                            void *dev_res_hi, void *dev_res_lo, void *dev_out, int n, int h, int w, int feat,
                            int epilogue, float res_scale, void *stream);

int dsen2_split3_f32(const float *dev_in_nhwc, void *dev_hx, void *dev_lo, int n, int h, int w, int c, void *stream);
int dsen2_conv3x3_body_bf16x3(const void *dev_in_planes, const float *host_kernel, const float *host_bias,
                              void *dev_res_hx, void *dev_res_lo, void *dev_out, int n, int h, int w, int feat,
                              int epilogue, float res_scale, void *stream);

int dsen2_conv3x3_first_planes(const float *dev_x10, const float *dev_x20, const float *dev_x60, int c10, int c20, int c60,
                               const float *host_kernel, const float *host_bias, int feat, int precision,
                               void *dev_out, void *dev_out2, int n, int h, int w, void *stream);

int dsen2_model_time_body_conv(dsen2_model *m, int layer, const float *dev_in, const float *dev_aux,
                               float *dev_out, int n, int h, int w, int iters, void *stream,
                               float *ms_per_launch);

int dsen2_model_train_workspace_bytes(const dsen2_model *m, int n, int h, int w, size_t *bytes);
int dsen2_model_gradients(dsen2_model *m, const float *x10, const float *x20, const float *x60, const float *target,
                          float *dev_out_or_NULL, float *dev_grad_flat, float *dev_loss2, int n, int h, int w, void *ws,
                          size_t ws_bytes, void *stream);
int dsen2_model_set_train_precision(dsen2_model *m, int precision);
int dsen2_model_get_weights(const dsen2_model *m, float *dev_flat, void *stream);
int dsen2_model_set_weights_device(dsen2_model *m, const float *dev_flat, void *stream);
int dsen2_nadam_step(float *p, const float *g, float *m, float *v, size_t count, float lr, float b1, float b2, float eps,
                     float mc_t, float mc_t1, float ms_new, float ms_next, float b2_pow_t, void *stream);
int dsen2_nadam_step_shards(float *p, const float *dev_g_shards, size_t shard_stride, int shards, const int *host_counts,
                            float *dev_g_mean_or_NULL, float *m, float *v, size_t count, float lr, float b1, float b2, float eps,
                            float mc_t, float mc_t1, float ms_new, float ms_next, float b2_pow_t, void *stream);
int dsen2_conv3x3_wgrad(const float *dev_a, const float *dev_g, float *dev_dw, float *dev_db, int n, int h, int w, int ca,
                        int cg, int ci, int co, float scale, void *stream);
int dsen2_conv3x3_wgrad_bf16x3(const void *dev_a_planes, const void *dev_g_planes, float *dev_dw, float *dev_db, int n, int h,
                               int w, int feat, float scale, void *stream);
int dsen2_conv3x3_wgrad_bf16(const void *dev_a, const void *dev_g, float *dev_dw, float *dev_db, int n, int h, int w, int feat,
                             float scale, void *stream);
int dsen2_conv3x3_wgrad_geometry(int kind, int n, int h, int w, int ca, int cg, long long *tiles, int *splits,
                                 size_t *workspace_floats);
int dsen2_join3_f32(const void *dev_hx, const void *dev_lo16, float *dev_out_nhwc, int n, int h, int w, int c, void *stream);

int dsen2_model_set_loss(dsen2_model *m, int kind, float param, int mask_mode);
int dsen2_loss_grad(const float *dev_out, const float *dev_target, int n, int c, int h, int w, int kind, float param,
                    int mask_mode, float *dev_g_nhwc16, float *dev_loss2, void *stream);
int dsen2_loss_sums_workspace_bytes(size_t *bytes);
int dsen2_loss_sums(const float *dev_pred, const float *dev_target, int n, int c, long long hw, int kind, float param,
                    int mask_mode, void *dev_work, size_t work_bytes, double *dev_out3, void *stream);

int dsen2_model_set_loss_ssim(dsen2_model *m, float weight, const double *host_window, int win, double c1, double c2);
int dsen2_ssim_loss_grad(const float *dev_out, const float *dev_target, int n, int c, int h, int w, float weight,
                         const double *host_window, int win, double c1, double c2, int mask_mode, float *dev_g_nhwc16,
                         double *dev_sums2, void *stream);
int dsen2_ssim_loss_sums_workspace_bytes(size_t *bytes);
int dsen2_ssim_loss_sums(const float *dev_pred, const float *dev_target, int n, int c, int h, int w, const double *host_window,
                         int win, double c1, double c2, int mask_mode, void *dev_work, size_t work_bytes, double *dev_out3,
                         void *stream);

int dsen2_upsample_mirror_bilinear(const float *dev_in, float *dev_out, int planes, int h, int w, int oh,
                                   int ow, float post_divisor, void *stream);
int dsen2_upsample_mirror_bilinear_ref(const float *dev_in, float *dev_out, int planes, int h, int w, int oh,
                                       int ow, float post_divisor, void *stream);

int dsen2_tile_gather(const float *dev_img, int H, int W, int C, int border, const int *dev_origins,
                      int count, int P, float divisor, float *dev_patches, void *stream);

int dsen2_recompose(const float *dev_patches, int count, int C, int P, int border, float *dev_img, int H,
                    int W, float scale, void *stream);
int dsen2_recompose_rows(const float *dev_patches, int count, int C, int P, int border, float *dev_img, int H,
                         int W, float scale, int row0, int row1, void *stream);

int dsen2_tile_nodata_geometry(int H, int W, int P, int border, int *x_tiles, int *y_tiles, size_t *bitmap_words);
int dsen2_tile_nodata(const float *dev_img10, int H, int W, int C10, int P, int border, unsigned char *dev_patch_empty,
                      unsigned int *dev_valid_bits, void *stream);
int dsen2_recompose_rows_nodata(const float *dev_patches, int slots, int C, int P, int border, const int *dev_slot_of_patch,
                                const unsigned int *dev_valid_bits, float *dev_img, int H, int W, float scale, int row0, int row1,
                                void *stream);

int dsen2_recompose_rows_blend(const float *dev_patches, int count_or_slots, int C, int P, int border, int feather,
                               const int *dev_slot_of_patch, const unsigned int *dev_valid_bits, float *dev_img, int H, int W,
                               float scale, int row0, int row1, void *stream);

#define DSEN2_DTYPE_U16 0
#define DSEN2_DTYPE_F32 1
int dsen2_down_pixel_aggr(const void *dev_img, int dtype, int H, int W, int C, int scale, const double *host_weights,
                          int radius, void *dev_out, int out_f64, void *stream);

typedef struct dsen2_corpus dsen2_corpus;
typedef struct dsen2_corpus_tile {
  const float *dev_lr10, *dev_lr20, *dev_lr60;
  const void *dev_gt;
  int grid_h, grid_w;
  int gt_dtype;
} dsen2_corpus_tile;
int dsen2_corpus_create(const dsen2_corpus_tile *host_tiles, int n_tiles, int run_60, dsen2_corpus **out);
void dsen2_corpus_destroy(dsen2_corpus *corpus);
int dsen2_corpus_batch(const dsen2_corpus *corpus, const int *host_samples, const int *dev_samples, int n, float divisor,
                       float *dev_x10, float *dev_x20, float *dev_x60_or_null, float *dev_y, void *stream);

#define DSEN2_MASK_BLANK_MAP 3
int dsen2_corpus_origin_mask(const void *dev_src, int dtype, int H, int W, int C, int grid_h, int grid_w, const int *host_holdout,
                             const int *dev_holdout, int m, int margin, unsigned char *dev_cells, unsigned char *dev_bitmap,
                             int *dev_count, void *stream);

int dsen2_class_valid_bits(const unsigned char *dev_cls, int Hs, int Ws, const unsigned char *host_lut256, int up, int down, int H,
                           int W, int dilate, const unsigned int *dev_and_bits_or_null, unsigned int *dev_valid_bits, void *stream);
int dsen2_tile_flags_from_bits(const unsigned int *dev_valid_bits, int H, int W, int P, int border, unsigned char *dev_patch_empty,
                               void *stream);
int dsen2_raster_apply_valid(void *dev_img, int dtype, int H, int W, int C, const unsigned int *dev_valid_bits, void *stream);
int dsen2_cells_from_valid_bits(const unsigned int *dev_valid_bits, int H, int W, int S, int accumulate, unsigned char *dev_cells,
                                void *stream);

int dsen2_abs_sq_error_sums_workspace_bytes(size_t *bytes);
int dsen2_abs_sq_error_sums(const float *dev_pred, const float *dev_target, long long count, void *dev_work, size_t work_bytes,
                            double *dev_out, void *stream);

#define DSEN2_DTYPE_F64 2
int dsen2_imresize_axis(const void *dev_in, int dtype, int H, int W, int C, int axis, int out_len, const double *dev_weights,
                        const int *dev_indices, int taps, double *dev_out, void *stream);

int dsen2_band_errors_workspace_bytes(int C, size_t *bytes);
int dsen2_band_errors(const void *dev_x, int x_dtype, const void *dev_gt, int gt_dtype, int H, int W, int C, void *dev_work,
                      size_t work_bytes, double *dev_out, void *stream);
int dsen2_imresize_band_errors(const void *dev_in, int dtype, int H, int W, int C, int axis, int out_len, const double *dev_weights,
                               const int *dev_indices, int taps, const void *dev_gt, int gt_dtype, void *dev_work,
                               size_t work_bytes, double *dev_out, void *stream);

int dsen2_quality_workspace_bytes(int C, size_t *bytes);
int dsen2_uiq_map(const void *dev_x, int x_dtype, const void *dev_y, int y_dtype, int H, int W, int C, int block,
                  double *dev_map_f64, void *stream);
int dsen2_uiq_sums(const void *dev_x, int x_dtype, const void *dev_y, int y_dtype, int H, int W, int C, int block, void *dev_work,
                   size_t work_bytes, double *dev_out, void *stream);
int dsen2_sam_sums(const void *dev_x, int x_dtype, const void *dev_y, int y_dtype, int H, int W, int C, void *dev_work,
                   size_t work_bytes, double *dev_out, void *stream);
int dsen2_imresize_uiq_sums(const void *dev_in, int dtype, int H, int W, int C, int axis, int out_len, const double *dev_weights,
                            const int *dev_indices, int taps, const void *dev_gt, int gt_dtype, int block, void *dev_work,
                            size_t work_bytes, double *dev_out, void *stream);
int dsen2_imresize_sam_sums(const void *dev_in, int dtype, int H, int W, int C, int axis, int out_len, const double *dev_weights,
                            const int *dev_indices, int taps, const void *dev_gt, int gt_dtype, void *dev_work, size_t work_bytes,
                            double *dev_out, void *stream);

int dsen2_ssim_map(const void *dev_x, int x_dtype, const void *dev_y, int y_dtype, int H, int W, int C, const double *host_window,
                   int win, double c1, double c2, double *dev_map_f64, void *stream);
int dsen2_ssim_sums(const void *dev_x, int x_dtype, const void *dev_y, int y_dtype, int H, int W, int C, const double *host_window,
                    int win, double c1, double c2, void *dev_work, size_t work_bytes, double *dev_out, void *stream);
int dsen2_imresize_ssim_sums(const void *dev_in, int dtype, int H, int W, int C, int axis, int out_len, const double *dev_weights,
                             const int *dev_indices, int taps, const void *dev_gt, int gt_dtype, const double *host_window, int win,
                             double c1, double c2, void *dev_work, size_t work_bytes, double *dev_out, void *stream);

#ifdef __cplusplus
}
#endif
#endif
```

Before: 40570 patches/s.

## Add 8x32 row-tile body32 conv form with wave-uniform border MFMA skipping

Adds a row-tile geometry for the fp32 body conv kernel: each tile covers 8 rows by 32 columns instead of 16x16. Each wave now owns one 32-channel weight block and four pixel rows. The new form skips the MFMA blocks for padded border rows and out-of-range rows, using a wave-uniform scalar branch in inline asm. It becomes the default whenever it needs no more tiles than the 16x16 form, which holds for 32x32 patches. The wider halo row (34 vs 18) cuts the halo overhead per output pixel and lets weight fragments be reused across four pixel blocks. The cost is more inline asm with manual hazard nops and a larger input staging buffer.

```diff
diff --git a/dsen2_amd/DSen2Net.py b/dsen2_amd/DSen2Net.py
--- a/dsen2_amd/DSen2Net.py
+++ b/dsen2_amd/DSen2Net.py
@@ -961,6 +961,12 @@
     return tiles.value, splits.value, floats.value
 
 
+def conv3x3_body32_geometry(h, w):
+    row, tx, ty = ctypes.c_int(0), ctypes.c_int(0), ctypes.c_int(0)
+    _lib.call('dsen2_conv3x3_body32_geometry', int(h), int(w), ctypes.byref(row), ctypes.byref(tx), ctypes.byref(ty))
+    return bool(row.value), tx.value, ty.value
+
+
 def conv3x3_first_planes(xs, kernel_hwio, bias, precision):
     kernel_hwio = np.ascontiguousarray(kernel_hwio, np.float32)
     bias = np.ascontiguousarray(bias, np.float32)
diff --git a/dsen2_amd/_lib.py b/dsen2_amd/_lib.py
--- a/dsen2_amd/_lib.py
+++ b/dsen2_amd/_lib.py
@@ -77,6 +77,7 @@
                                          c_void_p]),
     'dsen2_conv3x3_wgrad_geometry': (c_int, [c_int, c_int, c_int, c_int, c_int, c_int, ctypes.POINTER(ctypes.c_longlong), c_int_p,
                                              ctypes.POINTER(c_size_t)]),
+    'dsen2_conv3x3_body32_geometry': (c_int, [c_int, c_int, c_int_p, c_int_p, c_int_p]),
     'dsen2_join3_f32': (c_int, [c_void_p, c_void_p, c_void_p, c_int, c_int, c_int, c_int, c_void_p]),
     'dsen2_upsample_mirror_bilinear': (c_int, [c_void_p, c_void_p, c_int, c_int, c_int, c_int, c_int, ctypes.c_float,
                                                c_void_p]),
diff --git a/dsen2_amd/asm_contract.py b/dsen2_amd/asm_contract.py
--- a/dsen2_amd/asm_contract.py
+++ b/dsen2_amd/asm_contract.py
@@ -122,6 +122,16 @@
             copies = [body[mf[0]:mf[ITEM_MFMAS - 1]], body[mf[ITEM_MFMAS]:mf[-1]]]
             n_dma = [sum(1 for ln in c if ln.startswith('buffer_load_dword') and ln.endswith('lds')) for c in copies]
             need(min(n_dma) == 0 and max(n_dma) > 0, 'kernel %s: DMAs in both copies of the item loop' % name, n_dma)
+            row = re.search(r'ELb1ELi([12])EEE', name)
+            if row:
+                for c in copies:
+                    runs = re.findall(r'(?:M(\d+);)(?:M\1;){3}', ''.join(
+                        'M%s;' % re.match(r'v_mfma\S+ v\[(\d+):', ln).group(1) if ln.startswith('v_mfma') else '' for ln in c + ['v_mfma_x v[0:15]']))
+                    need(len(runs) >= ITEM_MFMAS // 4 - 1, 'kernel %s: MFMAs of a pixel block are not four in a row on one accumulator' % name)
+                if row.group(1) == '2':
+                    for c in copies:
+                        need(sum(1 for ln in c if ln.startswith('s_cbranch_scc1 .Lskip_block')) == ITEM_MFMAS // 4 - 1,
+                             'kernel %s: not one wave-uniform branch around every pixel block' % name)
             quiet, loud = (copies[0], copies[1]) if n_dma[0] == 0 else (copies[1], copies[0])
             need(not any(re.search(r'\bm0\b', ln) for ln in quiet), 'kernel %s: M0 use in the compute-only copy' % name)
             run = None
@@ -135,6 +145,10 @@
                 elif run and not re.match(r'(s_mov_b32 m0, |s_nop 0$)', ln):
                     need(run in (2, 4), 'kernel %s: a DMA statement of %d instructions' % (name, run))
                     run = None
+        rows = [k for k in asym if re.search(r'ELi4ELb1ELi2EEE', k)]
+        squares = [k for k in asym if re.search(r'ELi4ELb1ELi0EEE', k)]
+        need(len(rows) >= 4 and len(squares) >= 4, 'expected the row-tile and the 16 x 16 form for two widths and two epilogues',
+             [len(rows), len(squares)])
     if src == 'conv3x3_body16w.hip':
         expect = {0: (0, 32), 1: (64, 64), 3: (64, 64)}
         expect3 = {0: (0, 64), 1: (64, 96), 3: (64, 64)}
@@ -214,10 +228,10 @@
 
 
 TRAFFIC_KERNELS = {
-    'dsen2_20_fp32': ('conv3x3_body32.hip', r'conv3x3_body32_kernelILi128ELi128ELi0ELi0ELi0ELi4ELb1E'),
+    'dsen2_20_fp32': ('conv3x3_body32.hip', r'conv3x3_body32_kernelILi128ELi128ELi0ELi0ELi0ELi4ELb1ELi2E'),
     'vdsen2_20_bf16': ('conv3x3_body16w.hip', r'conv3x3_body16w_chain_kernelILi128ELi256ELi0E'),
     'dsen2_20_bf16x3': ('conv3x3_body16w.hip', r'conv3x3_body16w_x3_chain_kernelILi64ELi128E'),
-    'vdsen2_20_fp32': ('conv3x3_body32.hip', r'conv3x3_body32_kernelILi256ELi256ELi0ELi0ELi0ELi4ELb1E'),
+    'vdsen2_20_fp32': ('conv3x3_body32.hip', r'conv3x3_body32_kernelILi256ELi256ELi0ELi0ELi0ELi4ELb1ELi2E'),
     'dsen2_20_bf16': ('conv3x3_body16w.hip', r'conv3x3_body16w_chain_kernelILi64ELi128ELi0E'),
     'vdsen2_20_bf16x3': ('conv3x3_body16w.hip', r'conv3x3_body16w_x3_chain_kernelILi128ELi256E'),
 }
diff --git a/dsen2_amd/csrc/capi.hip b/dsen2_amd/csrc/capi.hip
--- a/dsen2_amd/csrc/capi.hip
+++ b/dsen2_amd/csrc/capi.hip
@@ -423,10 +423,10 @@
   Tuning& t = g_diag_tuning;
   switch (key) {
     case 0:
-      if (value != 0 && (value < 11 || value > 19)) return fail(DSEN2_ERR_INVALID, "body variant %d unknown", value);
+      if (value != 0 && (value < 11 || value > 21)) return fail(DSEN2_ERR_INVALID, "body variant %d unknown", value);
       t.first = value == 0 ? FirstKernel::Tile16 : FirstKernel::Direct;
       t.body = value == 0 ? BodyKernel::Tile : BodyKernel::Body32;
-      t.body32 = value == 0 ? Body32Form::DeferAsym : static_cast<Body32Form>(value - 11);
+      t.body32 = value == 0 ? Tuning().body32 : static_cast<Body32Form>(value - 11);
       return DSEN2_OK;
     case 2:
       if (value != 0 && value != 2 && value != 3) return fail(DSEN2_ERR_INVALID, "output variant %d unknown", value);
@@ -445,6 +445,13 @@
   return DSEN2_OK;
 }
 #endif
+
+int dsen2_conv3x3_body32_geometry(int h, int w, int* row_tiles, int* tiles_x, int* tiles_y) {
+  if (!row_tiles || !tiles_x || !tiles_y) return fail(DSEN2_ERR_INVALID, "NULL argument");
+  if (h <= 0 || w <= 0) return fail(DSEN2_ERR_INVALID, "bad shape h=%d w=%d", h, w);
+  *row_tiles = body32_form_at(Tuning().body32, h, w, tiles_x, tiles_y) == Body32Form::RowTile;
+  return DSEN2_OK;
+}
 
 int dsen2_device_count(void) {
   int n = 0;
diff --git a/dsen2_amd/csrc/conv3x3_body32.hip b/dsen2_amd/csrc/conv3x3_body32.hip
--- a/dsen2_amd/csrc/conv3x3_body32.hip
+++ b/dsen2_amd/csrc/conv3x3_body32.hip
@@ -6,21 +6,44 @@
 
 namespace {
 
-using dma::KC; using dma::NT; using dma::THREADS; using dma::QS; using dma::IN_BYTES; using dma::IN_BLOCKS;
-using dma::WCH; using dma::NWBUF; using dma::LDS_BYTES; using dma::wait_vmcnt;
+using dma::KC; using dma::NT; using dma::THREADS; using dma::IN_BLOCKS;
+using dma::WCH; using dma::NWBUF; using dma::wait_vmcnt;
 constexpr int KSTEPS = 4;
-constexpr int PB = 2, MB = 2;
 static_assert((8 * kHalo) % 16 == 0, "rows R and R+8 of a pixel block sit on the same banks");
 
-}
-
-template <int CIN, int COUT, int EPI, int ABL, int PRE, int STG, bool DEFER>
+template <int BIT>
+__device__ __forceinline__ void mfma_block_unless(f32x16& acc, const f32x4& w, const f32x4& x, unsigned mask) {
+  asm volatile(
+      "s_bitcmp1_b32 %9, %10\n\t"
+      "s_cbranch_scc1 .Lskip_block_%=\n\t"
+      "s_nop 1\n\t"
+      "v_mfma_f32_32x32x2_f32 %0, %1, %5, %0\n\t"
+      "v_mfma_f32_32x32x2_f32 %0, %2, %6, %0\n\t"
+      "v_mfma_f32_32x32x2_f32 %0, %3, %7, %0\n\t"
+      "v_mfma_f32_32x32x2_f32 %0, %4, %8, %0\n"
+      ".Lskip_block_%=:"
+      : "+v"(acc)
+      : "v"(w[0]), "v"(w[1]), "v"(w[2]), "v"(w[3]), "v"(x[0]), "v"(x[1]), "v"(x[2]), "v"(x[3]), "s"(mask), "n"(BIT)
+      : "scc");
+}
+__device__ __forceinline__ void mfma_results_fence(f32x16& a, f32x16& b, f32x16& c, f32x16& d) {
+  asm volatile("s_nop 15\n\ts_nop 3" : "+v"(a), "+v"(b), "+v"(c), "+v"(d));
+}
+
+}
+
+template <int CIN, int COUT, int EPI, int ABL, int PRE, int STG, bool DEFER, int ROW>
 __global__ __launch_bounds__(THREADS, 2) void conv3x3_body32_kernel(const ConvParams p, const int n_items) {
   constexpr int NCC = CIN / KC;
   constexpr int NS = COUT / NT;
   static_assert(NCC % 2 == 0, "input double buffer parity");
   constexpr bool ASYM = STG >= 2;
-  using Stage = dma::Stage<CIN, NS, false, ASYM ? dma::Role::Issuer : dma::Role::All>;
+  constexpr bool ROWT = ROW != 0;
+  static_assert(!ROWT || (ASYM && DEFER && PRE == 0), "the row-tile forms exist with the deferred epilogue and waves 0-3 as issuers only");
+  using Geo = dma::Geom<ROWT>;
+  constexpr int QS = Geo::QS, IN_BYTES = Geo::IN_BYTES, HW = Geo::HW;
+  constexpr int MB = ROWT ? 1 : 2, PB = ROWT ? 4 : 2;
+  using Stage = dma::Stage<CIN, NS, false, ASYM ? dma::Role::Issuer : dma::Role::All, ROWT>;
   constexpr int N_W = (ABL & 4) ? 0 : Stage::N_W;
 
   extern __shared__ __attribute__((aligned(16))) float smem[];
@@ -31,11 +54,11 @@
   const int tid = threadIdx.x;
   const int lane = tid & 63;
   const int wave = __builtin_amdgcn_readfirstlane(tid >> 6);
-  const int wn = wave & 1;
-  const int wp = wave >> 1;
+  const int wn = ROWT ? wave & 3 : wave & 1;
+  const int wp = ROWT ? wave >> 2 : wave >> 1;
   const int l31 = lane & 31;
   const int hsel = lane >> 5;
-  const int rh = l31 >> 4, c16 = l31 & 15;
+  const int row0 = ROWT ? 4 * wp : 2 * wp + 8 * (l31 >> 4), cx = ROWT ? l31 : l31 & 15;
 
   const int G = gridDim.x;
   const int lid = xcd_contiguous_id(blockIdx.x, G);
@@ -47,8 +70,8 @@
   Stage st;
   st.init(p, in_s, w_s, lane, wave, lid, G, n_items);
 
-  const int x_lane = (hsel * QS + (2 * wp + 8 * rh) * kHalo + c16) * 4;
-  const int w_lane = (hsel * NT + wn * 64 + l31) * 4;
+  const int x_lane = (hsel * QS + row0 * HW + cx) * 4;
+  const int w_lane = (hsel * NT + wn * 32 * MB + l31) * 4;
 
   if (!ASYM || wave < 4) {
     st.set_stage_item(lid);
@@ -71,19 +94,19 @@
   auto read_frags = [&](f32x4 (&wf)[MB], f32x4 (&xf)[PB], const float* ib, const float* wb, int tap, int s) {
     const int dy = tap / 3, dx = tap - dy * 3;
     const float* wp_ = wb + w_lane + (2 * s * NT) * 4;
-    const float* xp_ = ib + x_lane + (2 * s * QS + dy * kHalo + dx) * 4;
+    const float* xp_ = ib + x_lane + (2 * s * QS + dy * HW + dx) * 4;
 #pragma unroll
     for (int mb = 0; mb < MB; ++mb) wf[mb] = *reinterpret_cast<const f32x4*>(wp_ + mb * 32 * 4);
 #pragma unroll
-    for (int pb = 0; pb < PB; ++pb) xf[pb] = *reinterpret_cast<const f32x4*>(xp_ + pb * kHalo * 4);
+    for (int pb = 0; pb < PB; ++pb) xf[pb] = *reinterpret_cast<const f32x4*>(xp_ + pb * HW * 4);
   };
   read_frags(w_cur, x_cur, in_s, w_s, 0, 0);
 
   struct OutGeom { int img; unsigned lane_eoff; int ey; bool col_ok; int chb; };
   auto out_geom = [&](int item, bool valid) -> OutGeom {
-    const Tile t = tile_at<NS>(item, tiles_per_img, p.tiles_x);
-    const int chb = t.slab * NT + wn * 64 + 4 * hsel;
-    const int ex = t.tx0 + c16, ey = t.ty0 + 2 * wp + 8 * rh;
+    const Tile t = tile_at<NS, Geo::TH, Geo::TW>(item, tiles_per_img, p.tiles_x);
+    const int chb = t.slab * NT + wn * 32 * MB + 4 * hsel;
+    const int ex = t.tx0 + cx, ey = t.ty0 + row0;
     return OutGeom{t.img, (unsigned)((ey * p.w + ex) * COUT + chb), ey, valid && ex < p.w, chb};
   };
   auto aux_desc = [&](int img) {
@@ -122,11 +145,11 @@
     const auto out_rsrc = __builtin_amdgcn_make_buffer_rsrc(
         p.out + (size_t)g_.img * img_pix * COUT, 0, (unsigned)(img_pix * COUT * 4), 0x00020000);
     auto load_res = [&](int j) -> f32x4 {
-      const int mb = j >> 3, pb = (j >> 2) & 1, g = j & 3;
+      const int mb = j / (4 * PB), pb = (j >> 2) % PB, g = j & 3;
       return __builtin_bit_cast(f32x4, __builtin_amdgcn_raw_buffer_load_b128(aux_rsrc, byte_off(g_, mb, pb, g), 0, 0));
     };
     auto finish = [&](int j, const f32x16& a, f32x4 rr) {
-      const int mb = j >> 3, pb = (j >> 2) & 1, g = j & 3;
+      const int mb = j / (4 * PB), pb = (j >> 2) % PB, g = j & 3;
       const f32x4 bias = *reinterpret_cast<const f32x4*>(bias_s + g_.chb + mb * 32 + 8 * g);
       f32x4 v = {a[4 * g], a[4 * g + 1], a[4 * g + 2], a[4 * g + 3]};
       v = v + bias;
@@ -145,12 +168,13 @@
     if constexpr (!DEFER) {
 #pragma unroll
       for (int j = 0; j < 16; ++j) {
-        const int mb = j >> 3, pb = (j >> 2) & 1, g = j & 3;
+        const int mb = j / (4 * PB), pb = (j >> 2) % PB, g = j & 3;
         f32x4 rr = {1.f, 1.f, 1.f, 1.f};
         if constexpr (kRes) rr = mb < kPre ? resv[mb][pb][g] : load_res(j);
         finish(j, acc[mb][pb], rr);
       }
     } else {
+      if constexpr (ROW == 2) mfma_results_fence(acc[0][0], acc[0][1], acc[0][PB - 2], acc[0][PB - 1]);
 #pragma unroll
       for (int mb = 0; mb < MB; ++mb)
 #pragma unroll
@@ -160,7 +184,7 @@
         for (int j = 0; j < 16; ++j) {
           f32x4 rr = {1.f, 1.f, 1.f, 1.f};
           if constexpr (kRes) rr = load_res(j);
-          finish(j, held[j >> 3][(j >> 2) & 1], rr);
+          finish(j, held[j / (4 * PB)][(j >> 2) % PB], rr);
         }
       } else if constexpr (kRes) {
         rq[0] = load_res(0);
@@ -170,6 +194,16 @@
     if (it == my_items) break;
     const int item = lid + it * G;
     const bool have_next_item = it + 1 < my_items;
+    unsigned skip = 0;
+    if constexpr (ROW == 2) {
+      const int y0 = tile_at<NS, Geo::TH, Geo::TW>(item, tiles_per_img, p.tiles_x).ty0 + 4 * wp;
+#pragma unroll
+      for (int pb = 0; pb < PB; ++pb) {
+        const int y = y0 + pb;
+        const unsigned out = y >= p.h, top = y == 0, bot = y == p.h - 1;
+        skip |= ((top | out) << pb) | (out << (4 + pb)) | ((bot | out) << (8 + pb));
+      }
+    }
 #pragma unroll
     for (int mb = 0; mb < MB; ++mb)
 #pragma unroll
@@ -223,7 +257,7 @@
               const int j = 2 * tap + (s >> 1);
               f32x4 rr = {1.f, 1.f, 1.f, 1.f};
               if constexpr (kRes) rr = rq[2 * (tap & 1) + (s >> 1)];
-              finish(j, held[j >> 3][(j >> 2) & 1], rr);
+              finish(j, held[j / (4 * PB)][(j >> 2) % PB], rr);
             }
           }
           if constexpr (kPre > 0 && !DEFER) {
@@ -241,6 +275,19 @@
             }
           }
           __builtin_amdgcn_sched_barrier(0);
+          if constexpr (ROW == 2) {
+            const unsigned m = skip >> (4 * (tap / 3));
+            mfma_block_unless<0>(acc[0][0], w_cur[0], x_cur[0], m);
+            mfma_block_unless<1>(acc[0][1], w_cur[0], x_cur[1], m);
+            mfma_block_unless<2>(acc[0][PB - 2], w_cur[0], x_cur[PB - 2], m);
+            mfma_block_unless<3>(acc[0][PB - 1], w_cur[0], x_cur[PB - 1], m);
+          } else if constexpr (ROWT) {
+#pragma unroll
+            for (int pb = 0; pb < PB; ++pb)
+#pragma unroll
+              for (int j = 0; j < 4; ++j)
+                acc[0][pb] = __builtin_amdgcn_mfma_f32_32x32x2f32(w_cur[0][j], x_cur[pb][j], acc[0][pb], 0, 0, 0);
+          } else {
 #pragma unroll
           for (int j = 0; j < 4; ++j)
 #pragma unroll
@@ -248,6 +295,7 @@
 #pragma unroll
               for (int pb = 0; pb < PB; ++pb)
                 acc[mb][pb] = __builtin_amdgcn_mfma_f32_32x32x2f32(w_cur[mb][j], x_cur[pb][j], acc[mb][pb], 0, 0, 0);
+          }
 #pragma unroll
           for (int q = 0; q < MB; ++q) w_cur[q] = w_nxt[q];
 #pragma unroll
@@ -284,10 +332,11 @@
   wait_vmcnt<0>();
 }
 
-template <int CIN, int COUT, int EPI, int ABL = 0, int PRE = 0, int STG = 0, bool DEFER = false>
+template <int CIN, int COUT, int EPI, int ABL = 0, int PRE = 0, int STG = 0, bool DEFER = false, int ROW = 0>
 static hipError_t launch_body32_one(const ConvParams& p, hipStream_t stream) {
   const long long items = (long long)p.n * p.tiles_x * p.tiles_y * (COUT / NT);
-  return launch_persistent<conv3x3_body32_kernel<CIN, COUT, EPI, ABL, PRE, STG, DEFER>>(LDS_BYTES, THREADS, items, 1, 0, stream, p);
+  return launch_persistent<conv3x3_body32_kernel<CIN, COUT, EPI, ABL, PRE, STG, DEFER, ROW>>(dma::Geom<ROW != 0>::LDS_BYTES, THREADS, items,
+                                                                                             1, 0, stream, p);
 }
 
 constexpr int kAsym = 2 + KSTEPS / 2;
@@ -308,14 +357,20 @@
     return relu ? launch_body32_one<F, F, kEpiRelu, 0, 0, STG, true>(p, stream) : launch_body32_one<F, F, kEpiResidual, 0, 0, STG, true>(p, stream);
   DSEN2_ASYM(DeferAsymS0, 2) DSEN2_ASYM(DeferAsymS1, 3) DSEN2_ASYM(DeferAsymS3, 5) DSEN2_ASYM(DeferAsymPrio, 8)
 #undef DSEN2_ASYM
+  if (form == Body32Form::RowTileNoSkip)
+    return relu ? launch_body32_one<F, F, kEpiRelu, 0, 0, kAsym, true, 1>(p, stream) : launch_body32_one<F, F, kEpiResidual, 0, 0, kAsym, true, 1>(p, stream);
 #else
-  if (form != Body32Form::DeferAsym) return hipErrorInvalidValue;
+  if (form != Body32Form::DeferAsym && form != Body32Form::RowTile) return hipErrorInvalidValue;
 #endif
+  if (form == Body32Form::RowTile)
+    return relu ? launch_body32_one<F, F, kEpiRelu, 0, 0, kAsym, true, 2>(p, stream) : launch_body32_one<F, F, kEpiResidual, 0, 0, kAsym, true, 2>(p, stream);
   return relu ? launch_body32_one<F, F, kEpiRelu, 0, 0, kAsym, true>(p, stream) : launch_body32_one<F, F, kEpiResidual, 0, 0, kAsym, true>(p, stream);
 }
 
-hipError_t launch_conv3x3_body32(const ConvParams& p, int feat, int epilogue, Body32Form form, int ablate, hipStream_t stream) {
-  if ((size_t)p.h * p.w * feat * 4 >= 0x80000000ull) return hipErrorNotSupported;
+hipError_t launch_conv3x3_body32(const ConvParams& p_, int feat, int epilogue, Body32Form form, int ablate, hipStream_t stream) {
+  if ((size_t)p_.h * p_.w * feat * 4 >= 0x80000000ull) return hipErrorNotSupported;
+  ConvParams p = p_;
+  form = body32_form_at(form, p.h, p.w, &p.tiles_x, &p.tiles_y);
 #ifdef DSEN2_DIAG
   if (feat == 128 && ablate != 0) {
 #define DSEN2_ABL_ASYM(M)                                                                                \
@@ -324,6 +379,14 @@
                                 : launch_body32_one<128, 128, kEpiResidual, M, 0, kAsym, true>(p, stream);
     DSEN2_ABL_ASYM(3) DSEN2_ABL_ASYM(15) DSEN2_ABL_ASYM(16)
 #undef DSEN2_ABL_ASYM
+#define DSEN2_ABL_ROW(M, FORM, ROW)                                                                           \
+  if (ablate == M && form == Body32Form::FORM)                                                                \
+    return epilogue == kEpiRelu ? launch_body32_one<128, 128, kEpiRelu, M, 0, kAsym, true, ROW>(p, stream)    \
+                                : launch_body32_one<128, 128, kEpiResidual, M, 0, kAsym, true, ROW>(p, stream);
+    DSEN2_ABL_ROW(3, RowTile, 2) DSEN2_ABL_ROW(15, RowTile, 2) DSEN2_ABL_ROW(16, RowTile, 2)
+    DSEN2_ABL_ROW(3, RowTileNoSkip, 1) DSEN2_ABL_ROW(15, RowTileNoSkip, 1)
+    if (form == Body32Form::RowTile || form == Body32Form::RowTileNoSkip) return hipErrorInvalidValue;
+#undef DSEN2_ABL_ROW
 #define DSEN2_ABL(M)                                                                             \
   if (ablate == M)                                                                               \
     return epilogue == kEpiRelu ? launch_body32_one<128, 128, kEpiRelu, M>(p, stream)            \
diff --git a/dsen2_amd/csrc/conv3x3_dma.h b/dsen2_amd/csrc/conv3x3_dma.h
--- a/dsen2_amd/csrc/conv3x3_dma.h
+++ b/dsen2_amd/csrc/conv3x3_dma.h
@@ -7,14 +7,23 @@
 constexpr int KC = 32;
 constexpr int NT = 128;
 constexpr int THREADS = 512;
-constexpr int QS = 336;
-constexpr int IN_BYTES = 8 * QS * 16;
 constexpr int IN_BLOCKS = 6;
 constexpr int WCH = KC * NT;
 constexpr int NWBUF = 4;
-constexpr size_t LDS_BYTES = (size_t)2 * IN_BYTES + (size_t)NWBUF * WCH * 4 + 256 * 4;
-static_assert(QS >= kHaloPix && QS % 16 == 0 && 64 * (IN_BLOCKS - 1) + 16 == QS, "input chunk geometry");
-static_assert(LDS_BYTES <= 160 * 1024, "LDS budget");
+
+template <bool ROWT>
+struct Geom {
+  static constexpr int TH = ROWT ? 8 : kTile, TW = ROWT ? 32 : kTile;
+  static constexpr int HW = TW + 2;
+  static constexpr int HPIX = (TH + 2) * HW;
+  static constexpr int QS = ROWT ? 352 : 336;
+  static constexpr int TAIL = QS - 64 * (IN_BLOCKS - 1);
+  static constexpr int IN_BYTES = 8 * QS * 16;
+  static constexpr size_t LDS_BYTES = (size_t)2 * IN_BYTES + (size_t)NWBUF * WCH * 4 + 256 * 4;
+  static_assert(QS >= HPIX && QS % 16 == 0 && TAIL > 0 && TAIL <= 64 && TAIL % 16 == 0, "input chunk geometry");
+  static_assert((7 * QS + 64 * 4) * 16 + 1024 <= IN_BYTES && (7 * QS + 320) * 16 + TAIL * 16 == IN_BYTES, "input DMAs stay inside the buffer");
+  static_assert(LDS_BYTES <= 160 * 1024, "LDS budget");
+};
 
 template <int N>
 __device__ __forceinline__ void wait_vmcnt() {
@@ -28,8 +37,10 @@
 
 enum class Role { All, Issuer };
 
-template <int CINW, int NS, bool LAZY_VOFF = false, Role ROLE = Role::All>
+template <int CINW, int NS, bool LAZY_VOFF = false, Role ROLE = Role::All, bool ROWT = false>
 struct Stage {
+  using G_ = Geom<ROWT>;
+  static constexpr int QS = G_::QS, IN_BYTES = G_::IN_BYTES;
   static constexpr int N_W = ROLE == Role::Issuer ? 4 : 2;
   static constexpr int N_IN = ROLE == Role::Issuer ? 2 : 1;
   static constexpr int NCC = CINW / KC;
@@ -62,14 +73,14 @@
 
   __device__ __forceinline__ unsigned voff_of(int b, int ty0, int tx0) const {
     const int hp = 64 * b + lane;
-    const int hy = hp / kHalo, hx = hp - hy * kHalo;
+    const int hy = hp / G_::HW, hx = hp - hy * G_::HW;
     const int gy = ty0 - 1 + hy, gx = tx0 - 1 + hx;
-    const bool inb = hp < kHaloPix && (unsigned)gy < (unsigned)h && (unsigned)gx < (unsigned)w;
+    const bool inb = hp < G_::HPIX && (unsigned)gy < (unsigned)h && (unsigned)gx < (unsigned)w;
     return inb ? (unsigned)(((gy * w + gx) * CINW + wave * 4) * 4) : 0x80000000u;
   }
 
   __device__ __forceinline__ void set_stage_item(int item) {
-    const Tile t = tile_at<NS>(item, tiles_per_img, tiles_x);
+    const Tile t = tile_at<NS, G_::TH, G_::TW>(item, tiles_per_img, tiles_x);
     in_rsrc = __builtin_amdgcn_make_buffer_rsrc(const_cast<float*>(in) + (size_t)t.img * img_pix * CINW, 0,
                                                 (unsigned)(img_pix * CINW * 4), 0x00020000);
     if constexpr (LAZY_VOFF) {
@@ -94,7 +105,7 @@
                      "s_mov_b32 m0, %2\n\ts_nop 0\n\tbuffer_load_dwordx4 %3, %4, %6 offen lds\n\t"
                      "s_mov_b32 m0, %0"
                      : "=&s"(saved_m0) : "s"(m0v), "s"(m1v), "v"(voff), "s"(in_rsrc), "s"(so), "s"(so1) : "memory");
-      } else if (lane < 16) {
+      } else if (lane < G_::TAIL) {
         asm volatile("s_mov_b32 %0, m0\n\t"
                      "s_mov_b32 m0, %1\n\ts_nop 0\n\tbuffer_load_dwordx4 %3, %4, %5 offen lds\n\t"
                      "s_mov_b32 m0, %2\n\ts_nop 0\n\tbuffer_load_dwordx4 %3, %4, %6 offen lds\n\t"
@@ -107,7 +118,7 @@
     if (b < IN_BLOCKS - 1) {
       asm volatile("s_mov_b32 %0, m0\n\ts_mov_b32 m0, %1\n\ts_nop 0\n\tbuffer_load_dwordx4 %2, %3, %4 offen lds\n\ts_mov_b32 m0, %0"
                    : "=&s"(saved_m0) : "s"(m0v), "v"(voff), "s"(in_rsrc), "s"(so) : "memory");
-    } else if (lane < 16) {
+    } else if (lane < G_::TAIL) {
       asm volatile("s_mov_b32 %0, m0\n\ts_mov_b32 m0, %1\n\ts_nop 0\n\tbuffer_load_dwordx4 %2, %3, %4 offen lds\n\ts_mov_b32 m0, %0"
                    : "=&s"(saved_m0) : "s"(m0v), "v"(voff), "s"(in_rsrc), "s"(so) : "memory");
     }
diff --git a/dsen2_amd/csrc/conv_plan.hip b/dsen2_amd/csrc/conv_plan.hip
--- a/dsen2_amd/csrc/conv_plan.hip
+++ b/dsen2_amd/csrc/conv_plan.hip
@@ -113,6 +113,18 @@
   return true;
 }
 
+Body32Form body32_form_at(Body32Form form, int h, int w, int* tiles_x, int* tiles_y) {
+  const int tx16 = (w + kTile - 1) / kTile, ty16 = (h + kTile - 1) / kTile;
+  const int tx_row = (w + 31) / 32, ty_row = (h + 7) / 8;
+  const bool row = form == Body32Form::RowTile || form == Body32Form::RowTileNoSkip;
+  if (row && (long long)tx_row * ty_row <= (long long)tx16 * ty16) {
+    *tiles_x = tx_row; *tiles_y = ty_row;
+    return form;
+  }
+  *tiles_x = tx16; *tiles_y = ty16;
+  return row ? Body32Form::DeferAsym : form;
+}
+
 void pack(const ConvPlan& pl, const float* k, const float* bias, float* dst) {
   memset(dst, 0, sizeof(float) * (bias ? pl.floats : pl.weight_floats));
   switch (pl.kernel) {
diff --git a/dsen2_amd/csrc/dsen2_internal.h b/dsen2_amd/csrc/dsen2_internal.h
--- a/dsen2_amd/csrc/dsen2_internal.h
+++ b/dsen2_amd/csrc/dsen2_internal.h
@@ -34,12 +34,13 @@
 
 enum class FirstKernel { Direct, Tile16 };
 enum class BodyKernel { Body32, Tile };
-enum class Body32Form { StaggerA, Plain, DeferStaggerA, DeferStagger, DeferAsym, DeferAsymS0, DeferAsymS1, DeferAsymS3, DeferAsymPrio };
+enum class Body32Form { StaggerA, Plain, DeferStaggerA, DeferStagger, DeferAsym, DeferAsymS0, DeferAsymS1, DeferAsymS3, DeferAsymPrio,
+                        RowTileNoSkip, RowTile };
 enum class OutKernel { MfmaThenValu, Valu, Tile };
 struct Tuning {
   FirstKernel first = FirstKernel::Direct;
   BodyKernel body = BodyKernel::Body32;
-  Body32Form body32 = Body32Form::DeferAsym;
+  Body32Form body32 = Body32Form::RowTile;
   OutKernel out = OutKernel::MfmaThenValu;
   int ablate = 0;
   int grid_cap = 0;
@@ -84,6 +85,7 @@
 hipError_t launch_conv3x3_first16(const ConvParams& p, const FirstInputs& f, int cout, bool x3, hipStream_t stream);
 size_t first16_weight_u16(int cout, bool x3);
 void pack_first16_weights_host(const float* kernel_hwio, int cin, int cout, bool x3, uint16_t* dst);
+Body32Form body32_form_at(Body32Form form, int h, int w, int* tiles_x, int* tiles_y);
 hipError_t launch_conv3x3_body32(const ConvParams& p, int feat, int epilogue, Body32Form form, int ablate, hipStream_t stream);
 hipError_t launch_conv3x3_body16w(const ConvParams& p, int feat, int epilogue, bool x3, int ablate, hipStream_t stream, int grid_cap = 0);
 hipError_t launch_split3_f32(const float* in_nhwc, void* hx, void* lo, int n, int h, int w, int c, hipStream_t stream);
diff --git a/include/dsen2_hip.h b/include/dsen2_hip.h
--- a/include/dsen2_hip.h
+++ b/include/dsen2_hip.h
@@ -103,6 +103,7 @@
                              float scale, void *stream);
 int dsen2_conv3x3_wgrad_geometry(int kind, int n, int h, int w, int ca, int cg, long long *tiles, int *splits,
                                  size_t *workspace_floats);
+int dsen2_conv3x3_body32_geometry(int h, int w, int *row_tiles, int *tiles_x, int *tiles_y);
 int dsen2_join3_f32(const void *dev_hx, const void *dev_lo16, float *dev_out_nhwc, int n, int h, int w, int c, void *stream);
 
 int dsen2_model_set_loss(dsen2_model *m, int kind, float param, int mask_mode);
```

Measured after the change: 39940 patches/s. 1.6% lower.
